# pedro-morgado/spatialaudiogen

Measured on AMD Instinct MI355X. Metric: ambisonic seconds generated/sec (0.1 s windows, 224x448 video), higher is better.
Workload: dtype f32 (fp32 in / out / accumulate; products on the 16-bit matrix cores with fp32-equivalent operand splits: two fp16 planes (3 products per multiply) for the ResNet trunk's 3x3 convs, whose operand ranges batch-norm bounds, three bf16 planes (6 products) elsewhere - measured against the fp64 oracle as

## Files before the change

spatialaudiogen_amd/csrc/fft.hip:

```cpp
#include "kernels.h"
#include <mutex>

namespace sagen {

__device__ float2 g_tw[1024];
__device__ float g_hann[1024];

__global__ void fft_tables_kernel() {
    const int n = blockIdx.x * blockDim.x + threadIdx.x;
    if (n >= 1024) return;
    double s, c;
    sincospi(2.0 * (double)n / 1024.0, &s, &c);
    g_tw[n] = make_float2((float)c, (float)(-s));
    g_hann[n] = (float)(0.5 - 0.5 * cos(2.0 * M_PI / 1024.0 * (double)n));
}

int fft_tables_ensure(hipStream_t s) {
    static std::mutex mu;
    static bool done[64] = {};
    int dev = 0;
    SAGEN_HIP_CHECK(hipGetDevice(&dev));
    std::lock_guard<std::mutex> lk(mu);
    if (dev < 64 && done[dev]) return SAGEN_OK;
    hipLaunchKernelGGL(fft_tables_kernel, dim3(4), dim3(256), 0, s);
    SAGEN_LAUNCH_CHECK();
    SAGEN_HIP_CHECK(hipStreamSynchronize(s));
    if (dev < 64) done[dev] = true;
    return SAGEN_OK;
}

__device__ __forceinline__ float2 cmul(float2 a, float2 b) {
    return make_float2(a.x * b.x - a.y * b.y, a.x * b.y + a.y * b.x);
}

template <bool INV>
__device__ __forceinline__ float2* fft1024(float2* a, float2* b, int tid) {
    float2* src = a;
    float2* dst = b;
#pragma unroll
    for (int s = 0; s < 5; ++s) {
        const int Ns = 1 << (2 * s);
        const int k = tid & (Ns - 1);
        float2 u0 = src[tid], u1 = src[tid + 256], u2 = src[tid + 512], u3 = src[tid + 768];
        if (s > 0) {
            const int step = k * (256 / Ns);
            float2 w1 = g_tw[step], w2 = g_tw[2 * step], w3 = g_tw[3 * step];
            if (INV) { w1.y = -w1.y; w2.y = -w2.y; w3.y = -w3.y; }
            u1 = cmul(u1, w1); u2 = cmul(u2, w2); u3 = cmul(u3, w3);
        }
        const float2 v0 = make_float2(u0.x + u2.x, u0.y + u2.y);
        const float2 v1 = make_float2(u0.x - u2.x, u0.y - u2.y);
        const float2 v2 = make_float2(u1.x + u3.x, u1.y + u3.y);
        const float2 d = make_float2(u1.x - u3.x, u1.y - u3.y);
        const float2 v3 = INV ? make_float2(-d.y, d.x) : make_float2(d.y, -d.x);
        const int j0 = ((tid - k) << 2) + k;
        dst[j0] = make_float2(v0.x + v2.x, v0.y + v2.y);
        dst[j0 + Ns] = make_float2(v1.x + v3.x, v1.y + v3.y);
        dst[j0 + 2 * Ns] = make_float2(v0.x - v2.x, v0.y - v2.y);
        dst[j0 + 3 * Ns] = make_float2(v1.x - v3.x, v1.y - v3.y);
        __syncthreads();
        float2* t = src; src = dst; dst = t;
    }
    return src;
}

__global__ __launch_bounds__(256) void stft_kernel(const float* __restrict__ audio_, int n_samples, int f0, int f1,
                                                   float* __restrict__ mag_, int c0, int c1, float2* __restrict__ spec_,
                                                   float* __restrict__ zero_ptr_, int zero_n, const GroupInfo gi) {
    const float* __restrict__ audio = audio_ + (size_t)blockIdx.z * ((size_t)gridDim.y * n_samples);
    float* __restrict__ mag = SAGEN_GRP(mag_);
    float2* __restrict__ spec = SAGEN_GRP(spec_);
    float* __restrict__ zero_ptr = SAGEN_GRP(zero_ptr_);
    __shared__ float2 bufA[1024], bufB[1024];
    const int tid = threadIdx.x;
    for (int i = (blockIdx.y * gridDim.x + blockIdx.x) * 256 + tid; i < zero_n; i += gridDim.x * gridDim.y * 256) zero_ptr[i] = 0.f;
    const int b = blockIdx.y;
    const int fa = f0 + 2 * blockIdx.x, fb = fa + 1;
    const bool has_b = fb < f1;
    const float* xa = audio + (long)b * n_samples + 256L * fa;
#pragma unroll
    for (int t = 0; t < 4; ++t) {
        const int n = tid + 256 * t;
        const float h = g_hann[n];
        const float va = xa[n] * h;
        const float vb = has_b ? xa[256 + n] * h : 0.f;
        bufA[n] = make_float2(va, vb);
    }
    __syncthreads();
    const float2* Z = fft1024<false>(bufA, bufB, tid);
    const int nf = f1 - f0, nc = c1 - c0;
#pragma unroll
    for (int t = 0; t < 4; ++t) {
        const int k = tid + 256 * t;
        const float2 zk = Z[k];
        float2 zn = Z[(1024 - k) & 1023];
        zn.y = -zn.y;
        const float2 xA = make_float2(0.5f * (zk.x + zn.x), 0.5f * (zk.y + zn.y));
        const float dx = zk.x - zn.x, dy = zk.y - zn.y;
        const float2 xB = make_float2(0.5f * dy, -0.5f * dx);
        if (mag) {
            mag[((long)b * nf + (fa - f0)) * 1024 + k] = sqrtf(xA.x * xA.x + xA.y * xA.y);
            if (has_b) mag[((long)b * nf + (fb - f0)) * 1024 + k] = sqrtf(xB.x * xB.x + xB.y * xB.y);
        }
        if (spec && k <= 512) {
            if (fa >= c0 && fa < c1) spec[((long)b * nc + (fa - c0)) * 513 + k] = xA;
            if (has_b && fb >= c0 && fb < c1) spec[((long)b * nc + (fb - c0)) * 513 + k] = xB;
        }
    }
}

int stft_launch(const float* audio, int B, int n_samples, int f0, int f1, float* mag, int c0, int c1, float* spec,
                hipStream_t s, float* zero_ptr, int zero_n) {
    if (f1 <= f0 || 256L * (f1 - 1) + 1024 > n_samples)
        return fail(SAGEN_ERR_SHAPE, "stft: frames [%d,%d) do not fit %d samples", f0, f1, n_samples);
    if (spec && (c0 < f0 || c1 > f1 || c1 <= c0)) return fail(SAGEN_ERR_SHAPE, "stft: spec frames must lie in [f0,f1)");
    int rc = fft_tables_ensure(s);
    if (rc) return rc;
    const GroupInfo gi = cur_group();
    hipLaunchKernelGGL(stft_kernel, dim3(cdiv(f1 - f0, 2), B, gi.G), dim3(256), 0, s, audio, n_samples, f0, f1, mag, c0, c1,
                       (float2*)spec, zero_ptr, zero_ptr ? zero_n : 0, gi);
    SAGEN_LAUNCH_CHECK();
    return SAGEN_OK;
}

constexpr int MASK_F_LO = 1, MASK_F_HI = 24, MASK_NF = MASK_F_HI - MASK_F_LO;
constexpr int OUT_SHIFT = 1216;

template <int NTR>
__global__ __launch_bounds__(256) void mask_istft_kernel(const float* __restrict__ dmask_, long dmask_bstride, int dmask_f0,
                                                         const float2* __restrict__ spec_, const float* __restrict__ coeffs_,
                                                         float* __restrict__ frames_, const float* __restrict__ ebuf_, const GroupInfo gi) {
    const float* __restrict__ dmask = SAGEN_GRP(dmask_);
    const float2* __restrict__ spec = SAGEN_GRP(spec_);
    const float* __restrict__ coeffs = SAGEN_GRP(coeffs_);
    float* __restrict__ frames = SAGEN_GRP(frames_);
    const float* __restrict__ ebuf = SAGEN_GRP(ebuf_);
    __shared__ __attribute__((aligned(16))) float2 fftbuf[2048];
    float2* const bufA = fftbuf;
    float2* const bufB = fftbuf + 1024;
    __shared__ float E[6][1024];
    __shared__ float2 X[513];
    __shared__ float wl[2][3][NTR];
    const int tid = threadIdx.x;
    const int fi = blockIdx.x, f = MASK_F_LO + fi, b = blockIdx.y;
    const int n_lo = max(256 * f - OUT_SHIFT, 0), n_hi = min(256 * f - OUT_SHIFT + 1023, 4799);
    const int s_lo = n_lo / 1600, s_hi = n_hi / 1600;
    const bool two = s_hi != s_lo;

    for (int i = tid; i < 2 * 3 * NTR; i += 256) {
        const int j = i % NTR, o = (i / NTR) % 3, si = i / (3 * NTR);
        const int st = si ? s_hi : s_lo;
        wl[si][o][j] = coeffs[(((long)b * 3 + st) * 3 + o) * (NTR + 1) + j];
    }
    for (int k = tid; k < 513; k += 256) X[k] = spec[((long)b * 28 + f) * 513 + k];

    if (ebuf != nullptr) {
        const float4* src = reinterpret_cast<const float4*>(ebuf + ((long)b * MASK_NF + fi) * 1024 * 8);
        __syncthreads();
        for (int k = tid; k < 1024; k += 256) {
            const float4 lo = src[2 * k], hi = src[2 * k + 1];
            E[0][k] = lo.x; E[1][k] = lo.y; E[2][k] = lo.z; E[3][k] = lo.w; E[4][k] = hi.x; E[5][k] = hi.y;
        }
        __syncthreads();
    } else {
    constexpr int NC = NTR / 4;
    constexpr int RPP = 4096 / NTR;
    constexpr int TPRW = 256 / RPP;
    constexpr int NPASS = 1024 / RPP;
    float4* const stage = reinterpret_cast<float4*>(fftbuf);
    const float4* src = reinterpret_cast<const float4*>(dmask + (long)b * dmask_bstride + (long)(f - dmask_f0) * 1024 * NTR);
    float4 nx0 = src[tid], nx1 = src[tid + 256], nx2 = src[tid + 512], nx3 = src[tid + 768];
    __syncthreads();
    const int row = tid / TPRW, part = tid % TPRW;
    auto park = [&](int i, const float4& v) {
        const int idx = tid + 256 * i, r = idx / NC, ch = idx % NC;
        stage[r * NC + (ch ^ (r & (NC - 1)))] = v;
    };
#pragma unroll 1
    for (int ps = 0; ps < NPASS; ++ps) {
        park(0, nx0); park(1, nx1); park(2, nx2); park(3, nx3);
        __syncthreads();
        const int pn = ps + 1 < NPASS ? ps + 1 : ps;
        nx0 = src[pn * 1024 + tid]; nx1 = src[pn * 1024 + tid + 256]; nx2 = src[pn * 1024 + tid + 512]; nx3 = src[pn * 1024 + tid + 768];
        float e[6] = {0.f, 0.f, 0.f, 0.f, 0.f, 0.f};
#pragma unroll
        for (int q = 0; q < 4; ++q) {
            const float4 v = stage[row * NC + ((part * 4 + q) ^ (row & (NC - 1)))];
            const float sg[4] = {1.f / (1.f + expf(-v.x)), 1.f / (1.f + expf(-v.y)), 1.f / (1.f + expf(-v.z)),
                                 1.f / (1.f + expf(-v.w))};
#pragma unroll
            for (int u = 0; u < 4; ++u) {
                const int j = (part * 4 + q) * 4 + u;
#pragma unroll
                for (int o = 0; o < 3; ++o) {
                    e[o] = fmaf(wl[0][o][j], sg[u], e[o]);
                    if (two) e[3 + o] = fmaf(wl[1][o][j], sg[u], e[3 + o]);
                }
            }
        }
#pragma unroll
        for (int c = 0; c < 6; ++c) {
            e[c] = wave_sum<1, TPRW>(e[c]);
            if (part == 0) E[c][ps * RPP + row] = e[c];
        }
        __syncthreads();
    }
    }

    float* fout = frames + ((long)b * MASK_NF + fi) * 3 * 1024;
    const int npack = two ? 3 : 2;
    for (int pk = 0; pk < npack; ++pk) {
        int ca, cb;
        if (pk == 0) { ca = 0; cb = 1; }
        else if (pk == 1) { ca = 2; cb = two ? 5 : -1; }
        else { ca = 3; cb = 4; }
#pragma unroll
        for (int t = 0; t < 4; ++t) {
            const int k = tid + 256 * t;
            const int km = (1024 - k) & 1023;
            float2 xk = (k <= 512) ? X[k] : X[km];
            if (k > 512) xk.y = -xk.y;
            const float ma = 0.5f * (E[ca][k] + E[ca][km]);
            const float mb = cb >= 0 ? 0.5f * (E[cb][k] + E[cb][km]) : 0.f;
            bufA[k] = make_float2(ma * xk.x - mb * xk.y, ma * xk.y + mb * xk.x);
        }
        __syncthreads();
        const float2* Y = fft1024<true>(bufA, bufB, tid);
#pragma unroll
        for (int t = 0; t < 4; ++t) {
            const int p = tid + 256 * t;
            const int n = 256 * f + p - OUT_SHIFT;
            if (n >= 0 && n < 4800) {
                const int st = n / 1600;
                const float2 y = Y[p];
                const int oa = ca % 3, sa = (ca / 3) ? s_hi : s_lo;
                if (st == sa) fout[oa * 1024 + p] = y.x * (1.f / 1024.f);
                if (cb >= 0) {
                    const int ob = cb % 3, sb = (cb / 3) ? s_hi : s_lo;
                    if (st == sb) fout[ob * 1024 + p] = y.y * (1.f / 1024.f);
                }
            }
        }
        __syncthreads();
    }
}

__global__ __launch_bounds__(256) void ola_mix_kernel(const float* __restrict__ frames_, const float* __restrict__ coeffs_,
                                                      int ntr, float* __restrict__ out_, int B, const GroupInfo gi) {
    const float* __restrict__ frames = SAGEN_GRP(frames_);
    const float* __restrict__ coeffs = SAGEN_GRP(coeffs_);
    float* __restrict__ out = out_ + (size_t)blockIdx.z * ((size_t)B * 4800 * 3);
    const long total = (long)B * 4800 * 3;
    for (long i = (long)blockIdx.x * 256 + threadIdx.x; i < total; i += (long)gridDim.x * 256) {
        const int o = (int)(i % 3);
        long r = i / 3;
        const int n = (int)(r % 4800);
        const int b = (int)(r / 4800);
        const int st = n / 1600;
        float acc = 0.f;
        const int fl = max((n + 193 + 255) / 256, MASK_F_LO), fh = min((n + OUT_SHIFT) / 256, MASK_F_HI - 1);
        for (int f = fl; f <= fh; ++f)
            acc += frames[(((long)b * MASK_NF + (f - MASK_F_LO)) * 3 + o) * 1024 + (n + OUT_SHIFT - 256 * f)];
        out[i] = fmaf(acc, 0.25f, coeffs[(((long)b * 3 + st) * 3 + o) * (ntr + 1) + ntr]);
    }
}

size_t mask_istft_scratch_bytes(int B) { return (size_t)B * MASK_NF * 3 * 1024 * sizeof(float); }

int mask_istft_mix_launch(const float* dmask, long dmask_bstride, int dmask_f0, const float* spec, const float* coeffs,
                          int B, int ntracks, float* out, float* scratch, hipStream_t s, const float* ebuf) {
    int rc = fft_tables_ensure(s);
    if (rc) return rc;
    if (dmask_f0 > MASK_F_LO) return fail(SAGEN_ERR_SHAPE, "mask_istft: dmask must start at frame <= %d", MASK_F_LO);
    const GroupInfo gi = cur_group();
    dim3 grid(MASK_NF, B, gi.G);
    if (ntracks == 32)
        hipLaunchKernelGGL(mask_istft_kernel<32>, grid, dim3(256), 0, s, dmask, dmask_bstride, dmask_f0, (const float2*)spec, coeffs, scratch, ebuf, gi);
    else if (ntracks == 64)
        hipLaunchKernelGGL(mask_istft_kernel<64>, grid, dim3(256), 0, s, dmask, dmask_bstride, dmask_f0, (const float2*)spec, coeffs, scratch, ebuf, gi);
    else if (ntracks == 16)
        hipLaunchKernelGGL(mask_istft_kernel<16>, grid, dim3(256), 0, s, dmask, dmask_bstride, dmask_f0, (const float2*)spec, coeffs, scratch, ebuf, gi);
    else
        return fail(SAGEN_ERR_UNSUPPORTED, "mask_istft: num_sep_tracks=%d (supported: 16, 32, 64)", ntracks);
    SAGEN_LAUNCH_CHECK();
    const long total = (long)B * 4800 * 3;
    hipLaunchKernelGGL(ola_mix_kernel, dim3((int)std::min<long>(cdiv(total, 256), 4096L), 1, gi.G), dim3(256), 0, s, scratch, coeffs,
                       ntracks, out, B, gi);
    SAGEN_LAUNCH_CHECK();
    return SAGEN_OK;
}

__global__ __launch_bounds__(256) void stft_multi_kernel(const float* __restrict__ audio_, int n_samples, int nin, int f0, int f1,
                                                         float* __restrict__ mag_, int c0, int c1, float2* __restrict__ spec_,
                                                         float* __restrict__ zero_ptr_, int zero_n, const GroupInfo gi) {
    const float* __restrict__ audio = audio_ + (size_t)blockIdx.z * ((size_t)gridDim.y * n_samples * nin);
    float* __restrict__ mag = SAGEN_GRP(mag_);
    float2* __restrict__ spec = SAGEN_GRP(spec_);
    float* __restrict__ zero_ptr = SAGEN_GRP(zero_ptr_);
    __shared__ float2 bufA[1024], bufB[1024];
    const int tid = threadIdx.x;
    for (int i = (blockIdx.y * gridDim.x + blockIdx.x) * 256 + tid; i < zero_n; i += gridDim.x * gridDim.y * 256) zero_ptr[i] = 0.f;
    const int b = blockIdx.y, ch = blockIdx.x % nin;
    const int fa = f0 + 2 * (blockIdx.x / nin), fb = fa + 1;
    const bool has_b = fb < f1;
    const float* xa = audio + ((long)b * n_samples + 256L * fa) * nin + ch;
#pragma unroll
    for (int t = 0; t < 4; ++t) {
        const int n = tid + 256 * t;
        const float h = g_hann[n];
        const float va = xa[(long)n * nin] * h;
        const float vb = has_b ? xa[(long)(256 + n) * nin] * h : 0.f;
        bufA[n] = make_float2(va, vb);
    }
    __syncthreads();
    const float2* Z = fft1024<false>(bufA, bufB, tid);
    const int nf = f1 - f0, nc = c1 - c0;
#pragma unroll
    for (int t = 0; t < 4; ++t) {
        const int k = tid + 256 * t;
        const float2 zk = Z[k];
        float2 zn = Z[(1024 - k) & 1023];
        zn.y = -zn.y;
        const float2 xA = make_float2(0.5f * (zk.x + zn.x), 0.5f * (zk.y + zn.y));
        const float dx = zk.x - zn.x, dy = zk.y - zn.y;
        const float2 xB = make_float2(0.5f * dy, -0.5f * dx);
        if (mag) {
            mag[(((long)b * nf + (fa - f0)) * 1024 + k) * nin + ch] = sqrtf(xA.x * xA.x + xA.y * xA.y);
            if (has_b) mag[(((long)b * nf + (fb - f0)) * 1024 + k) * nin + ch] = sqrtf(xB.x * xB.x + xB.y * xB.y);
        }
        if (spec && k <= 512) {
            float2* sp = spec + ((long)b * nin + ch) * nc * 513;
            if (fa >= c0 && fa < c1) sp[(long)(fa - c0) * 513 + k] = xA;
            if (has_b && fb >= c0 && fb < c1) sp[(long)(fb - c0) * 513 + k] = xB;
        }
    }
}

int stft_multi_launch(const float* audio, int B, int n_samples, int nin, int f0, int f1, float* mag, int c0, int c1, float* spec,
                      hipStream_t s, float* zero_ptr, int zero_n) {
    if (nin < 1 || nin > 16) return fail(SAGEN_ERR_SHAPE, "stft: %d input channels", nin);
    if (f1 <= f0 || 256L * (f1 - 1) + 1024 > n_samples)
        return fail(SAGEN_ERR_SHAPE, "stft: frames [%d,%d) do not fit %d samples", f0, f1, n_samples);
    if (spec && (c0 < f0 || c1 > f1 || c1 <= c0)) return fail(SAGEN_ERR_SHAPE, "stft: spec frames must lie in [f0,f1)");
    int rc = fft_tables_ensure(s);
    if (rc) return rc;
    const GroupInfo gi = cur_group();
    hipLaunchKernelGGL(stft_multi_kernel, dim3(cdiv(f1 - f0, 2) * nin, B, gi.G), dim3(256), 0, s, audio, n_samples, nin, f0, f1, mag, c0, c1,
                       (float2*)spec, zero_ptr, zero_ptr ? zero_n : 0, gi);
    SAGEN_LAUNCH_CHECK();
    return SAGEN_OK;
}

template <int NTR, int NIN, int NOUT>
__global__ __launch_bounds__(256) void mask_istft_hoa_kernel(const float* __restrict__ dmask_, long dmask_bstride, int dmask_f0,
                                                             const float2* __restrict__ spec_, const float* __restrict__ coeffs_,
                                                             float* __restrict__ frames_, const GroupInfo gi) {
    constexpr int QPI = NTR / 4;
    constexpr int CPB = NIN * QPI;
    static_assert(CPB <= 64 && (CPB & (CPB - 1)) == 0, "one bin's chunks must fit a power-of-two lane group of a wave");
    constexpr int BPI = 256 / CPB;
    constexpr int NS = 2 * NOUT;
    const float* __restrict__ dmask = SAGEN_GRP(dmask_);
    const float2* __restrict__ spec = SAGEN_GRP(spec_);
    const float* __restrict__ coeffs = SAGEN_GRP(coeffs_);
    float* __restrict__ frames = SAGEN_GRP(frames_);
    __shared__ float2 Y[NS][1024];
    __shared__ float2 fbuf[2][1024];
    const int tid = threadIdx.x;
    const int fi = blockIdx.x, f = MASK_F_LO + fi, b = blockIdx.y;
    const int n_lo = max(256 * f - OUT_SHIFT, 0), n_hi = min(256 * f - OUT_SHIFT + 1023, 4799);
    const int s_lo = n_lo / 1600, s_hi = n_hi / 1600;
    const bool two = s_hi != s_lo;

    const int q = tid % CPB, i = q / QPI, j0 = (q % QPI) * 4;
    float w[2][NOUT][4];
#pragma unroll
    for (int si = 0; si < 2; ++si)
#pragma unroll
        for (int o = 0; o < NOUT; ++o)
#pragma unroll
            for (int u = 0; u < 4; ++u)
                w[si][o][u] = coeffs[((((long)b * 3 + (si ? s_hi : s_lo)) * NOUT + o) * NIN + i) * (NTR + 1) + j0 + u];
    const float4* src = reinterpret_cast<const float4*>(dmask + (long)b * dmask_bstride + (long)(f - dmask_f0) * 1024 * NIN * NTR);
    const float2* X = spec + ((long)b * NIN + i) * 28 * 513 + (long)f * 513;
#pragma unroll 2
    for (int k = tid / CPB; k < 1024; k += BPI) {
        const float4 v = src[(long)k * CPB + q];
        float2 xk = X[k <= 512 ? k : 1024 - k];
        if (k > 512) xk.y = -xk.y;
        const float sg[4] = {1.f / (1.f + expf(-v.x)), 1.f / (1.f + expf(-v.y)), 1.f / (1.f + expf(-v.z)), 1.f / (1.f + expf(-v.w))};
        float yr[2][NOUT], yi[2][NOUT];
#pragma unroll
        for (int si = 0; si < 2; ++si)
#pragma unroll
            for (int o = 0; o < NOUT; ++o) {
                float m = 0.f;
#pragma unroll
                for (int u = 0; u < 4; ++u) m = fmaf(w[si][o][u], sg[u], m);
                m = wave_sum<1, QPI>(m);
                yr[si][o] = wave_sum<QPI, CPB>(m * xk.x);
                yi[si][o] = wave_sum<QPI, CPB>(m * xk.y);
            }
        if (q == 0) {
#pragma unroll
            for (int si = 0; si < 2; ++si)
#pragma unroll
                for (int o = 0; o < NOUT; ++o) Y[si * NOUT + o][k] = make_float2(yr[si][o], yi[si][o]);
        }
    }
    __syncthreads();

    float* fout = frames + ((long)b * MASK_NF + fi) * NOUT * 1024;
    const int ns = two ? NS : NOUT;
    for (int ca = 0; ca < ns; ca += 2) {
        const int cb = ca + 1 < ns ? ca + 1 : -1;
#pragma unroll
        for (int t = 0; t < 4; ++t) {
            const int k = tid + 256 * t;
            const int km = (1024 - k) & 1023;
            const float2 a0 = Y[ca][k], a1 = Y[ca][km];
            const float2 ha = make_float2(0.5f * (a0.x + a1.x), 0.5f * (a0.y - a1.y));
            float2 hb = make_float2(0.f, 0.f);
            if (cb >= 0) {
                const float2 b0 = Y[cb][k], b1 = Y[cb][km];
                hb = make_float2(0.5f * (b0.x + b1.x), 0.5f * (b0.y - b1.y));
            }
            fbuf[0][k] = make_float2(ha.x - hb.y, ha.y + hb.x);
        }
        __syncthreads();
        const float2* R = fft1024<true>(fbuf[0], fbuf[1], tid);
#pragma unroll
        for (int t = 0; t < 4; ++t) {
            const int p = tid + 256 * t;
            const int n = 256 * f + p - OUT_SHIFT;
            if (n >= 0 && n < 4800) {
                const int st = n / 1600;
                const float2 y = R[p];
                if (st == ((ca / NOUT) ? s_hi : s_lo)) fout[(ca % NOUT) * 1024 + p] = y.x * (1.f / 1024.f);
                if (cb >= 0 && st == ((cb / NOUT) ? s_hi : s_lo)) fout[(cb % NOUT) * 1024 + p] = y.y * (1.f / 1024.f);
            }
        }
        __syncthreads();
    }
}

template <int NIN, int NOUT>
__global__ __launch_bounds__(256) void ola_mix_hoa_kernel(const float* __restrict__ frames_, const float* __restrict__ coeffs_,
                                                          int ntr, float* __restrict__ out_, int B, const GroupInfo gi) {
    const float* __restrict__ frames = SAGEN_GRP(frames_);
    const float* __restrict__ coeffs = SAGEN_GRP(coeffs_);
    float* __restrict__ out = out_ + (size_t)blockIdx.z * ((size_t)B * 4800 * NOUT);
    const long total = (long)B * 4800 * NOUT;
    for (long idx = (long)blockIdx.x * 256 + threadIdx.x; idx < total; idx += (long)gridDim.x * 256) {
        const int o = (int)(idx % NOUT);
        const long r = idx / NOUT;
        const int n = (int)(r % 4800);
        const int b = (int)(r / 4800);
        const int st = n / 1600;
        float acc = 0.f;
        const int fl = max((n + 193 + 255) / 256, MASK_F_LO), fh = min((n + OUT_SHIFT) / 256, MASK_F_HI - 1);
        for (int f = fl; f <= fh; ++f)
            acc += frames[(((long)b * MASK_NF + (f - MASK_F_LO)) * NOUT + o) * 1024 + (n + OUT_SHIFT - 256 * f)];
        out[idx] = fmaf(acc, 0.25f, coeffs[((((long)b * 3 + st) * NOUT + o) * NIN + 0) * (ntr + 1) + ntr]);
    }
}

size_t mask_istft_hoa_scratch_bytes(int B, int nout) { return (size_t)B * MASK_NF * nout * 1024 * sizeof(float); }

int mask_istft_hoa_launch(const float* dmask, long dmask_bstride, int dmask_f0, const float* spec, const float* coeffs, int B,
                          int ntracks, int nin, int nout, float* out, float* scratch, hipStream_t s) {
    int rc = fft_tables_ensure(s);
    if (rc) return rc;
    if (dmask_f0 > MASK_F_LO || dmask_f0 < 0) return fail(SAGEN_ERR_SHAPE, "mask_istft_hoa: dmask must start at frame 0..%d", MASK_F_LO);
    if (nin != 4 || nout != 5) return fail(SAGEN_ERR_UNSUPPORTED, "mask_istft_hoa: (nin, nout) = (%d, %d) (supported: (4, 5), ambi_order 2)", nin, nout);
    const GroupInfo gi = cur_group();
    dim3 grid(MASK_NF, B, gi.G);
    if (ntracks == 32)
        hipLaunchKernelGGL((mask_istft_hoa_kernel<32, 4, 5>), grid, dim3(256), 0, s, dmask, dmask_bstride, dmask_f0, (const float2*)spec, coeffs, scratch, gi);
    else if (ntracks == 64)
        hipLaunchKernelGGL((mask_istft_hoa_kernel<64, 4, 5>), grid, dim3(256), 0, s, dmask, dmask_bstride, dmask_f0, (const float2*)spec, coeffs, scratch, gi);
    else if (ntracks == 16)
        hipLaunchKernelGGL((mask_istft_hoa_kernel<16, 4, 5>), grid, dim3(256), 0, s, dmask, dmask_bstride, dmask_f0, (const float2*)spec, coeffs, scratch, gi);
    else
        return fail(SAGEN_ERR_UNSUPPORTED, "mask_istft_hoa: num_sep_tracks=%d (supported: 16, 32, 64)", ntracks);
    SAGEN_LAUNCH_CHECK();
    const long total = (long)B * 4800 * nout;
    hipLaunchKernelGGL((ola_mix_hoa_kernel<4, 5>), dim3((int)std::min<long>(cdiv(total, 256), 4096L), 1, gi.G), dim3(256), 0, s, scratch, coeffs,
                       ntracks, out, B, gi);
    SAGEN_LAUNCH_CHECK();
    return SAGEN_OK;
}

template <int NTR>
__global__ __launch_bounds__(256) void mask_istft_bwd_kernel(const float* __restrict__ dmask, long dmask_bstride, int dmask_f0,
                                                             const float2* __restrict__ spec, const float* __restrict__ coeffs,
                                                             const float* __restrict__ dpred, float* __restrict__ d_dmask,
                                                             long dd_bstride, int dd_f0, float* __restrict__ partial) {
    __shared__ __attribute__((aligned(16))) float2 fftbuf[2048];
    float2* const bufA = fftbuf;
    float2* const bufB = fftbuf + 1024;
    __shared__ float Q[6][1024];
// ... 162 lines not shown
```

spatialaudiogen_amd/csrc/kernels.h:

```cpp
#pragma once
#include "common.h"
#include "wave_reduce.h"

namespace sagen {

struct BnRef {
    const double* acc = nullptr;
    const float* gamma = nullptr;
    const float* beta = nullptr;
    double inv_count = 0.0;
    float eps = 1e-3f;
};

constexpr int H2_AMAX_SLOTS = 64, H2_AMAX_STRIDE = 32, H2_AMAX_FLOATS = H2_AMAX_SLOTS * H2_AMAX_STRIDE;

struct IgemmDesc {
    const float* x = nullptr;
    const float* w = nullptr;
    int w_split = 0;
    float* y = nullptr;
    const float* bias = nullptr;
    const float* in_scale = nullptr;
    const float* in_shift = nullptr;
    BnRef bn_in;
// ... 2 lines not shown
    float* splitk_ws = nullptr;
    int* sk_ticket = nullptr;
    int sk_rep = 1;
    int M = 0, N = 0, K = 0, Kpad = 0;
    int Hg = 1, Wg = 1, g_h0 = 0, g_w0 = 0;
    int Hin = 1, Win = 1, Cin = 0, ldx = 0;
    long x_bstride = 0;
    int in_sh = 1, in_sw = 1;
    int ntaps = 1, TW = 1, tap_sh = 1, tap_sw = 1, tap_h0 = 0, tap_w0 = 0;
    int log2Cin = -1;
    int dsh = 1, dsw = 1, Cout = 0;
    int Hlim = 1, Wlim = 1;
    long y_bstride = 0;
    long y_rstride = 0;
    int ldy = 0;
    int relu_out = 0;
    int splitk = 1;
    unsigned x_bytes = 0, w_bytes = 0;
    unsigned y_bytes = 0;
    int no_bounds = 0;
    int uniform_taps = 0;
    const void* xp3 = nullptr;
    unsigned xp3_bytes = 0, xp3_cstride = 0;
    int p3_np = 0;
    int xp3_fmt = 0;
    int xp3_row0 = 0, xp3_rows = 0;
    const void* wh2 = nullptr;
    unsigned wh2_bytes = 0;
    const float* h2_a_inv = nullptr;
    const float* h2_w_inv = nullptr;
    unsigned p3_magic_wp = 0, p3_magic_h = 0;
    const float* mm_coeffs = nullptr;
    float* mm_out = nullptr;
    int mm_row0 = 0, mm_nf = 0;
    int mm_f_lo = 1;
    void* trace = nullptr;
    int trace_block = 0;
    GroupInfo grp;
};
__device__ __forceinline__ void igemm_relocate(IgemmDesc& d, int g) {
    const GroupInfo gi = d.grp;
    d.x = grp_ptr(d.x, gi, g); d.y = grp_ptr(d.y, gi, g);
    d.in_scale = grp_ptr(d.in_scale, gi, g); d.in_shift = grp_ptr(d.in_shift, gi, g);
    d.bn_in.acc = grp_ptr(d.bn_in.acc, gi, g);
    d.stats = grp_ptr(d.stats, gi, g); d.amax_out = grp_ptr(d.amax_out, gi, g);
    d.splitk_ws = grp_ptr(d.splitk_ws, gi, g); d.sk_ticket = grp_ptr(d.sk_ticket, gi, g);
    d.xp3 = grp_ptr(d.xp3, gi, g);
    d.h2_a_inv = grp_ptr(d.h2_a_inv, gi, g); d.h2_w_inv = grp_ptr(d.h2_w_inv, gi, g);
    d.mm_coeffs = grp_ptr(d.mm_coeffs, gi, g); d.mm_out = grp_ptr(d.mm_out, gi, g);
}

enum IgemmTile {
    TILE_128x128 = 0, TILE_128x64, TILE_256x64, TILE_64x64, TILE_128x32, TILE_32x128,
    TILE_128x128_S2, TILE_128x64_S2, TILE_256x64_S2, TILE_64x64_S2,
    TILE_64x128, TILE_64x128_S2, TILE_64x256, TILE_64x256_S2, TILE_256x32,
    TILE_64x64_K32, TILE_64x128_K32, TILE_128x64_K32, TILE_128x128_K32, TILE_32x128_K32, TILE_128x32_K32,
    TILE_B3_128x128, TILE_B3_128x64, TILE_B3_256x64, TILE_B3_64x64, TILE_B3_64x128, TILE_B3_64x256, TILE_B3_32x128,
    TILE_B3_128x32,
    TILE_B3_128x64_K2, TILE_B3_64x64_K2, TILE_B3_64x128_K2, TILE_B3_32x128_K2, TILE_B3_128x32_K2,
    TILE_B3DW_128x128, TILE_B3DW_128x64, TILE_B3DW_256x64, TILE_B3DW_64x128, TILE_B3DW_64x64, TILE_B3DW_64x256,
    TILE_B3DWM_128x64, TILE_B3DWM_256x64, TILE_B3DWM_64x64, TILE_B3DWM_64x128,
    TILE_B3S2_256x64, TILE_B3S2_128x64,
    TILE_P3_128x64, TILE_P3_128x128, TILE_P3_64x64,
    TILE_P3PP_PAIR, TILE_P3PP_SPLITK,
    TILE_P3G_128x64_K2, TILE_P3G_64x64_K2, TILE_P3G_64x128_K2, TILE_P3G_128x128_K1,
    TILE_P3H_128x64, TILE_P3H_128x128, TILE_P3H_64x64, TILE_P3H_256x64,
    TILE_P3GH_128x64_K3, TILE_P3GH_64x64_K4, TILE_P3GH_128x128_K2, TILE_P3GH_64x128_K3,
    TILE_P3H_128x64_C2, TILE_P3H_64x64_C2, TILE_P3H_64x64_C4,
    TILE_P3GH_MM_64x128_K2, TILE_P3GH_MM_64x128_K4, TILE_P3GH_MM_128x128_K2, TILE_P3GH_MM_128x256_K2,
    TILE_P3HR_256x64, TILE_P3HR_128x64, TILE_P3HR_64x64_C2,
    TILE_P3HR_128x128,
    TILE_AUTO
};

int igemm_launch(const IgemmDesc& d, IgemmTile tile, hipStream_t s);
int igemm_grid_m(const IgemmDesc& d, IgemmTile tile);
IgemmTile igemm_pick_tile(const IgemmDesc& d);
const char* igemm_tile_name(IgemmTile t);
int igemm_tile_bm(IgemmTile t);
int igemm_tile_bn(IgemmTile t);
int igemm_tile_bk(IgemmTile t);
bool igemm_tile_split(IgemmTile t);
int igemm3_dispatch(const IgemmDesc& d, IgemmTile tile, hipStream_t s);
int igemm3dw_dispatch(const IgemmDesc& d, IgemmTile tile, hipStream_t s);
int igemm3s2_dispatch(const IgemmDesc& d, IgemmTile tile, hipStream_t s);
int conv3p_dispatch(const IgemmDesc& d, IgemmTile tile, hipStream_t s);
int conv3g_dispatch(const IgemmDesc& d, IgemmTile tile, hipStream_t s);
int conv3h_dispatch(const IgemmDesc& d, IgemmTile tile, hipStream_t s);
int h2_filter_pack_launch(const float* wp, int N, int Kpad, void* w2, unsigned* scratch, float* w_inv, hipStream_t s);
struct H2Job {
    const float* wp = nullptr;
    void* w2 = nullptr;
    float* w_inv = nullptr;
    int N = 0, Kpad = 0, first_block = 0, pad_ = 0;
};
int h2_filter_pack_multi_launch(const H2Job* jobs_dev, int njobs, int nblocks, unsigned* amax, hipStream_t s);
bool conv3g_ok(const IgemmDesc& d);
constexpr int SK_TICKETS = 8192;
inline bool igemm_tile_fused_splitk(IgemmTile) { return true; }
bool igemm_tile_p3(IgemmTile t);
bool igemm_tile_grouped(IgemmTile t);
bool igemm_tile_dh_split(IgemmTile t);
bool igemm_p3_eligible(const IgemmDesc& d);
bool igemm_tile_ok(const IgemmDesc& d, IgemmTile t);
constexpr int SPLITK_RB = 16;
int splitk_reduce_launch(const float* ws, int splitk, int M, int N, const float* bias, int relu,
                         float* y, int ldy, int rep, double* stats, hipStream_t s, float* amax_out = nullptr);

struct DeconvGather {
    int B = 0, Hin = 0, Win = 0, kh = 1, kw = 1, sh = 1, sw = 1, Cout = 0;
    int in_row0 = 0, R = 0;
    int y0 = 0, y1 = 0;
    int relu = 0, ldy = 0;
    const float* bias = nullptr;
    float* y = nullptr;
    float* amax_out = nullptr;
};
int deconv_gather_launch(const float* ws, int splitk, const DeconvGather& g, hipStream_t s);

int pack_conv_launch(const float* w_hwio, int ntaps, int cin_src, int cin_pad, int cout,
                     float* wp, int Npad, int Kpad, hipStream_t s, int tw_src = 0, int tw_pad = 0);
int pack_split_launch(float* wp, int N, int Kpad, hipStream_t s);
inline size_t packed_split_floats(size_t n_fp32) { return n_fp32 + (3 * n_fp32 + 1) / 2; }
enum PackKind { PACK_CONV = 0, PACK_DECONV, PACK_FLIPT, PACK_ROWS, PACK_DECONV_PHASE };
struct PackJob {
    const float* src = nullptr;
    float* dst = nullptr;
    int kind = 0, N = 0, Kpad = 0;
    int p[7] = {0, 0, 0, 0, 0, 0, 0};
    int first_block = 0;
};
inline int pack_job_blocks(int kind, long N, long Kpad) {
    return kind == PACK_CONV ? (int)(((N + 31) / 32) * ((Kpad + 31) / 32)) : (int)((N * Kpad + 1023) / 1024);
}
int pack_multi_launch(const PackJob* jobs_dev, int njobs, int nblocks, hipStream_t s, int block0 = 0);
int pack_deconv_launch(const float* w_hwoi, int kh, int kw, int cout, int cin, int sh, int sw,
                       float* wp, int Npad, int Kpad, hipStream_t s);

int bn_finalize_launch(const double* stats, long count, int C, const float* gamma,
                       const float* beta, float eps, float* scale, float* shift, hipStream_t s);
int bn_apply_relu_launch(const float* x, const float* scale, const float* shift, const BnRef& bn, const float* residual,
                         float* y, long n_pixels, int C, hipStream_t s);
int maxpool3x3s2_launch(const float* x, const float* scale, const float* shift, const BnRef& bn, float* y,
                        int B, int H, int W, int C, hipStream_t s);
int pad_nhwc3to4_launch(const float* x, float* y, int B, int H, int W, int pt, int pb, int pl, int pr,
                        hipStream_t s);
int pad_u8_nhwc3to4_launch(const unsigned char* x, float* y, int B, int H, int W, int pt, int pb, int pl, int pr, hipStream_t s);
int stempool_launch(const float* xpad, const float* wp, const float* gamma, float* pooled, double* stats, int B, hipStream_t s);
size_t stem8_plane_bytes(int B);
int stem8_prep_launch(const unsigned char* x, void* plane, int B, hipStream_t s, float* zero_ptr = nullptr, long zero_n = 0, int half = 0);
int stem8pool_h2_launch(const void* plane, const float* wp, const void* wh2, const float* w_inv, const float* gamma, float* pooled, double* stats, int B,
                        hipStream_t s);
int stem8pool_launch(const void* plane, const float* wp, const float* gamma, float* pooled, double* stats, int B, hipStream_t s);
int stem16_prep_launch(const float* x, void* planes, float* part, float* a_inv, int B, hipStream_t s, float* zero_ptr = nullptr, long zero_n = 0);
int stem16pool_launch(const void* planes, const void* wh2, const float* gamma, float* pooled, double* stats, const float* a_inv, const float* w_inv,
                      int B, hipStream_t s);
constexpr int STEM16_PARTS = 1024;
int stem8raw_launch(const void* plane, const float* wp, float* y0, double* stats, int B, hipStream_t s);
int stem8rawpool_launch(const void* plane, const float* wp, const float* gamma, float* y0, float* pooled, double* stats, int B, hipStream_t s);
int assemble_wyzx_launch(const float* audio, const float* yzx, float* out, int B, int snd_size,
                         int snd_contx, int snd_dur, hipStream_t s);
int power_map_launch(const float* ambi, long T, const float* sh, int P, float* rms, hipStream_t s);
int power_map_batched_launch(const float* ambi, int nchunks, long T, const float* sh, int P, float* rms, double* moments, hipStream_t s);
int nosep_mix_launch(const float* audio, const float* coeffs, float* out, int B, int snd_size,
                     int snd_contx, int snd_dur, int num_out, hipStream_t s);
int nosep_mix_multi_launch(const float* audio, const float* coeffs, float* out, int B, int snd_size, int snd_contx,
                           int snd_dur, int nin, int num_out, hipStream_t s);

size_t p3_bytes(int B, int H, int W, int C);
constexpr int H2S_FILTER_FIRST = 8;
constexpr int H2S_FIXED_FIRST = 232;
constexpr int H2S_A_INV_X = 232;
constexpr int H2S_A_INV_B = 236;
constexpr int H2S_S16_A_INV = 238;
constexpr int H2_RIG_OFF = 240;
struct P3hScale {
    float* a_inv = nullptr;
    const float* res_bound = nullptr;
    const double* res_acc = nullptr;
    double res_inv_count = 0.0;
    float* bound_out = nullptr;
    unsigned* sat_count = nullptr;
    unsigned char* relu_bits = nullptr;
    const void* res_planes = nullptr;
    const float* res_a_inv = nullptr;
};
int p3_pack_launch(const float* x, const float* scale, const float* shift, const BnRef& bn, const float* residual, int relu,
                   float* y, void* p3, int B, int H, int W, int C, hipStream_t s, int fmt = 0, const P3hScale* h2 = nullptr);
size_t p3h_bytes(int B, int H, int W, int C);
int h2_pack_rows_launch(const float* x, long x_bstride, long x_rstride, int ldx, int row0, int B, int R, int W, int C, const float* amax0,
                        const float* amax1, void* planes, float* a_inv, unsigned* sat_count, hipStream_t s);
int p3_maxpool_launch(const float* x, const float* scale, const float* shift, const BnRef& bn, float* y, void* p3, int B, int H,
                      int W, int C, hipStream_t s, int fmt = 0, const P3hScale* h2 = nullptr);

int fft_tables_ensure(hipStream_t s);
int stft_launch(const float* audio, int B, int n_samples, int f0, int f1, float* mag,
                int c0, int c1, float* spec, hipStream_t s, float* zero_ptr = nullptr, int zero_n = 0);
size_t mask_istft_scratch_bytes(int B);
int mask_istft_mix_launch(const float* dmask, long dmask_bstride, int dmask_f0, const float* spec,
                          const float* coeffs, int B, int ntracks, float* out, float* scratch,
                          hipStream_t s, const float* ebuf = nullptr);
int stft_multi_launch(const float* audio, int B, int n_samples, int nin, int f0, int f1, float* mag, int c0, int c1, float* spec,
                      hipStream_t s, float* zero_ptr = nullptr, int zero_n = 0);
size_t mask_istft_hoa_scratch_bytes(int B, int nout);
int mask_istft_hoa_launch(const float* dmask, long dmask_bstride, int dmask_f0, const float* spec, const float* coeffs, int B,
                          int ntracks, int nin, int nout, float* out, float* scratch, hipStream_t s);

size_t eval_scratch_floats(int B);
int eval_init_launch(float* scratch, hipStream_t s);
int eval_metrics_launch(const float* pred, const float* gt, int B, float* ps, double* pw, float* scratch, hipStream_t s);
size_t eval_scratch_floats_c(int B, int C);
int eval_metrics_c_launch(const float* pred, const float* gt, int B, int C, float* ps, double* pw, float* scratch, hipStream_t s);
size_t evalx_scratch_floats(int B, int C);
int evalx_mel_env_launch(const float* pred, const float* gt, int B, int C, float* mel_lsd, float* env_mse, float* scratch,
                         hipStream_t s);
int evalx_emd_launch(const float* p, const float* q, int n_maps, int nodes, const double* cost, double* out, unsigned int* not_converged,
                     hipStream_t s);

int stft_loss_grad_launch(const float* pred, const float* gt, const float* mask, int B, float* grad, double* loss, hipStream_t s);
int adam_update_launch(float* p, const float* g, float* m, float* v, long n, float lr_t, float beta1, float beta2, float eps,
                       float gscale, hipStream_t s);

struct WgradDesc {
    const float* g = nullptr;
    const float* d = nullptr;
    float* out = nullptr;
    float* ws = nullptr;
    int B = 1, Hd = 1, Wd = 1;
    int HG = 1, WG = 1, ldg = 0, Cg = 0;
    int ldd = 0, Cd = 0;
    unsigned g_bstride = 0, g_rstride = 0, d_bstride = 0, d_rstride = 0;
    int sh = 1, sw = 1, TH = 1, TW = 1, h0 = 0, w0 = 0;
    int tsh = 1, tsw = 1;
    int splitk = 1;
    int defer_reduce = 0;
    const void* gp = nullptr;
    const void* dp = nullptr;
    const float* gp_a_inv = nullptr;
    const float* dp_a_inv = nullptr;
    unsigned gp_bytes = 0, dp_bytes = 0;
    int P = 0, fold = 1;
    unsigned g_bytes = 0, d_bytes = 0, magic_w = 0, magic_h = 0;
};
int wgrad_launch(const WgradDesc& d, hipStream_t s);
int wgrad_pick_splitk(const WgradDesc& d, size_t ws_capacity_floats);
int wgrad_reduce_launch(const WgradDesc& d, hipStream_t s);
const char* wgrad_kernel_name(const WgradDesc& d);
bool wgrad_reads_fp32_operands();
bool wgrad_planes_enabled();

size_t reduce_scratch_floats(int C);
int relu_bwd_launch(const float* ga, int lda, const float* gb, int ldb, const float* act, int ldact, float* dy, int lddy, long R,
                    int C, double* colsum, float* scratch, hipStream_t s, float* colsum_f32 = nullptr,
                    long band_rows = 0, long batch_rows = 0, long row0 = 0);
int bn_bwd_reduce_launch(const float* ga, const float* gb, const float* act, const float* y, const BnRef& bn, long n_pixels, int C,
                         double* acc, float* scratch, hipStream_t s, int self_mask = 0, float* mx_part = nullptr, int* mx_blocks = nullptr,
                         const unsigned char* relu_bits = nullptr);
int bn_bwd_apply_launch(const float* ga, const float* gb, const float* act, const float* y, const BnRef& bn, const double* acc,
                        long n_pixels, int C, float* dy, float* dz_out, float* dgamma, float* dbeta, hipStream_t s, int self_mask = 0);
int bn_bwd_apply_h2_launch(const float* ga, const float* gb, const float* act, const float* y, const BnRef& bn, const double* acc,
                           int B, int H, int W, int C, float* dy, float* dz_out, float* dgamma, float* dbeta, hipStream_t s, int self_mask,
                           void* planes, const float* mx_part, int mx_blocks, float* a_inv, unsigned* sat_count,
                           const unsigned char* relu_bits = nullptr);
int maxpool_bwd_launch(const float* y0, const BnRef& bn, const float* pooled, const float* ga, const float* gb, float* dz,
                       int B, int H, int W, int C, hipStream_t s);
int maxpool_bn_bwd_launch(const float* y0, const BnRef& bn, const float* pooled, const float* ga, const float* gb, float* dy0, int B,
                          int H, int W, int C, double* acc, float* scratch, float* dgamma, float* dbeta, hipStream_t s,
                          const float* pooled_raw = nullptr);
int sum_rows_launch(const float* ina, int lda, const float* inb, int ldb, int rep, long M, int C, float* out, int ldo, hipStream_t s);
int acc_to_f32_launch(const double* acc, float* dst, int n, hipStream_t s);
int bn_moving_update_launch(const BnRef& bn, float* moving_mean, float* moving_var, int C, float decay, hipStream_t s);
constexpr int BN_MOVING_MAX_JOBS = 40;
struct BnMovingJob { const double* acc = nullptr; double inv_count = 0.0; float* mm = nullptr; float* mv = nullptr; int C = 0; };
int bn_moving_update_multi_launch(const BnMovingJob* jobs, int n, float decay, hipStream_t s);
int pack_conv_flipT_launch(const float* w_hwio, int ntaps, int cin, int cout, float* wp, int Kpad, hipStream_t s);
int pack_rows_launch(const float* w, int rows, int cols, float* wp, int Kpad, hipStream_t s);
int stem_wgrad_unpack_launch(const float* tmp, float* dw, hipStream_t s);

size_t mask_istft_bwd_scratch_floats(int B, int ntracks);
int mask_istft_mix_bwd_launch(const float* dmask, long dmask_bstride, int dmask_f0, const float* spec, const float* coeffs,
                              const float* dpred, int B, int ntracks, float* d_dmask, long dd_bstride, int dd_f0, float* dcoeffs,
                              int ldc, float* scratch, hipStream_t s);

}
```

spatialaudiogen_amd/csrc/model.h:

```cpp
#pragma once
#include "kernels.h"
#include "fcm.h"
#include <algorithm>
#include <cstdlib>
#include <functional>
#include <map>
#include <string>
#include <vector>

namespace sagen {

struct VarSpec {
    std::string name;
    int ndim;
    int64_t shape[4];
    long numel() const {
        long n = 1;
        for (int i = 0; i < ndim; ++i) n *= shape[i];
        return n;
    }
};

struct Buf {
    size_t off = 0, n = 0;
};

struct Named {
    Buf buf;
    size_t extra_off = 0;
    int ndim = 0;
    int64_t shape[4] = {0, 0, 0, 0};
    int64_t pixel_stride = 0;
};

static const int AENC_F[5] = {32, 64, 128, 256, 512};
static const int AENC_K[5][2] = {{7, 16}, {3, 7}, {3, 5}, {3, 5}, {3, 5}};
static const int AENC_S[5][2] = {{4, 8}, {2, 4}, {2, 2}, {1, 1}, {1, 1}};

}

using namespace sagen;

constexpr int SAGEN_MAX_GROUPS = 32;

struct ProfRec {
    std::string kernel, layer;
    double flops = 0.0;
    hipEvent_t e0 = nullptr, e1 = nullptr;
};

struct Choice {
    int tile = -1;
    int splitk = 0;
    float us = 0.f;
};

struct sagen_ctx {
    sagen_config cfg;
    std::map<std::string, Choice> plan;
    std::map<std::string, bool> materialize;
    bool tuning = false;
    bool fp32_only = false;
    bool use_p3 = true;
    int p3_from_stage = 3;
    hipEvent_t tune_e0 = nullptr, tune_e1 = nullptr;
    hipStream_t aux = nullptr;
    hipEvent_t ev_fork = nullptr, ev_join = nullptr, ev_stft = nullptr, ev_pack = nullptr;
    int pack_early_jobs = 0, pack_early_blocks = 0;
    bool late_repack = false;
    bool profiling = false;
    std::vector<ProfRec> prof;
    std::vector<hipEvent_t> event_pool;
    size_t events_used = 0;
    int B = 0;
    int snd_size = 52799, snd_contx = 48000, snd_dur = 4800;
    int enc_h[6], enc_w[6], enc_c[6];
    int Cb = 0;
    int nsep = 32;
    int nin = 1, nout = 3;
    bool has_video = false, has_flow = false, freq_mask = true;

    std::vector<VarSpec> vars;
    std::map<std::string, int> var_index;
    std::vector<const float*> var_ptr;
    bool bound = false;

    int G = 1;
    int tune_groups = 0;
    int inter_group = 0;
    size_t grp_off = 0, grp_floats = 0;
    GroupInfo group_info() const {
        GroupInfo gi;
        if (G > 1 && ws) {
            gi.lo = reinterpret_cast<const char*>(ws + grp_off);
            gi.span = (unsigned long long)grp_floats * sizeof(float);
            gi.stride = gi.span;
            gi.G = G;
        }
        return gi;
    }
    size_t ws_floats = 0;
    float* ws = nullptr;
    std::map<std::string, Buf> bufs;
    std::map<std::string, Named> named;
    std::vector<PackJob> pack_jobs, pack_jobs_bwd;
    int pack_blocks = 0, pack_blocks_bwd = 0;
    bool train_mode = false;
    bool train_ready = false;
    bool stem_fused = true;
    bool materialize_mask = false;
    bool mask_fused_last = false;
    bool video_u8 = false;
    bool train_h2 = true;
    bool use_h2 = true;
    bool train_h2d = true;
    bool no_aud_planes = false;
    bool no_dh_split = false;
    bool sk_fused = false;
    bool train_h2w = true;
    std::map<std::string, int> h2d_slot;
    std::vector<H2Job> h2d_jobs;
    int h2d_blocks = 0;
    std::map<std::string, int> h2_slot;
    std::vector<H2Job> h2_jobs;
    int h2_blocks = 0;
    bool use_p3g = true;
    bool rawpool_last = false;
    bool train_rawpool = true;
    bool train_bands = true;
    int dec_lo[7] = {0, 0, 0, 0, 0, 0, 0}, dec_hi[7] = {0, 0, 0, 0, 0, 0, 0};
    bool no_scatter = false, no_d1_planes = false, no_lean_trunk = false;
    int dec_planes_min_batch = 16;
    bool use_fcm = false;
    std::map<std::string, int> fcm_slices;
    bool stem8h = true;
    bool stem16 = true;
    bool stem8 = true;
    size_t tws_floats = 0;
    float* tws = nullptr;
    std::map<std::string, Buf> tbufs;
    std::vector<float*> grad_ptr;
    std::vector<int> ms_bucket;
    std::vector<int> ms_count, ms_left;
    std::vector<hipEvent_t> ms_event;
    std::vector<char> ms_done;
    std::vector<int> ms_touched;
    hipEvent_t ms_tmp = nullptr;
    std::vector<float*> mov_ptr;
    Buf talloc(const std::string& name, size_t n) {
        Buf b;
        b.off = tws_floats;
        b.n = n;
        tws_floats += (n + 63) / 64 * 64;
        tbufs[name] = b;
        return b;
    }
    size_t cap(const std::string& name) const { auto it = bufs.find(name); return it != bufs.end() ? it->second.n : tbufs.at(name).n; }

    Buf alloc(const std::string& name, size_t n) {
        Buf b;
        b.off = ws_floats;
        b.n = n;
        ws_floats += (n + 63) / 64 * 64;
        bufs[name] = b;
        return b;
    }
    float* p(const std::string& name) const {
        auto it = bufs.find(name);
        if (it != bufs.end()) return ws + it->second.off;
        return tws + tbufs.at(name).off;
    }
    const float* v(const std::string& name) const { return var_ptr[var_index.at(name)]; }
    void add_var(const std::string& name, std::initializer_list<int64_t> shape) {
        VarSpec s;
        s.name = name;
        s.ndim = (int)shape.size();
        int i = 0;
        for (auto d : shape) s.shape[i++] = d;
        for (; i < 4; ++i) s.shape[i] = 1;
        var_index[name] = (int)vars.size();
        vars.push_back(s);
    }
    void expose(const std::string& name, const std::string& buf, size_t extra, std::initializer_list<int64_t> shape,
                int64_t pixel_stride) {
        Named nm;
        nm.buf = bufs.at(buf);
        nm.extra_off = extra;
        nm.ndim = (int)shape.size();
        int i = 0;
        for (auto d : shape) nm.shape[i++] = d;
        nm.pixel_stride = pixel_stride;
        named[name] = nm;
    }
};

namespace sagen {

static inline void add_resnet_vars(sagen_ctx* c, const std::string& scope) {
    auto bn = [&](const std::string& p, int ch) {
        for (const char* leaf : {"beta", "gamma", "moving_mean", "moving_variance"}) c->add_var(p + "/bn/" + leaf, {ch});
    };
    c->add_var(scope + "/conv1/conv/weights", {7, 7, 3, 64});
    bn(scope + "/conv1/conv", 64);
    int cin = 64;
    const int couts[4] = {64, 128, 256, 512};
    for (int st = 0; st < 4; ++st) {
        const int cout = couts[st];
        for (int unit = 1; unit <= 2; ++unit) {
            const std::string pfx = scope + "/conv" + std::to_string(st + 2) + "_" + std::to_string(unit);
            if (unit == 1 && cin != cout) c->add_var(pfx + "/shortcut/weights", {1, 1, cin, cout});
            c->add_var(pfx + "/conv_1/weights", {3, 3, cin, cout});
            bn(pfx + "/conv_1", cout);
            c->add_var(pfx + "/conv_2/weights", {3, 3, cout, cout});
            bn(pfx + "/conv_2", cout);
            cin = cout;
        }
    }
}

static inline bool conv3g_ok_desc(const IgemmDesc& d, int cin) {
    return cin % 16 == 0 && d.Kpad == d.K && d.in_scale == nullptr && d.bn_in.acc == nullptr && d.dsh * d.dsw == 1;
}

static inline size_t packed_floats(long N, long K) { return (size_t)N * ((K + 15) / 16 * 16); }

static inline int auto_splitk(const IgemmDesc& d, IgemmTile tile) {
    const int bm = (tile == TILE_32x128) ? 32 : 64, bn = (tile == TILE_32x128) ? 128 : 64;
    const long blocks = (long)cdiv(d.M, bm) * cdiv(d.N, bn);
    const int nk = d.Kpad / 16;
    if (blocks >= 384 || nk < 16) return 1;
    int sk = (int)std::min<long>({(512 + blocks - 1) / blocks, (long)nk / 8, 64L});
    return std::max(sk, 1);
}

}


int sagen_repack_impl(sagen_ctx* c, hipStream_t s);
int sagen_repack_part(sagen_ctx* c, hipStream_t s, int part);
bool sagen_forward_forks(const sagen_ctx* c);
int sagen_upload_pack_jobs(std::vector<PackJob>& jobs, void* dev, hipStream_t s);
int sagen_forward_impl(sagen_ctx* c, const float* audio, const float* video, const float* flow, float* out, hipStream_t s);

namespace sagen {

struct Fwd {
    sagen_ctx* c;
    hipStream_t s;
    int rc = SAGEN_OK;
    std::string layer;
    std::string wsname = "splitk";
    std::string sfx;
    hipEvent_t wait_before_mfma = nullptr;
    hipEvent_t wait_packs = nullptr;
    std::function<int(const float* ws, int sk, hipStream_t s)> custom_reduce;
    const char* custom_reduce_name = "";

    hipEvent_t next_event() {
        if (c->events_used == c->event_pool.size()) {
            hipEvent_t e = nullptr;
            if (hipEventCreate(&e) != hipSuccess) return nullptr;
            c->event_pool.push_back(e);
        }
        return c->event_pool[c->events_used++];
    }
    template <class F>
    void timed(const char* kernel, double flops, F&& launch) {
        if (rc) return;
        if (!c->profiling) { rc = launch(); return; }
        ProfRec r;
        r.kernel = kernel; r.layer = layer; r.flops = flops;
        r.e0 = next_event(); r.e1 = next_event();
        if (!r.e0 || !r.e1) { rc = fail(SAGEN_ERR_HIP, "hipEventCreate failed"); return; }
        hipError_t he = hipEventRecord(r.e0, s);
        rc = launch();
        if (he == hipSuccess) he = hipEventRecord(r.e1, s);
        if (he != hipSuccess && !rc) rc = fail(SAGEN_ERR_HIP, "hipEventRecord: %s", hipGetErrorString(he));
        c->prof.push_back(r);
    }

    bool dense_out(const IgemmDesc& d) const {
        return d.dsh * d.dsw == 1 && d.g_h0 == 0 && d.g_w0 == 0 && d.y_rstride == (long)d.Wg * d.ldy &&
               (d.M <= d.Hg * d.Wg || d.y_bstride == (long)d.Hg * d.Wg * d.ldy);
    }
    size_t ws_capacity() const { return c->bufs.at(wsname).n; }
    hipError_t memset_groups(void* p, size_t bytes) {
        for (int g = 0; g < c->G; ++g) {
            const hipError_t e = hipMemsetAsync(reinterpret_cast<char*>(p) + (size_t)g * c->grp_floats * sizeof(float), 0, bytes, s);
            if (e != hipSuccess) return e;
        }
// ... 105 lines not shown
        for (int k = 0; k < nc; ++k) {
            std::sort(runs[k].begin(), runs[k].end());
            top[k].us = runs[k][runs[k].size() / 2];
            if (top[k].us < top[best].us) best = k;
        }
        return top[best];
    }

    int contract(const IgemmDesc& d_in, int rep = 1, bool allow_split = true) {
        if (rc) return 0;
        IgemmDesc d = d_in;
        d.w_split = c->fp32_only ? 0 : 1;
        if (rep > 1 && !dense_out(d)) { rc = fail(SAGEN_ERR_UNSUPPORTED, "replicated store needs a dense plain epilogue"); return 0; }
        Choice ch;
        auto it = c->plan.find(layer);
        if (c->tuning) {
            const bool was_prof = c->profiling;
            c->profiling = false;
            ch = tune(d, rep, allow_split);
            c->profiling = was_prof;
            c->plan[layer] = ch;
            if (d.stats && !rc && memset_groups(d.stats, (size_t)2 * d.N * sizeof(double)) != hipSuccess)
                rc = fail(SAGEN_ERR_HIP, "autotune: memset failed");
        } else if (it != c->plan.end()) {
            ch = it->second;
            if (!igemm_tile_ok(d, (IgemmTile)ch.tile)) ch = heuristic(d, rep, allow_split);
            const bool dh3 = ch.splitk == 3 && igemm_tile_dh_split((IgemmTile)ch.tile);
            if (ch.splitk > 1 && (!allow_split || !dense_out(d) || (igemm_tile_p3((IgemmTile)ch.tile) && !dh3) || d.Kpad / igemm_tile_bk((IgemmTile)ch.tile) / ch.splitk < 1)) ch.splitk = 1;
        } else {
            ch = heuristic(d, rep, allow_split);
        }
        if ((ch.splitk > 1 || rep > 1 || custom_reduce) && (size_t)std::max(ch.splitk, 1) * d.M * d.N > ws_capacity()) {
            rc = fail(SAGEN_ERR_WORKSPACE, "split-K scratch too small for %s", layer.c_str());
            return 0;
        }
        return run_choice(d, rep, (IgemmTile)ch.tile, std::max(ch.splitk, 1));
    }
    void gemm(const IgemmDesc& d, int rep = 1, bool allow_split = true) { contract(d, rep, allow_split); }

    IgemmDesc conv_desc(const float* x, int Hin, int Win, int Cin, int ldx, const float* wp, int kh, int kw, int sh, int sw,
                        bool same, int Cout, float* y, int ldy, int& Hout, int& Wout) {
        IgemmDesc d;
        int pt = 0, pl = 0;
        if (same) {
            Hout = cdiv(Hin, sh); Wout = cdiv(Win, sw);
            pt = std::max((Hout - 1) * sh + kh - Hin, 0) / 2;
            pl = std::max((Wout - 1) * sw + kw - Win, 0) / 2;
        } else {
            Hout = (Hin - kh) / sh + 1; Wout = (Win - kw) / sw + 1;
        }
        d.x = x; d.w = wp; d.y = y;
        d.M = c->B * Hout * Wout; d.N = Cout; d.K = kh * kw * Cin; d.Kpad = (d.K + 15) / 16 * 16;
        d.Hg = Hout; d.Wg = Wout;
        d.Hin = Hin; d.Win = Win; d.Cin = Cin; d.ldx = ldx; d.x_bstride = (long)Hin * Win * ldx;
        d.in_sh = sh; d.in_sw = sw;
        d.ntaps = kh * kw; d.TW = kw; d.tap_sh = 1; d.tap_sw = 1; d.tap_h0 = -pt; d.tap_w0 = -pl;
        d.log2Cin = ilog2_exact(Cin);
        d.Cout = Cout; d.Hlim = Hout; d.Wlim = Wout;
        d.ldy = ldy; d.y_rstride = (long)Wout * ldy; d.y_bstride = (long)Hout * Wout * ldy;
        return d;
    }

    void fc(const float* x, int M, int K, int ldx, const std::string& name, int N, bool relu, float* y, int ldy, int rep = 1, float* amax_out = nullptr) {
        layer = name;
        IgemmDesc d;
        d.x = x; d.w = c->p("pk:" + name + "/weights"); d.y = y; d.bias = c->v(name + "/biases");
        d.M = M; d.N = N; d.K = K; d.Kpad = (K + 15) / 16 * 16;
        d.Hg = 1; d.Wg = 1; d.Hin = 1; d.Win = 1; d.Cin = K; d.ldx = ldx; d.x_bstride = ldx;
        d.ntaps = 1; d.Cout = N; d.Hlim = 1; d.Wlim = 1; d.ldy = ldy; d.y_rstride = ldy; d.y_bstride = ldy;
        d.relu_out = relu;
        d.amax_out = amax_out;
        gemm(d, rep);
    }

    void deconv(const float* x, int Hin, int Win, int Cin, int l, float* y, int ldy, bool relu, int a0, int a1, int Ylim,
                long y_bstride, long y_row0, const float* mm_coeffs = nullptr, float* mm_out = nullptr, int mm_nf = 0,
                const std::function<void(IgemmDesc&)>& tweak = nullptr) {
        const std::string name = "separation/deconv" + std::to_string(l + 1);
        layer = name;
        const int kh = AENC_K[l][0], kw = AENC_K[l][1], sh = AENC_S[l][0], sw = AENC_S[l][1];
        const int Cout = l == 0 ? c->nsep * c->nin : AENC_F[l - 1];
        const int Hout = Hin * sh + kh - sh, Wout = Win * sw + kw - sw;
        const int nth = cdiv(kh, sh), ntw = cdiv(kw, sw);
        IgemmDesc d;
        d.x = x; d.w = c->p("pk:" + name + "/weights"); d.bias = c->v(name + "/biases");
        d.Hg = (a1 > a0 ? a1 - a0 : cdiv(Hout, sh)); d.g_h0 = a0; d.Wg = cdiv(Wout, sw);
        d.M = c->B * d.Hg * d.Wg; d.N = sh * sw * Cout; d.K = nth * ntw * Cin; d.Kpad = (d.K + 15) / 16 * 16;
        d.Hin = Hin; d.Win = Win; d.Cin = Cin; d.ldx = Cin; d.x_bstride = (long)Hin * Win * Cin;
        d.ntaps = nth * ntw; d.TW = ntw; d.tap_sh = -1; d.tap_sw = -1; d.log2Cin = ilog2_exact(Cin);
        d.dsh = sh; d.dsw = sw; d.Cout = Cout;
        d.Hlim = Ylim > 0 ? Ylim : Hout; d.Wlim = Wout;
        d.ldy = ldy; d.y_rstride = (long)Wout * ldy;
        d.y_bstride = y_bstride > 0 ? y_bstride : (long)Hout * Wout * ldy;
        d.y = y - y_row0 * d.y_rstride;
        d.relu_out = relu;
        if (mm_out) { d.mm_coeffs = mm_coeffs; d.mm_out = mm_out; d.mm_row0 = (int)y_row0; d.mm_nf = mm_nf; d.mm_f_lo = 1; }
        if (tweak) tweak(d);
        gemm(d);
    }

    float* cat_amax(int l, int half) { return c->p("amax") + (size_t)((l - 1) * 2 + half) * H2_AMAX_FLOATS; }
    float* cat_a_inv(int l) { return c->p("amax") + (size_t)10 * H2_AMAX_FLOATS + l; }
    void deconv_scatter(const float* x, int Hin, int Win, int Cin, int l, float* y, int ldy, bool relu, int in_row0, int R, int y0, int y1,
                        float* amax_out = nullptr, bool x_planes = false) {
        const std::string name = "separation/deconv" + std::to_string(l + 1);
        layer = name;
        DeconvGather gd;
        gd.B = c->B; gd.Hin = Hin; gd.Win = Win; gd.kh = AENC_K[l][0]; gd.kw = AENC_K[l][1]; gd.sh = AENC_S[l][0]; gd.sw = AENC_S[l][1];
        gd.Cout = l == 0 ? c->nsep : AENC_F[l - 1];
        gd.in_row0 = in_row0; gd.R = R; gd.y0 = y0; gd.y1 = y1; gd.relu = relu ? 1 : 0; gd.ldy = ldy;
        gd.bias = c->v(name + "/biases"); gd.y = y; gd.amax_out = amax_out;
        IgemmDesc d;
        d.x = x + (long)in_row0 * Win * Cin; d.w = c->p("pks:" + name + "/weights");
        d.M = c->B * R * Win; d.N = gd.kh * gd.kw * gd.Cout; d.K = Cin; d.Kpad = Cin;
        d.Hg = R; d.Wg = Win; d.Hin = Hin - in_row0; d.Win = Win; d.Cin = Cin; d.ldx = Cin; d.x_bstride = (long)Hin * Win * Cin;
        d.ntaps = 1; d.Cout = d.N; d.Hlim = R; d.Wlim = Win; d.ldy = d.N; d.y_rstride = (long)Win * d.N; d.y_bstride = (long)R * Win * d.N;
        d.y = c->ws + c->bufs.at(wsname).off;
        if (x_planes && !c->tuning) {
            auto it = c->plan.find(name);
            if (it != c->plan.end() && !igemm_tile_p3((IgemmTile)it->second.tile)) x_planes = false;
        }
        if (x_planes) {
            const int lx = l + 1;
            void* planes = c->p("catp");
            timed("h2_pack_rows_kernel", 0.0, [&] {
                return h2_pack_rows_launch(x, (long)Hin * Win * Cin, (long)Win * Cin, Cin, in_row0, c->B, R, Win, Cin, cat_amax(lx, 0), cat_amax(lx, 1), planes,
                                           cat_a_inv(lx), reinterpret_cast<unsigned*>(c->p("h2s") + 7), s); });
            d.xp3 = planes; d.xp3_fmt = 1; d.xp3_row0 = 0; d.xp3_rows = R;
            d.p3_np = c->B * R * (Win + 1);
            d.xp3_cstride = (unsigned)((size_t)d.p3_np * 64);
            d.xp3_bytes = (unsigned)((size_t)d.xp3_cstride * (Cin / 16));
            d.wh2 = c->p("pkhs:" + name + "/weights"); d.wh2_bytes = (unsigned)((size_t)d.N * d.Kpad * 4);
            d.h2_a_inv = cat_a_inv(lx); d.h2_w_inv = c->p("h2s") + c->h2_slot.at("pks:" + name);
        }
        custom_reduce_name = "deconv_gather_kernel";
        custom_reduce = [gd](const float* ws, int sk, hipStream_t st) { return deconv_gather_launch(ws, sk, gd, st); };
        gemm(d);
        custom_reduce = nullptr;
    }

    bool h2() const { return c->use_h2 && c->use_p3 && !c->fp32_only && (!c->train_mode || c->train_h2); }
    int p3_fmt() const { return h2() ? 1 : 0; }
    float* h2_a_inv() { return c->p("h2s") + (sfx.empty() ? 0 : 1); }
    float* h2_a_inv_x(int parity) { return c->p("h2s") + H2S_A_INV_X + 2 * (parity & 1) + (sfx.empty() ? 0 : 1); }
    float* h2_a_inv_b() { return c->p("h2s") + H2S_A_INV_B + (sfx.empty() ? 0 : 1); }
    float* h2_xbound(int parity) { return c->p("h2s") + 2 + 2 * (parity & 1) + (sfx.empty() ? 0 : 1); }
    P3hScale h2_scale(float* bound_out = nullptr, const float* res_bound = nullptr, const double* res_acc = nullptr, double res_inv_count = 0.0) {
        P3hScale h;
        h.a_inv = h2_a_inv(); h.bound_out = bound_out; h.res_bound = res_bound; h.res_acc = res_acc; h.res_inv_count = res_inv_count;
        h.sat_count = reinterpret_cast<unsigned*>(c->p("h2s") + 7);
        return h;
    }

    double* bn_acc(int layer_index) { return reinterpret_cast<double*>(c->p("bnacc" + sfx)) + (size_t)layer_index * 2 * 512; }
    BnRef bn_ref(int layer_index, const std::string& bn_name, long count) {
        BnRef r;
        r.acc = bn_acc(layer_index);
        r.gamma = c->v(bn_name + "/bn/gamma");
        r.beta = c->v(bn_name + "/bn/beta");
        r.inv_count = 1.0 / (double)count;
        r.eps = 1e-3f;
        return r;
    }

    void conv_bn(const float* x, int Hin, int Win, int Cin, const std::string& name, int k, int stride, int Cout,
                 const BnRef& bn_in, float* y, int& Hout, int& Wout, int bn_index, const std::string& plan_key = "",
                 const void* planes = nullptr, const float* planes_a_inv = nullptr) {
        if (rc) return;
        IgemmDesc d = conv_desc(x, Hin, Win, Cin, Cin, c->p("pk:" + name + "/weights"), k, k, stride, stride, true, Cout, y,
                                Cout, Hout, Wout);
        if (planes) {
            d.xp3 = planes;
            d.p3_np = c->B * Hin * (Win + 1);
            auto hs = c->h2_slot.find(name);
            if (h2() && (stride == 1 || c->use_p3g) && k == 3 && hs != c->h2_slot.end()) {
                d.xp3_fmt = 1;
                d.xp3_cstride = (unsigned)((size_t)d.p3_np * 64);
                d.xp3_bytes = (unsigned)p3h_bytes(c->B, Hin, Win, Cin);
                d.wh2 = c->p("pkh:" + name + "/weights");
                d.wh2_bytes = (unsigned)((size_t)d.N * d.Kpad * 4);
                d.h2_a_inv = planes_a_inv ? planes_a_inv : h2_a_inv();
                d.h2_w_inv = c->p("h2s") + hs->second;
            } else {
                d.xp3_cstride = (unsigned)((size_t)d.p3_np * 96);
                d.xp3_bytes = (unsigned)p3_bytes(c->B, Hin, Win, Cin);
            }
        }
        d.bn_in = bn_in;
        d.stats = bn_acc(bn_index);
        layer = plan_key.empty() ? name : plan_key;
        contract(d);
    }

    const float* resnet(const float* img, const std::string& scope) {
        const int B = c->B;
        int li = 0;
        const bool tune_general = c->tuning && c->G == 1;
        const bool fast8 = c->video_u8 && scope == "video_encoder" && c->stem8 && !tune_general && !c->fp32_only && !c->train_mode;
        const bool fast8h = fast8 && c->stem8h && h2() && c->h2_slot.count(scope + "/conv1/conv") != 0;
        const bool fast16 = !fast8 && !(c->video_u8 && scope == "video_encoder") && c->stem16 && !tune_general && !c->fp32_only && !c->train_mode && h2() &&
                            c->use_p3 && c->p3_from_stage <= 2 && c->bufs.count("s16:part" + sfx) != 0 && c->h2_slot.count(scope + "/conv1/conv") != 0;
        if (!fast8 && !fast16 && !rc && hipMemsetAsync(c->p("bnacc" + sfx), 0, c->bufs.at("bnacc" + sfx).n * sizeof(float), s) != hipSuccess)
            rc = fail(SAGEN_ERR_HIP, "hipMemsetAsync(bn accumulators) failed");
        layer = scope + "/pad";
        const bool pool_planes = c->use_p3 && c->p3_from_stage <= 2;
        const bool no_lean = c->no_lean_trunk;
        const bool lean = !no_lean && h2() && pool_planes && c->use_p3g && c->bufs.count("p3b" + sfx) != 0 && !c->train_mode;
        float* const s16_a_inv = c->p("h2s") + H2S_S16_A_INV + (sfx.empty() ? 0 : 1);
        if (fast16)
            timed("stem16_amax_kernel+stem16_prep_kernel", 0.0, [&] { return stem16_prep_launch(img, c->p("xpad" + sfx), c->p("s16:part" + sfx), s16_a_inv, B, s,
                                                                                               c->p("bnacc" + sfx), (long)c->bufs.at("bnacc" + sfx).n); });
        else if (fast8)
            timed("stem8_prep_kernel", 0.0, [&] { return stem8_prep_launch(reinterpret_cast<const unsigned char*>(img), c->p("xpad" + sfx), B, s,
                                                                          c->p("bnacc" + sfx), (long)c->bufs.at("bnacc" + sfx).n, fast8h ? 1 : 0); });
        else if (c->video_u8 && scope == "video_encoder")
            timed("pad_u8_nhwc3to4_kernel", 0.0, [&] { return pad_u8_nhwc3to4_launch(reinterpret_cast<const unsigned char*>(img), c->p("xpad" + sfx), B, 224, 448, 2, 3, 2, 4, s); });
        else
            timed("pad_nhwc3to4_kernel", 0.0, [&] { return pad_nhwc3to4_launch(img, c->p("xpad" + sfx), B, 224, 448, 2, 3, 2, 4, s); });
        int H = 0, W = 0;
        if (!rc && wait_before_mfma) {
            if (hipStreamWaitEvent(s, wait_before_mfma, 0) != hipSuccess) rc = fail(SAGEN_ERR_HIP, "hipStreamWaitEvent failed");
            wait_before_mfma = nullptr;
        }
        {
            const std::string name = scope + "/conv1/conv";
            const bool fused = c->stem_fused && !c->tuning && !c->fp32_only && !(c->use_p3 && c->p3_from_stage <= 2);
            if (fast8 || fast16) {
                H = 112; W = 224;
                layer = name + "+pool";
                if (fast16)
                    timed("stem8pool_kernel<f16>", 2.0 * B * H * W * 64 * 224, [&] {
                        return stem16pool_launch(c->p("xpad" + sfx), c->p("pkh:" + name + "/weights"), c->v(name + "/bn/gamma"), c->p("rx0" + sfx), bn_acc(li),
                                                 s16_a_inv, c->p("h2s") + c->h2_slot.at(name), B, s); });
                else if (fast8h)
                    timed("stem8pool_kernel<h2>", 2.0 * B * H * W * 64 * 224, [&] {
                        return stem8pool_h2_launch(c->p("xpad" + sfx), c->p("pk:" + name + "/weights"), c->p("pkh:" + name + "/weights"), c->p("h2s") + c->h2_slot.at(name),
                                                   c->v(name + "/bn/gamma"), c->p("rx0" + sfx), bn_acc(li), B, s); });
                else
                timed("stem8pool_kernel", 2.0 * B * H * W * 64 * 224, [&] {
                    return stem8pool_launch(c->p("xpad" + sfx), c->p("pk:" + name + "/weights"), c->v(name + "/bn/gamma"), c->p("rx0" + sfx), bn_acc(li), B, s); });
                const BnRef bnf = bn_ref(li, name, (long)B * H * W);
                layer = name + "/bn-relu";
                P3hScale hs0 = h2_scale(h2_xbound(0));
                if (lean) hs0.a_inv = h2_a_inv_x(0);
                if (pool_planes)
                    timed("p3_pack_kernel", 0.0, [&] { return p3_pack_launch(c->p("rx0" + sfx), nullptr, nullptr, bnf, nullptr, 1, lean ? nullptr : c->p("rx0" + sfx), c->p("p3" + sfx), B, 56, 112, 64, s, p3_fmt(), &hs0); });
                else
                    timed("bn_apply_relu_kernel", 0.0, [&] { return bn_apply_relu_launch(c->p("rx0" + sfx), nullptr, nullptr, bnf, nullptr, c->p("rx0" + sfx), (long)B * 56 * 112, 64, s); });
            } else if (fused) {
                H = 112; W = 224;
                layer = name + "+pool";
                timed("stempool_kernel", 2.0 * B * H * W * 64 * 224, [&] {
                    return stempool_launch(c->p("xpad" + sfx), c->p("pk:" + name + "/weights"), c->v(name + "/bn/gamma"), c->p("rx0" + sfx), bn_acc(li), B, s); });
                const BnRef bnf = bn_ref(li, name, (long)B * H * W);
                layer = name + "/bn-relu";
                timed("bn_apply_relu_kernel", 0.0, [&] { return bn_apply_relu_launch(c->p("rx0" + sfx), nullptr, nullptr, bnf, nullptr, c->p("rx0" + sfx), (long)B * 56 * 112, 64, s); });
            } else {
            IgemmDesc d = conv_desc(c->p("xpad" + sfx), 229, 454, 4, 4, c->p("pk:" + name + "/weights"), 7, 8, 2, 2, false, 64,
                                    c->p("y0" + sfx), 64, H, W);
            d.stats = bn_acc(li);
            layer = name;
            contract(d);
            const BnRef bn = bn_ref(li, name, (long)B * H * W);
            if (c->use_p3 && c->p3_from_stage <= 2)
            {
                P3hScale hs0 = h2_scale(h2_xbound(0));
                if (lean) hs0.a_inv = h2_a_inv_x(0);
                timed("p3_maxpool_kernel", 0.0, [&] { return p3_maxpool_launch(c->p("y0" + sfx), nullptr, nullptr, bn, lean ? nullptr : c->p("rx0" + sfx), c->p("p3" + sfx), B, H, W, 64, s, p3_fmt(), &hs0); });
            }
            else
                timed("maxpool3x3s2_kernel", 0.0, [&] { return maxpool3x3s2_launch(c->p("y0" + sfx), nullptr, nullptr, bn, c->p("rx0" + sfx), B, H, W, 64, s); });
            }
            ++li;
            H = (H + 1) / 2; W = (W + 1) / 2;
        }
        float* xin = c->p("rx0" + sfx);
        float* xout = c->p("rx1" + sfx);
        int cin = 64;
        const int couts[4] = {64, 128, 256, 512};
        bool x_in_planes = pool_planes;
        int xb_par = 0;
        bool x_fp32_valid = !lean;
        for (int st = 0; st < 4; ++st) {
            const int cout = couts[st];
            for (int unit = 1; unit <= 2; ++unit) {
                const std::string pfx = scope + "/conv" + std::to_string(st + 2) + "_" + std::to_string(unit);
                const bool first = unit == 1 && cin != cout;
                const int stride = first ? 2 : 1;
                int Ho = 0, Wo = 0;
                const float* shortcut = xin;
                const bool p3_here = c->use_p3 && st + 2 >= c->p3_from_stage;
                void* planes = p3_here ? (void*)c->p((lean ? "p3b" : "p3") + sfx) : nullptr;
                void* const xplanes = p3_here ? (void*)c->p("p3" + sfx) : nullptr;
                const float* const x_ai = lean ? h2_a_inv_x(xb_par) : nullptr;
                const void* in_planes = (p3_here && x_in_planes) ? xplanes : nullptr;
                if (first) {
                    IgemmDesc d = conv_desc(xin, H, W, cin, cin, c->p("pk:" + pfx + "/shortcut/weights"), 1, 1, 2, 2, true,
                                            cout, c->p("rsc" + sfx), cout, Ho, Wo);
                    if (!x_fp32_valid) d.x = nullptr;
                    if (in_planes) {
                        d.xp3 = in_planes;
                        d.p3_np = B * H * (W + 1);
                        auto hs = c->h2_slot.find(pfx + "/shortcut");
                        if (h2() && hs != c->h2_slot.end()) {
                            d.xp3_fmt = 1;
                            d.xp3_cstride = (unsigned)((size_t)d.p3_np * 64);
                            d.xp3_bytes = (unsigned)p3h_bytes(B, H, W, cin);
                            d.wh2 = c->p("pkh:" + pfx + "/shortcut/weights");
                            d.wh2_bytes = (unsigned)((size_t)d.N * d.Kpad * 4);
                            d.h2_a_inv = x_ai ? x_ai : h2_a_inv();
                            d.h2_w_inv = c->p("h2s") + hs->second;
                        } else {
                            d.xp3_cstride = (unsigned)((size_t)d.p3_np * 96);
                            d.xp3_bytes = (unsigned)p3_bytes(B, H, W, cin);
                        }
                    }
                    if (h2() && p3_here) d.stats = bn_acc(20 + st);
                    layer = pfx + "/shortcut";
                    gemm(d, 1, false);
                    shortcut = c->p("rsc" + sfx);
                }
                conv_bn(x_fp32_valid ? xin : nullptr, H, W, cin, pfx + "/conv_1", 3, stride, cout, BnRef(), c->p("ry1" + sfx), Ho, Wo, li, "", in_planes, x_ai);
                const BnRef bn1 = bn_ref(li, pfx + "/conv_1", (long)B * Ho * Wo);
                ++li;
                int H2, W2;
                if (p3_here) {
                    layer = pfx + "/bn1-relu";
                    P3hScale hs1 = h2_scale();
                    if (lean) hs1.a_inv = h2_a_inv_b();
                    timed("p3_pack_kernel", 0.0, [&] { return p3_pack_launch(c->p("ry1" + sfx), nullptr, nullptr, bn1, nullptr, 1, nullptr, planes, B, Ho, Wo, cout, s, p3_fmt(), &hs1); });
                    conv_bn(nullptr, Ho, Wo, cout, pfx + "/conv_2", 3, 1, cout, BnRef(), c->p("ry2" + sfx), H2, W2, li, "", planes, lean ? h2_a_inv_b() : nullptr);
                    const BnRef bn2 = bn_ref(li, pfx + "/conv_2", (long)B * Ho * Wo);
                    layer = pfx + "/merge";
                    const bool to_next_stage = unit == 2 && c->use_p3g && st < 3;
                    const bool next_p3 = unit == 1 || to_next_stage;
                    P3hScale hs2 = first ? h2_scale(h2_xbound(xb_par ^ 1), nullptr, bn_acc(20 + st), 1.0 / ((double)B * Ho * Wo))
                                         : h2_scale(h2_xbound(xb_par ^ 1), h2_xbound(xb_par));
                    const bool res_planes = lean && !first;
                    const bool y_fp32 = lean ? !next_p3 : !to_next_stage;
                    if (lean) {
                        hs2.a_inv = h2_a_inv_x(xb_par ^ 1);
                        if (res_planes) { hs2.res_planes = xplanes; hs2.res_a_inv = h2_a_inv_x(xb_par); }
                    }
                    xb_par ^= 1;
                    timed("p3_pack_kernel", 0.0, [&] { return p3_pack_launch(c->p("ry2" + sfx), nullptr, nullptr, bn2, res_planes ? nullptr : shortcut, 1, y_fp32 ? xout : nullptr, next_p3 ? xplanes : nullptr, B, Ho, Wo, cout, s, p3_fmt(), &hs2); });
                    x_in_planes = next_p3;
                    x_fp32_valid = y_fp32;
                    ++li;
                    std::swap(xin, xout);
                    H = Ho; W = Wo; cin = cout;
                    continue;
                }
                const std::string l2 = pfx + "/conv_2";
                auto run_prologue = [&] { conv_bn(c->p("ry1" + sfx), Ho, Wo, cout, l2, 3, 1, cout, bn1, c->p("ry2" + sfx), H2, W2, li); };
                auto run_materialized = [&](const std::string& key) {
                    layer = pfx + "/bn1-relu";
                    timed("bn_apply_relu_kernel", 0.0, [&] { return bn_apply_relu_launch(c->p("ry1" + sfx), nullptr, nullptr, bn1, nullptr, c->p("ry1n" + sfx), (long)B * Ho * Wo, cout, s); });
                    conv_bn(c->p("ry1n" + sfx), Ho, Wo, cout, l2, 3, 1, cout, BnRef(), c->p("ry2" + sfx), H2, W2, li, key);
                };
                if (c->tuning && !rc) {
                    run_prologue();
                    const float t_pro = c->plan[l2].us;
                    (void)hipEventRecord(c->tune_e0, s);
                    (void)bn_apply_relu_launch(c->p("ry1" + sfx), nullptr, nullptr, bn1, nullptr, c->p("ry1n" + sfx), (long)B * Ho * Wo, cout, s);
                    (void)hipEventRecord(c->tune_e1, s);
                    (void)hipEventSynchronize(c->tune_e1);
                    float ms = 0.f;
                    (void)hipEventElapsedTime(&ms, c->tune_e0, c->tune_e1);
                    if (!rc && hipMemsetAsync(bn_acc(li), 0, (size_t)2 * cout * sizeof(double), s) != hipSuccess) rc = fail(SAGEN_ERR_HIP, "memset failed");
                    run_materialized(l2 + "#mat");
                    const float t_mat = c->plan[l2 + "#mat"].us + ms * 1e3f;
                    c->materialize[l2] = t_mat < t_pro;
                    if (!c->materialize[l2] && !rc) {
                        if (hipMemsetAsync(bn_acc(li), 0, (size_t)2 * cout * sizeof(double), s) != hipSuccess) rc = fail(SAGEN_ERR_HIP, "memset failed");
                        c->tuning = false; run_prologue(); c->tuning = true;
                    }
                } else if (c->materialize.count(l2) && c->materialize[l2]) {
                    run_materialized(l2 + "#mat");
                } else {
                    run_prologue();
                }
                const BnRef bn2 = bn_ref(li, pfx + "/conv_2", (long)B * Ho * Wo);
                layer = pfx + "/merge";
                const bool planes_out = unit == 2 && st < 3 && c->use_p3g && c->use_p3 && st + 3 >= c->p3_from_stage;
                if (planes_out)
                    timed("p3_pack_kernel", 0.0, [&] { return p3_pack_launch(c->p("ry2" + sfx), nullptr, nullptr, bn2, shortcut, 1, nullptr, c->p("p3" + sfx), B, Ho, Wo, cout, s); });
// ... 155 lines not shown
```

spatialaudiogen_amd/csrc/model.hip:

```cpp
#include "model.h"

void sagen_destroy_impl(sagen_ctx* c);
int sagen_groups_impl(const sagen_ctx* c) { return c->G; }
int sagen_create_impl(sagen_ctx** out, const sagen_config* cfg, int groups) {
    if (!out || !cfg) return fail(SAGEN_ERR_NULL, "sagen_create: null argument");
    if (groups < 1 || groups > SAGEN_MAX_GROUPS) return fail(SAGEN_ERR_SHAPE, "sagen_create_grouped: groups=%d (1..%d)", groups, SAGEN_MAX_GROUPS);
    if (groups > 1 && cfg->separation != SAGEN_SEP_FREQ_MASK)
        return fail(SAGEN_ERR_UNSUPPORTED, "sagen_create_grouped: the grouped launch covers the FREQ_MASK path only");
    if (cfg->batch <= 0) return fail(SAGEN_ERR_SHAPE, "sagen_create: batch=%d", cfg->batch);
    if (!(cfg->encoders & SAGEN_ENC_AUDIO))
        return fail(SAGEN_ERR_UNSUPPORTED, "the audio encoder is mandatory (reference model.py:207)");
    if (cfg->audio_rate != 48000 || cfg->video_rate != 10 || cfg->context != 1.0f || cfg->sample_duration != 0.1f ||
        cfg->fft_window != 0.025f)
        return fail(SAGEN_ERR_UNSUPPORTED,
                    "HIP path implements audio_rate=48000 video_rate=10 context=1.0 sample_duration=0.1 "
                    "fft_window=0.025 (the geometry of every BASELINE config)");
    if (cfg->ambi_order != 1 && cfg->ambi_order != 2)
        return fail(SAGEN_ERR_UNSUPPORTED, "ambi_order=%d (supported: 1, 2; order 3 would need audio_encoder/conv1 with cin = 9, "
                    "which the contraction kernels do not take)", cfg->ambi_order);
    if (cfg->separation != SAGEN_SEP_NONE && cfg->separation != SAGEN_SEP_FREQ_MASK)
        return fail(SAGEN_ERR_UNSUPPORTED, "unknown separation mode %d", cfg->separation);
    if (cfg->separation == SAGEN_SEP_NONE && cfg->num_sep_tracks > 1)
        return fail(SAGEN_ERR_UNSUPPORTED, "separation 'none' decodes the mono track only: num_sep_tracks must be 1 (got %d); the reference's fc3 "
                    "would be [.., 3*(num_sep_tracks+1)] (model.py:254) against a single separated track (model.py:274-280)", cfg->num_sep_tracks);
    if (cfg->separation == SAGEN_SEP_FREQ_MASK && cfg->num_sep_tracks != 16 && cfg->num_sep_tracks != 32 &&
        cfg->num_sep_tracks != 64)
        return fail(SAGEN_ERR_UNSUPPORTED, "num_sep_tracks=%d (supported 16/32/64)", cfg->num_sep_tracks);
    if (cfg->n_loc_units < 0 || cfg->n_loc_units > 4) return fail(SAGEN_ERR_SHAPE, "n_loc_units=%d", cfg->n_loc_units);
    for (int i = 0; i < cfg->n_loc_units; ++i)
        if (cfg->loc_units[i] <= 0 || cfg->loc_units[i] % 4) return fail(SAGEN_ERR_UNSUPPORTED, "loc_units[%d]=%d must be a positive multiple of 4", i, cfg->loc_units[i]);

    sagen_ctx* c = new sagen_ctx();
    c->G = groups;

    c->fp32_only = getenv("SAGEN_FP32_ONLY") != nullptr;
    c->use_p3 = !c->fp32_only && getenv("SAGEN_NO_P3") == nullptr;
    if (const char* e = getenv("SAGEN_P3_FROM_STAGE")) c->p3_from_stage = atoi(e);
    c->stem_fused = getenv("SAGEN_NO_STEMPOOL") == nullptr && (getenv("SAGEN_ONE_STREAM") == nullptr || getenv("SAGEN_STEMPOOL") != nullptr);
    c->stem8 = getenv("SAGEN_NO_STEM8") == nullptr;
    c->stem16 = getenv("SAGEN_NO_STEM16") == nullptr;
    c->stem8h = getenv("SAGEN_NO_STEM8_H2") == nullptr;
    c->use_h2 = getenv("SAGEN_NO_H2") == nullptr;
    c->train_h2 = getenv("SAGEN_TRAIN_NO_H2") == nullptr;
    c->train_h2d = getenv("SAGEN_TRAIN_NO_H2D") == nullptr;
    c->train_h2w = getenv("SAGEN_TRAIN_NO_H2W") == nullptr;
    c->sk_fused = getenv("SAGEN_SK_FUSED") != nullptr;
    c->no_dh_split = getenv("SAGEN_NO_DH_SPLIT") != nullptr;
    c->no_aud_planes = getenv("SAGEN_NO_AUDIO_PLANES") != nullptr;
    if (const char* e = getenv("SAGEN_TUNE_GROUPS")) c->tune_groups = atoi(e);
    c->no_scatter = getenv("SAGEN_NO_DECONV_SCATTER") != nullptr;
    c->train_bands = getenv("SAGEN_TRAIN_NO_BANDS") == nullptr;
    c->train_rawpool = getenv("SAGEN_TRAIN_NO_RAWPOOL") == nullptr;
    c->no_d1_planes = getenv("SAGEN_NO_DECONV1_PLANES") != nullptr;
    c->no_lean_trunk = getenv("SAGEN_NO_LEAN_TRUNK") != nullptr;
    if (getenv("SAGEN_NO_DECODER_PLANES") != nullptr) c->dec_planes_min_batch = 1 << 30;
    if (getenv("SAGEN_P3_FROM_STAGE") == nullptr) c->p3_from_stage = (c->use_h2 && c->use_p3) ? 2 : 3;
    c->use_p3g = c->use_p3 && (getenv("SAGEN_P3G") != nullptr || (c->use_h2 && getenv("SAGEN_NO_P3G") == nullptr));
    c->cfg = *cfg;
    c->B = cfg->batch;
    c->has_video = cfg->encoders & SAGEN_ENC_VIDEO;
    c->has_flow = cfg->encoders & SAGEN_ENC_FLOW;
    c->freq_mask = cfg->separation == SAGEN_SEP_FREQ_MASK;
    c->nsep = c->freq_mask ? cfg->num_sep_tracks : 1;
    c->nin = cfg->ambi_order * cfg->ambi_order;
    c->nout = (cfg->ambi_order + 1) * (cfg->ambi_order + 1) - cfg->ambi_order * cfg->ambi_order;
    const int B = c->B;

    c->enc_h[0] = 127; c->enc_w[0] = 1024; c->enc_c[0] = c->nin;
    for (int l = 0; l < 5; ++l) {
        c->enc_h[l + 1] = (c->enc_h[l] - AENC_K[l][0]) / AENC_S[l][0] + 1;
        c->enc_w[l + 1] = (c->enc_w[l] - AENC_K[l][1]) / AENC_S[l][1] + 1;
        c->enc_c[l + 1] = AENC_F[l];
    }
    c->Cb = 1024 + (c->has_video ? 512 : 0) + (c->has_flow ? 512 : 0);

    {
        int cin = c->nin;
        for (int l = 0; l < 5; ++l) {
            const std::string n = "audio_encoder/conv" + std::to_string(l + 1);
            c->add_var(n + "/weights", {AENC_K[l][0], AENC_K[l][1], cin, AENC_F[l]});
            c->add_var(n + "/biases", {AENC_F[l]});
            cin = AENC_F[l];
        }
        if (c->has_video) add_resnet_vars(c, "video_encoder");
        if (c->has_flow) add_resnet_vars(c, "flow_encoder");
        c->add_var("bottleneck/audio-fc/weights", {c->enc_w[5] * c->enc_c[5], 1024});
        c->add_var("bottleneck/audio-fc/biases", {1024});
        for (const char* e : {"video", "flow"}) {
            if ((std::string(e) == "video" && !c->has_video) || (std::string(e) == "flow" && !c->has_flow)) continue;
            c->add_var(std::string("bottleneck/") + e + "-fc-red/weights", {512, 128});
            c->add_var(std::string("bottleneck/") + e + "-fc-red/biases", {128});
            c->add_var(std::string("bottleneck/") + e + "-fc/weights", {7 * 14 * 128, 512});
            c->add_var(std::string("bottleneck/") + e + "-fc/biases", {512});
        }
        int fin = c->Cb;
        for (int i = 0; i < cfg->n_loc_units; ++i) {
            const std::string n = "localization/fc" + std::to_string(i + 1);
            c->add_var(n + "/weights", {fin, cfg->loc_units[i]});
            c->add_var(n + "/biases", {cfg->loc_units[i]});
            fin = cfg->loc_units[i];
        }
        const int nlast = c->nout * c->nin * (c->nsep + 1);
        const std::string n = "localization/fc" + std::to_string(cfg->n_loc_units + 1);
        c->add_var(n + "/weights", {fin, nlast});
        c->add_var(n + "/biases", {nlast});
        if (c->freq_mask) {
            c->add_var("separation/fc-feats/weights", {c->Cb, 512});
            c->add_var("separation/fc-feats/biases", {512});
            const int nfs[5] = {c->nsep * c->nin, 32, 64, 128, 256};
            int dcin = 1024;
            for (int l = 4; l >= 0; --l) {
                const std::string dn = "separation/deconv" + std::to_string(l + 1);
                c->add_var(dn + "/weights", {AENC_K[l][0], AENC_K[l][1], nfs[l], dcin});
                c->add_var(dn + "/biases", {nfs[l]});
                dcin = nfs[l] + (l > 0 ? AENC_F[l - 1] : 0);
            }
        }
    }
    c->var_ptr.assign(c->vars.size(), nullptr);

    size_t h2_pack_blocks = 0;
    for (const auto& vs : c->vars) {
        if (vs.name.size() < 8 || vs.name.compare(vs.name.size() - 8, 8, "/weights") != 0) continue;
        size_t n;
        if (vs.name.find("/deconv") != std::string::npos) {
            const int l = vs.name[vs.name.find("/deconv") + 7] - '1';
            const int sh = AENC_S[l][0], sw = AENC_S[l][1];
            const long taps = (long)cdiv(vs.shape[0], sh) * cdiv(vs.shape[1], sw);
            n = packed_floats((long)sh * sw * vs.shape[2], taps * vs.shape[3]);
        } else if (vs.ndim == 4) {
            long cinp = vs.shape[2] == 3 ? 4 : vs.shape[2];
            long taps = vs.shape[0] * vs.shape[1];
            if (vs.shape[2] == 3) taps = vs.shape[0] * (vs.shape[1] + 1);
            if (vs.shape[2] == 1) { cinp = vs.shape[1]; taps = vs.shape[0]; }
            n = packed_floats(vs.shape[3], taps * cinp);
        } else {
            n = packed_floats(vs.shape[1], vs.shape[0]);
        }
        c->alloc("pk:" + vs.name, packed_split_floats(n));
        if (vs.name.find("/deconv") != std::string::npos) {
            const int l = vs.name[vs.name.find("/deconv") + 7] - '1';
            if (l >= 1 && vs.shape[3] % 16 == 0) {
                const size_t ns = packed_floats((long)vs.shape[0] * vs.shape[1] * vs.shape[2], vs.shape[3]);
                c->alloc("pks:" + vs.name, packed_split_floats(ns));
                c->alloc("pkhs:" + vs.name, ns);
                h2_pack_blocks += ns / 1024 + 1;
                c->h2_slot["pks:" + vs.name.substr(0, vs.name.size() - 8)] = -1;
            }
        }
        if ((vs.ndim == 4 && ((vs.shape[0] == 3 && vs.shape[1] == 3) || (vs.shape[0] == 1 && vs.shape[1] == 1)) && vs.shape[2] % 16 == 0 &&
             vs.name.find("_encoder/conv") != std::string::npos) || vs.name == "separation/deconv1/weights" ||
            (vs.ndim == 4 && vs.shape[2] == 3 && vs.name.find("_encoder/conv1/conv/weights") != std::string::npos) ||
            (vs.ndim == 4 && vs.shape[2] % 16 == 0 && vs.name.compare(0, 18, "audio_encoder/conv") == 0)) {
            c->alloc("pkh:" + vs.name, n);
            h2_pack_blocks += n / 1024 + 1;
            c->h2_slot[vs.name.substr(0, vs.name.size() - 8)] = -1;
        }
    }
    {
        int slot = H2S_FILTER_FIRST;
        for (auto& kv : c->h2_slot) kv.second = slot++;
        static_assert(H2S_A_INV_X + 4 <= H2S_A_INV_B && H2S_A_INV_B + 2 <= H2S_S16_A_INV && H2S_S16_A_INV + 2 <= H2_RIG_OFF &&
                      2 + H2_RIG_OFF + 4 <= 256, "h2s: the fixed slots overlap");
        if (slot > H2S_FIXED_FIRST) return fail(SAGEN_ERR_UNSUPPORTED, "too many fp16x2 layers for the scale table");
    }
    c->alloc("h2:jobs", (c->h2_slot.size() + 1) * sizeof(H2Job) / sizeof(float) + 64);
    c->alloc("h2:amax", c->h2_slot.size() + h2_pack_blocks + 64);
    c->alloc("pk:jobs", (c->vars.size() + 1) * sizeof(PackJob) / sizeof(float) + 64);
    c->grp_off = c->ws_floats;
    c->alloc("h2s", 256);
    c->alloc("mag", (size_t)B * 127 * 1024 * c->nin);
    c->alloc("spec", (size_t)B * c->nin * 28 * 513 * 2);
    for (int l = 1; l <= 5; ++l)
        c->alloc("cat" + std::to_string(l), (size_t)B * c->enc_h[l] * c->enc_w[l] * 2 * c->enc_c[l]);
    c->alloc("bott", (size_t)B * 3 * c->Cb);
    for (int i = 0; i < cfg->n_loc_units; ++i) c->alloc("loc" + std::to_string(i + 1), (size_t)B * 3 * cfg->loc_units[i]);
    c->alloc("coeffs", (size_t)B * 3 * c->nout * c->nin * (c->nsep + 1));
    {
        struct L { std::string name; int rows, K, N; };
        std::vector<L> ls;
        ls.push_back({"bottleneck/audio-fc", 3 * B, c->enc_w[5] * c->enc_c[5], 1024});
        if (c->has_video) ls.push_back({"bottleneck/video-fc", B, 7 * 14 * 128, 512});
        if (c->has_flow) ls.push_back({"bottleneck/flow-fc", B, 7 * 14 * 128, 512});
        int fin = c->Cb;
        for (int i = 0; i < cfg->n_loc_units; ++i) { ls.push_back({"localization/fc" + std::to_string(i + 1), 3 * B, fin, cfg->loc_units[i]}); fin = cfg->loc_units[i]; }
        ls.push_back({"localization/fc" + std::to_string(cfg->n_loc_units + 1), 3 * B, fin, c->nout * c->nin * (c->nsep + 1)});
        if (c->freq_mask) ls.push_back({"separation/fc-feats", 3 * B, c->Cb, 512});
        bool ok = getenv("SAGEN_FCM") != nullptr && !c->sk_fused && 3 * B <= FCM_MAX_M;
        for (const L& l : ls) ok = ok && fcm_pick_slices(l.K, (long)l.K * l.N) > 0;
        c->use_fcm = ok;
        if (ok)
            for (const L& l : ls) {
                int ns = fcm_pick_slices(l.K, (long)l.K * l.N);
                if (l.name == "separation/fc-feats") ns = c->fcm_slices.at("localization/fc1");
// ... 125 lines not shown
        j.kind = PACK_DECONV;
        j.N = sh * sw * (int)vs.shape[2];
        j.Kpad = (nth * ntw * (int)vs.shape[3] + 15) / 16 * 16;
        j.p[0] = (int)vs.shape[0]; j.p[1] = (int)vs.shape[1]; j.p[2] = (int)vs.shape[2]; j.p[3] = (int)vs.shape[3]; j.p[4] = sh; j.p[5] = sw; j.p[6] = ntw;
    } else if (vs.ndim == 4) {
        int cin = (int)vs.shape[2], cinp = cin == 3 ? 4 : cin, taps = (int)(vs.shape[0] * vs.shape[1]);
        if (cin == 1) { cin = cinp = (int)vs.shape[1]; taps = (int)vs.shape[0]; }
        const bool stem = cin == 3;
        if (stem) taps = (int)(vs.shape[0] * (vs.shape[1] + 1));
        j.kind = PACK_CONV;
        j.N = (int)vs.shape[3];
        j.Kpad = (taps * cinp + 15) / 16 * 16;
        j.p[0] = taps; j.p[1] = cin; j.p[2] = cinp; j.p[3] = (int)vs.shape[3];
        j.p[4] = stem ? (int)vs.shape[1] : 0; j.p[5] = stem ? (int)vs.shape[1] + 1 : 0;
    } else {
        const int K = (int)vs.shape[0], N = (int)vs.shape[1];
        j.kind = PACK_CONV;
        j.N = N; j.Kpad = (K + 15) / 16 * 16;
        j.p[0] = 1; j.p[1] = K; j.p[2] = K; j.p[3] = N;
    }
    return j;
}

int sagen_upload_pack_jobs(std::vector<PackJob>& jobs, void* dev, hipStream_t s) {
    int nb = 0;
    for (auto& j : jobs) { j.first_block = nb; nb += pack_job_blocks(j.kind, j.N, j.Kpad); }
    if (!jobs.empty() && hipMemcpyAsync(dev, jobs.data(), jobs.size() * sizeof(PackJob), hipMemcpyHostToDevice, s) != hipSuccess) return -1;
    return nb;
}

int sagen_repack_part(sagen_ctx* c, hipStream_t s, int part) {
    if (c->pack_jobs.empty()) {
        for (int pass = 0; pass < 2; ++pass) {
            for (const auto& vs : c->vars) {
                if (vs.name.size() < 8 || vs.name.compare(vs.name.size() - 8, 8, "/weights") != 0) continue;
                const bool stem = vs.name.find("/conv1/conv/") != std::string::npos;
                if (stem == (pass == 0)) c->pack_jobs.push_back(forward_pack_job(c, vs));
                if (pass == 1 && c->bufs.count("pks:" + vs.name)) {
                    PackJob j;
                    j.src = c->v(vs.name); j.dst = c->p("pks:" + vs.name);
                    j.kind = PACK_ROWS;
                    j.N = (int)(vs.shape[0] * vs.shape[1] * vs.shape[2]); j.Kpad = (int)vs.shape[3];
                    j.p[0] = j.N; j.p[1] = (int)vs.shape[3];
                    c->pack_jobs.push_back(j);
                }
            }
            if (pass == 0) c->pack_early_jobs = (int)c->pack_jobs.size();
        }
        if (c->pack_jobs.size() * sizeof(PackJob) > c->bufs.at("pk:jobs").n * sizeof(float)) return fail(SAGEN_ERR_WORKSPACE, "pack job table too small");
        c->pack_blocks = sagen_upload_pack_jobs(c->pack_jobs, c->p("pk:jobs"), s);
        if (c->pack_blocks < 0) return fail(SAGEN_ERR_HIP, "pack job upload failed");
        c->pack_early_blocks = c->pack_early_jobs < (int)c->pack_jobs.size() ? c->pack_jobs[c->pack_early_jobs].first_block : c->pack_blocks;
    }
    const PackJob* jobs = reinterpret_cast<const PackJob*>(c->p("pk:jobs"));
    const int ne = c->pack_early_jobs, be = c->pack_early_blocks, n = (int)c->pack_jobs.size();
    int rc = SAGEN_OK;
    if (part == 1) return ne > 0 ? pack_multi_launch(jobs, ne, be, s) : SAGEN_OK;
    if (part == 2) rc = n > ne ? pack_multi_launch(jobs + ne, n - ne, c->pack_blocks - be, s, be) : SAGEN_OK;
    else rc = pack_multi_launch(jobs, n, c->pack_blocks, s);
    if (rc || c->fp32_only || !c->use_p3) return rc;
    if (c->h2_jobs.empty()) {
        int nb = 0;
        for (const auto& kv : c->h2_slot) {
            const bool scatter = kv.first.compare(0, 4, "pks:") == 0;
            const std::string vname = (scatter ? kv.first.substr(4) : kv.first) + "/weights";
            const VarSpec* vs = nullptr;
            for (const auto& v : c->vars) if (v.name == vname) vs = &v;
            if (!vs) continue;
            H2Job j;
            if (scatter) {
                j.N = (int)(vs->shape[0] * vs->shape[1] * vs->shape[2]); j.Kpad = (int)vs->shape[3];
                j.wp = c->p("pks:" + vs->name); j.w2 = c->p("pkhs:" + vs->name); j.w_inv = c->p("h2s") + kv.second;
                j.first_block = nb;
                nb += (int)(((long)j.N * j.Kpad + 1023) / 1024);
                c->h2_jobs.push_back(j);
                continue;
            }
            j.N = (int)vs->shape[3]; j.Kpad = (int)(vs->shape[0] * vs->shape[1] * vs->shape[2]);
            if (vs->shape[2] == 3) j.Kpad = (int)(vs->shape[0] * (vs->shape[1] + 1) * 4);
            if (vs->name.find("/deconv") != std::string::npos) {
                const int l = vs->name[vs->name.find("/deconv") + 7] - '1';
                j.N = AENC_S[l][0] * AENC_S[l][1] * (int)vs->shape[2];
                j.Kpad = cdiv(vs->shape[0], AENC_S[l][0]) * cdiv(vs->shape[1], AENC_S[l][1]) * (int)vs->shape[3];
            }
            j.wp = c->p("pk:" + vs->name); j.w2 = c->p("pkh:" + vs->name); j.w_inv = c->p("h2s") + kv.second;
            j.first_block = nb;
            nb += (int)(((long)j.N * j.Kpad + 1023) / 1024);
            c->h2_jobs.push_back(j);
        }
        c->h2_blocks = nb;
        if (c->h2_jobs.size() * sizeof(H2Job) > c->bufs.at("h2:jobs").n * sizeof(float)) return fail(SAGEN_ERR_WORKSPACE, "fp16x2 job table too small");
        if (!c->h2_jobs.empty() && hipMemcpyAsync(c->p("h2:jobs"), c->h2_jobs.data(), c->h2_jobs.size() * sizeof(H2Job), hipMemcpyHostToDevice, s) != hipSuccess)
            return fail(SAGEN_ERR_HIP, "fp16x2 job upload failed");
    }
    return h2_filter_pack_multi_launch(reinterpret_cast<const H2Job*>(c->p("h2:jobs")), (int)c->h2_jobs.size(), c->h2_blocks,
                                       reinterpret_cast<unsigned*>(c->p("h2:amax")), s);
}
int sagen_repack_impl(sagen_ctx* c, hipStream_t s) { return sagen_repack_part(c, s, 0); }
bool sagen_forward_forks(const sagen_ctx* c) {
    static const bool one_stream = getenv("SAGEN_ONE_STREAM") != nullptr;
    return c->aux && !c->tuning && !one_stream && (c->has_video || c->has_flow);
}


int sagen_forward_impl(sagen_ctx* c, const float* audio, const float* video, const float* flow, float* out, hipStream_t s) {
    if (!c || !audio || !out) return fail(SAGEN_ERR_NULL, "sagen_forward: null argument");
    if (!c->bound) return fail(SAGEN_ERR_WEIGHTS, "sagen_forward: weights are not bound");
    if (c->has_video && !video) return fail(SAGEN_ERR_NULL, "sagen_forward: video encoder enabled but video is NULL");
    if (c->has_flow && !flow) return fail(SAGEN_ERR_NULL, "sagen_forward: flow encoder enabled but flow is NULL");
    const int B = c->B;
    c->events_used = 0;
    c->prof.clear();
    struct GroupScope {
        GroupInfo saved;
        explicit GroupScope(const GroupInfo& gi) : saved(cur_group()) { cur_group() = gi; }
        ~GroupScope() { cur_group() = saved; }
    } group_scope(c->group_info());
    if (c->G > 1) {
        if (c->train_mode) return fail(SAGEN_ERR_UNSUPPORTED, "the training step has no grouped launch");
        if (!c->freq_mask || c->fp32_only || !c->use_h2 || !c->use_p3 || !c->use_p3g || c->p3_from_stage > 2 || c->no_lean_trunk || c->use_fcm || c->sk_fused ||
            (c->has_video && !c->video_u8 && !c->stem16) || (c->has_video && c->video_u8 && !c->stem8) || (c->has_flow && !c->stem16))
            return fail(SAGEN_ERR_UNSUPPORTED, "grouped forward: an option moved the path off the kernels that take a group dimension "
                        "(fp16x2 / planes_from_stage / plane_gather / u8_fast_stem / f16_fast_stem must keep their defaults)");
    }

    const bool forked = sagen_forward_forks(c);
    Fwd f{c, s};
    Fwd g{c, forked ? c->aux : s};
    auto bail = [&](int rc) {
        if (forked) {
            if (hipEventRecord(c->ev_join, c->aux) == hipSuccess) (void)hipStreamWaitEvent(s, c->ev_join, 0);
            else (void)hipStreamSynchronize(c->aux);
        }
        return rc;
    };
    if (forked) {
        g.wsname = "splitk_aux";
        SAGEN_HIP_CHECK(hipEventRecord(c->ev_fork, s));
        SAGEN_HIP_CHECK(hipStreamWaitEvent(c->aux, c->ev_fork, 0));
    }

    const bool no_d1p = c->no_d1_planes;
    bool d1_planes = !no_d1p && !c->sk_fused && c->freq_mask && !c->train_mode && !c->materialize_mask && !c->fp32_only && c->nsep == 32 && c->nin == 1 && f.h2() &&
                     c->bufs.count("cat1p") != 0 && c->h2_slot.count("separation/deconv1") != 0 && getenv("SAGEN_NO_MASKFUSE") == nullptr;
    if (d1_planes && !c->tuning) {
        auto it = c->plan.find("separation/deconv1");
        if (it != c->plan.end() && !igemm_tile_p3((IgemmTile)it->second.tile)) d1_planes = false;
    }
    const bool no_decp = c->dec_planes_min_batch > (1 << 29);
    static const bool train_no_decp = getenv("SAGEN_TRAIN_NO_DEC_PLANES") != nullptr;
    const bool dec_planes = !no_decp && c->B >= c->dec_planes_min_batch && !c->sk_fused && c->freq_mask && !(c->train_mode && (train_no_decp || !c->train_bands)) &&
                            !c->fp32_only && f.h2() && c->bufs.count("catp") != 0 && !c->no_scatter;
    const bool want_amax = d1_planes || dec_planes;

    g.layer = "stft";
    if (c->nin == 1)
        g.timed("stft_kernel", 0.0, [&] { return stft_launch(audio, B, c->snd_size, 46, 173, c->p("mag"), 89, 117, c->p("spec"), g.s,
                                                             want_amax ? c->p("amax") : nullptr, 10 * H2_AMAX_FLOATS + 64); });
    else
        g.timed("stft_multi_kernel", 0.0, [&] { return stft_multi_launch(audio, B, c->snd_size, c->nin, 46, 173, c->p("mag"), 89, 117, c->p("spec"), g.s,
                                                                         want_amax ? c->p("amax") : nullptr, 10 * H2_AMAX_FLOATS + 64); });
    if (forked) {
        SAGEN_HIP_CHECK(hipEventRecord(c->ev_stft, c->aux));
        f.wait_before_mfma = c->ev_stft;
    }
    if (c->late_repack) {
        c->late_repack = false;
        if (!forked) return bail(fail(SAGEN_ERR_UNSUPPORTED, "late repack without a second stream"));
        const int rc = sagen_repack_part(c, c->aux, 2);
        if (rc) return bail(rc);
        SAGEN_HIP_CHECK(hipEventRecord(c->ev_pack, c->aux));
        f.wait_packs = c->ev_pack;
    }

    for (int l = 0; l < 5 && !g.rc; ++l) {
        const std::string name = "audio_encoder/conv" + std::to_string(l + 1);
        const int ce = c->enc_c[l + 1];
        float* y = c->p("cat" + std::to_string(l + 1)) + (l == 4 ? 0 : ce);
        int Ho, Wo;
        IgemmDesc d;
        if (l == 0 && c->nin > 1) {
            d = g.conv_desc(c->p("mag"), 127, 1024, c->nin, c->nin, c->p("pk:" + name + "/weights"), 7, 16, 4, 8, false, ce, y, 2 * ce, Ho, Wo);
        } else if (l == 0) {
            d = g.conv_desc(c->p("mag"), 127, 1024, 16, 1, c->p("pk:" + name + "/weights"), 7, 1, 4, 8, false, ce, y, 2 * ce, Ho, Wo);
            Wo = c->enc_w[1];
            d.M = B * Ho * Wo; d.Wg = Wo; d.Wlim = Wo;
            d.y_rstride = (long)Wo * 2 * ce; d.y_bstride = (long)Ho * Wo * 2 * ce;
        } else {
            const int cp = c->enc_c[l];
            const float* x = c->p("cat" + std::to_string(l)) + (l == 5 ? 0 : cp);
            d = g.conv_desc(x, c->enc_h[l], c->enc_w[l], cp, 2 * cp, c->p("pk:" + name + "/weights"), AENC_K[l][0], AENC_K[l][1],
                            AENC_S[l][0], AENC_S[l][1], false, ce, y, 2 * ce, Ho, Wo);
        }
        d.bias = c->v(name + "/biases");
        d.relu_out = 1;
        if (want_amax) d.amax_out = g.cat_amax(l + 1, 1);
        g.layer = name;
        bool aud_planes = l >= 1 && want_amax && !c->no_aud_planes && f.h2() && c->bufs.count("aencp") != 0 && c->h2_slot.count(name) != 0 &&
                          conv3g_ok_desc(d, c->enc_c[l]);
        if (aud_planes && !c->tuning) {
            auto it = c->plan.find(name);
            if (it != c->plan.end() ? !igemm_tile_p3((IgemmTile)it->second.tile)
                                    : B < 128)
                aud_planes = false;
        }
        if (aud_planes) {
            const int cp = c->enc_c[l], Hl = c->enc_h[l], Wl = c->enc_w[l];
            float* const a_inv = c->p("amax") + (size_t)10 * H2_AMAX_FLOATS + 8 + l;
            g.layer = name + "/planes";
            g.timed("h2_pack_rows_kernel", 0.0, [&] {
                return h2_pack_rows_launch(c->p("cat" + std::to_string(l)) + cp, (long)Hl * Wl * 2 * cp, (long)Wl * 2 * cp, 2 * cp, 0, B, Hl, Wl, cp,
                                           g.cat_amax(l, 1), nullptr, c->p("aencp"), a_inv, reinterpret_cast<unsigned*>(c->p("h2s") + 7), g.s); });
            g.layer = name;
            d.xp3 = c->p("aencp"); d.xp3_fmt = 1; d.xp3_row0 = 0; d.xp3_rows = 0;
            d.p3_np = B * Hl * (Wl + 1);
            d.xp3_cstride = (unsigned)((size_t)d.p3_np * 64);
            d.xp3_bytes = (unsigned)((size_t)d.xp3_cstride * (cp / 16));
            d.wh2 = c->p("pkh:" + name + "/weights"); d.wh2_bytes = (unsigned)((size_t)d.N * d.Kpad * 4);
            d.h2_a_inv = a_inv; d.h2_w_inv = c->p("h2s") + c->h2_slot.at(name);
        }
        g.gemm(d);
    }

    float* bott = c->p("bott");
    const bool fcm = c->use_fcm && !c->train_mode && !c->tuning;
    auto fcm_layer = [&](Fwd& w, const std::string& label, int M, int K, const std::vector<FcmSeg>& segs, const std::vector<std::string>& names, const std::vector<int>& Ns) {
        FcmDesc fd;
        fd.M = M; fd.K = K; fd.nseg = (int)segs.size(); fd.njobs = (int)names.size(); fd.nslices = c->fcm_slices.at(names[0]);
        for (size_t q = 0; q < segs.size(); ++q) fd.seg[q] = segs[q];
        double fl = 0.0;
        for (size_t j = 0; j < names.size(); ++j) {
            fd.job[j].w = c->v(names[j] + "/weights"); fd.job[j].N = Ns[j]; fd.job[j].out = c->p("fcm:" + names[j]);
            fl += 2.0 * M * K * Ns[j];
        }
        w.layer = label;
        w.timed(M <= 32 ? "fcm_kernel<1>" : (M <= 64 ? "fcm_kernel<2>" : "fcm_kernel<3>"), fl, [&] { return fcm_launch(fd, w.s); });
    };
    auto fcm_finish = [&](Fwd& w, const std::string& name, int rows, int N, bool relu, float* y, int ldy, int rep, float* amax_out = nullptr) {
        w.layer = name;
        w.timed("splitk_reduce_kernel", 0.0, [&] {
            return splitk_reduce_launch(c->p("fcm:" + name), c->fcm_slices.at(name), rows, N, c->v(name + "/biases"), relu ? 1 : 0, y, ldy, rep, nullptr, w.s, amax_out); });
    };
    if (fcm) {
        std::vector<FcmSeg> segs(6);
        for (int wq = 0; wq < 6; ++wq) {
            segs[wq].p = c->p("cat5") + (size_t)wq * 1024; segs[wq].k0 = wq * 512; segs[wq].k1 = (wq + 1) * 512; segs[wq].ld = 6 * 1024;
        }
        fcm_layer(g, "bottleneck/audio-fc", B * 3, 6 * 512, segs, {"bottleneck/audio-fc"}, {1024});
        fcm_finish(g, "bottleneck/audio-fc", B * 3, 1024, true, bott, c->Cb, 1);
    } else {
        IgemmDesc d;
        d.x = c->p("cat5"); d.w = c->p("pk:bottleneck/audio-fc/weights"); d.y = bott; d.bias = c->v("bottleneck/audio-fc/biases");
        d.M = B * 3; d.N = 1024; d.K = 6 * 512; d.Kpad = d.K;
        d.Hg = 3; d.Wg = 1; d.Hin = 3; d.Win = 6; d.Cin = 512; d.ldx = 1024; d.x_bstride = 3L * 6 * 1024;
        d.ntaps = 6; d.TW = 6; d.log2Cin = 9;
        d.Cout = 1024; d.Hlim = 3; d.Wlim = 1; d.ldy = c->Cb; d.y_rstride = c->Cb; d.y_bstride = 3L * c->Cb;
        d.relu_out = 1;
        g.layer = "bottleneck/audio-fc";
        g.gemm(d);
    }
    int choff = 1024;
    for (int e = 0; e < 2; ++e) {
        const bool on = e == 0 ? c->has_video : c->has_flow;
        if (!on) continue;
        const std::string enc = e == 0 ? "video" : "flow";
        Fwd& w = (e == 1 && c->has_video) ? g : f;
        w.sfx = (e == 1 && c->has_video) ? "_b" : "";
        const float* feat = c->train_mode ? w.resnet_train(e == 0 ? video : flow, enc + "_encoder")
                                          : w.resnet(e == 0 ? video : flow, enc + "_encoder");
        w.fc(feat, B * 98, 512, 512, "bottleneck/" + enc + "-fc-red", 128, true, c->p("fcred" + w.sfx), 128);
        if (fcm) {
            FcmSeg sg;
            sg.p = c->p("fcred" + w.sfx); sg.k0 = 0; sg.k1 = 98 * 128; sg.ld = 98 * 128;
            fcm_layer(w, "bottleneck/" + enc + "-fc", B, 98 * 128, {sg}, {"bottleneck/" + enc + "-fc"}, {512});
            fcm_finish(w, "bottleneck/" + enc + "-fc", B, 512, true, bott + choff, c->Cb, 3);
        } else {
            w.fc(c->p("fcred" + w.sfx), B, 98 * 128, 98 * 128, "bottleneck/" + enc + "-fc", 512, true, bott + choff, c->Cb, 3);
        }
        choff += 512;
    }
    if (f.rc || g.rc) return bail(f.rc ? f.rc : g.rc);
    if (forked) {
        SAGEN_HIP_CHECK(hipEventRecord(c->ev_join, c->aux));
        SAGEN_HIP_CHECK(hipStreamWaitEvent(s, c->ev_join, 0));
    }

    static const bool no_fork2 = getenv("SAGEN_NO_FORK2") != nullptr;
    const bool fork2 = forked && c->freq_mask && !no_fork2;
    const int nlast_fcm = c->nout * c->nin * (c->nsep + 1);
    if (fcm) {
        const int M3 = B * 3, nl = c->cfg.n_loc_units;
        auto plain = [&](const float* x, int K) { FcmSeg sg; sg.p = x; sg.k0 = 0; sg.k1 = K; sg.ld = K; return sg; };
        std::vector<std::string> names{"localization/fc1"};
        std::vector<int> Ns{nl > 0 ? c->cfg.loc_units[0] : nlast_fcm};
        if (c->freq_mask) { names.push_back("separation/fc-feats"); Ns.push_back(512); }
        fcm_layer(f, c->freq_mask ? "localization/fc1+separation/fc-feats" : "localization/fc1", M3, c->Cb, {plain(bott, c->Cb)}, names, Ns);
        if (c->freq_mask) fcm_finish(f, "separation/fc-feats", M3, 512, true, c->p("cat5") + 512, 1024, 6, want_amax ? f.cat_amax(5, 0) : nullptr);
        if (fork2) {
            SAGEN_HIP_CHECK(hipEventRecord(c->ev_fork, s));
            SAGEN_HIP_CHECK(hipStreamWaitEvent(c->aux, c->ev_fork, 0));
        }
        Fwd& w = fork2 ? g : f;
        int K = Ns[0];
        for (int i = 1; i <= nl; ++i) {
            const std::string prev = "localization/fc" + std::to_string(i), cur = "localization/fc" + std::to_string(i + 1);
            const int N = i < nl ? c->cfg.loc_units[i] : nlast_fcm;
            float* y = c->p("loc" + std::to_string(i));
            fcm_finish(w, prev, M3, K, true, y, K, 1);
            fcm_layer(w, cur, M3, K, {plain(y, K)}, {cur}, {N});
            K = N;
        }
        fcm_finish(w, "localization/fc" + std::to_string(nl + 1), M3, nlast_fcm, false, c->p("coeffs"), nlast_fcm, 1);
        if (f.rc || g.rc) return bail(f.rc ? f.rc : g.rc);
    } else {
// ... 61 lines not shown
        SAGEN_HIP_CHECK(hipStreamWaitEvent(s, c->ev_join, 0));
    }
    float* const ebuf = fused_tail ? c->p("dmask") : nullptr;
    std::function<void(IgemmDesc&)> d1_tweak = nullptr;
    if (d1_planes && fused_tail) {
        const int W1 = c->enc_w[1], C1 = 2 * c->enc_c[1];
        f.layer = "separation/cat1-planes";
        f.timed("h2_pack_rows_kernel", 0.0, [&] {
            return h2_pack_rows_launch(c->p("cat1"), (long)c->enc_h[1] * W1 * C1, (long)W1 * C1, C1, 10, B, 7, W1, C1, f.cat_amax(1, 0), f.cat_amax(1, 1), c->p("cat1p"),
                                       f.cat_a_inv(1), reinterpret_cast<unsigned*>(c->p("h2s") + 7), s); });
        const float* w_inv = c->p("h2s") + c->h2_slot.at("separation/deconv1");
        const void* planes = c->p("cat1p");
        const void* wh2 = c->p("pkh:separation/deconv1/weights");
        const float* a_inv = f.cat_a_inv(1);
        d1_tweak = [=](IgemmDesc& d) {
            d.xp3 = planes; d.xp3_fmt = 1; d.xp3_row0 = 10; d.xp3_rows = 7;
            d.p3_np = B * 7 * (W1 + 1);
            d.xp3_cstride = (unsigned)((size_t)d.p3_np * 64);
            d.xp3_bytes = (unsigned)((size_t)d.xp3_cstride * (C1 / 16));
            d.wh2 = wh2; d.wh2_bytes = (unsigned)((size_t)d.N * d.Kpad * 4);
            d.h2_a_inv = a_inv; d.h2_w_inv = w_inv;
        };
    }
    const int nmask = c->nsep * c->nin;
    f.deconv(c->p("cat1"), 31, 127, 64, 0, c->p("dmask"), nmask, false, 11, 17, 67, 23L * 1024 * nmask, 44, c->p("coeffs"), ebuf, 23, d1_tweak);
    if (fork2 && !fused_tail) {
        SAGEN_HIP_CHECK(hipEventRecord(c->ev_join, c->aux));
        SAGEN_HIP_CHECK(hipStreamWaitEvent(s, c->ev_join, 0));
    }
    f.layer = "separation/mask-istft-mix";
    if (c->nin > 1) {
        f.timed("mask_istft_hoa_kernel+ola_mix_hoa_kernel", 0.0, [&] {
            return mask_istft_hoa_launch(c->p("dmask"), 23L * 1024 * nmask, 1, c->p("spec"), c->p("coeffs"), B, c->nsep, c->nin, c->nout, out,
                                         c->p("frames"), s); });
        return f.rc;
    }
    f.timed("mask_istft_kernel+ola_mix_kernel", 0.0, [&] {
        return mask_istft_mix_launch(c->p("dmask"), 23L * 1024 * c->nsep, 1, c->p("spec"), c->p("coeffs"), B, c->nsep, out,
                                     c->p("frames"), s, ebuf); });
    return f.rc;
}
int sagen_forward_u8_impl(sagen_ctx* c, const float* audio, const uint8_t* video_u8, const float* flow, float* out, hipStream_t s) {
    if (!c) return fail(SAGEN_ERR_NULL, "sagen_forward_u8: null ctx");
    if (!c->has_video) return fail(SAGEN_ERR_UNSUPPORTED, "sagen_forward_u8: the video encoder is not enabled");
    c->video_u8 = true;
    const int rc = sagen_forward_impl(c, audio, reinterpret_cast<const float*>(video_u8), flow, out, s);
    c->video_u8 = false;
    return rc;
}
void sagen_destroy_impl(sagen_ctx* c) {
    if (!c) return;
    for (hipEvent_t e : c->event_pool) (void)hipEventDestroy(e);
    if (c->tune_e0) { (void)hipEventDestroy(c->tune_e0); (void)hipEventDestroy(c->tune_e1); }
    if (c->ev_fork) (void)hipEventDestroy(c->ev_fork);
    if (c->ev_join) (void)hipEventDestroy(c->ev_join);
    if (c->ev_stft) (void)hipEventDestroy(c->ev_stft);
    if (c->ev_pack) (void)hipEventDestroy(c->ev_pack);
    if (c->aux) (void)hipStreamDestroy(c->aux);
    delete c;
}


int sagen_autotune_impl(sagen_ctx* c, const float* audio, const float* video, const float* flow, float* out, hipStream_t s) {
    if (!c) return fail(SAGEN_ERR_NULL, "sagen_autotune: null ctx");
    if (getenv("SAGEN_NO_AUTOTUNE")) return SAGEN_OK;
    if (!c->tune_e0) {
        SAGEN_HIP_CHECK(hipEventCreate(&c->tune_e0));
        SAGEN_HIP_CHECK(hipEventCreate(&c->tune_e1));
    }
    c->plan.clear();
    c->materialize.clear();
    c->tuning = true;
    const int rc = sagen_forward_impl(c, audio, video, flow, out, s);
    c->tuning = false;
    if (rc) { c->plan.clear(); return rc; }
    SAGEN_HIP_CHECK(hipStreamSynchronize(s));
    return SAGEN_OK;
}

int sagen_plan_set_impl(sagen_ctx* c, const char* layer, int tile, int splitk) {
    const std::string name(layer);
    const std::string sfx = "#materialize";
    if (name.size() > sfx.size() && name.compare(name.size() - sfx.size(), sfx.size(), sfx) == 0) {
        c->materialize[name.substr(0, name.size() - sfx.size())] = splitk != 0;
        return SAGEN_OK;
    }
    if (tile < 0 || tile >= (int)TILE_AUTO || splitk < 1 || splitk > 64) return fail(SAGEN_ERR_SHAPE, "sagen_plan_set: tile=%d splitk=%d", tile, splitk);
    Choice ch;
    ch.tile = tile; ch.splitk = splitk;
    c->plan[layer] = ch;
    return SAGEN_OK;
}

int sagen_plan_describe_impl(sagen_ctx* c, char* buf, size_t buflen) {
    std::string out;
    for (const auto& kv : c->plan) {
        char line[512];
        snprintf(line, sizeof line, "%s\t%s\t%d\t%.2f\n", kv.first.c_str(), igemm_tile_name((IgemmTile)kv.second.tile),
                 kv.second.splitk, kv.second.us);
        out += line;
    }
    int n = (int)c->plan.size();
    for (const auto& kv : c->materialize) {
        out += kv.first + "#materialize\t-\t" + (kv.second ? "1" : "0") + "\t0\n";
        ++n;
    }
    if (out.size() + 1 > buflen) return fail(SAGEN_ERR_WORKSPACE, "plan description needs %zu bytes", out.size() + 1);
    memcpy(buf, out.c_str(), out.size() + 1);
    return n;
}

int sagen_profile_enable_impl(sagen_ctx* c, int on) {
    c->profiling = on != 0;
    c->prof.clear();
    c->events_used = 0;
    return SAGEN_OK;
}

int sagen_profile_report_impl(sagen_ctx* c, char* buf, size_t buflen) {
    std::string out;
    for (const ProfRec& r : c->prof) {
        float ms = 0.f;
        hipError_t e = hipEventSynchronize(r.e1);
        if (e == hipSuccess) e = hipEventElapsedTime(&ms, r.e0, r.e1);
        if (e != hipSuccess) return fail(SAGEN_ERR_HIP, "profile: %s", hipGetErrorString(e));
        char line[512];
        snprintf(line, sizeof line, "%s\t%s\t%.3f\t%.6g\n", r.kernel.c_str(), r.layer.c_str(), ms * 1e3, r.flops);
        out += line;
    }
    if (out.size() + 1 > buflen) return fail(SAGEN_ERR_WORKSPACE, "profile report needs %zu bytes", out.size() + 1);
    memcpy(buf, out.c_str(), out.size() + 1);
    return (int)c->prof.size();
}
size_t sagen_workspace_bytes_impl(const sagen_ctx* c) { return c->ws_floats * sizeof(float); }
int sagen_num_variables_impl(const sagen_ctx* c) { return (int)c->vars.size(); }
int sagen_variable_spec_impl(const sagen_ctx* c, int i, const char** name, int32_t* ndim, int64_t shape[4]) {
    if (i < 0 || i >= (int)c->vars.size()) return fail(SAGEN_ERR_SHAPE, "variable index %d out of range", i);
    *name = c->vars[i].name.c_str();
    *ndim = c->vars[i].ndim;
    for (int k = 0; k < 4; ++k) shape[k] = c->vars[i].shape[k];
    return SAGEN_OK;
}
int sagen_set_option_impl(sagen_ctx* c, const char* name, int value) {
    const std::string n = name;
    if (n == "materialize_mask") { c->materialize_mask = value != 0; return SAGEN_OK; }
    if (n == "intermediate_group") {
        if (value < 0 || value >= c->G) return fail(SAGEN_ERR_SHAPE, "intermediate_group=%d of %d groups", value, c->G);
        c->inter_group = value;
        return SAGEN_OK;
    }
    if (n == "u8_fast_stem") { c->stem8 = value != 0; return SAGEN_OK; }
    if (n == "f16_fast_stem") { c->stem16 = value != 0; return SAGEN_OK; }
    if (n == "u8_stem_h2") { c->stem8h = value != 0; return SAGEN_OK; }
    if (n == "train_bands") { c->train_bands = value != 0; return SAGEN_OK; }
    if (n == "train_rawpool") { c->train_rawpool = value != 0; return SAGEN_OK; }
    if (n == "fp16x2") { c->use_h2 = value != 0; return SAGEN_OK; }
    if (n == "planes_from_stage") { if (value < 2 || value > 6) return fail(SAGEN_ERR_SHAPE, "planes_from_stage in 2..6"); c->p3_from_stage = value; return SAGEN_OK; }
    if (n == "decoder_planes") { c->dec_planes_min_batch = value ? 1 : (1 << 30); return SAGEN_OK; }
    if (n == "plane_gather") { c->use_p3g = c->use_p3 && value != 0; return SAGEN_OK; }
    return fail(SAGEN_ERR_UNSUPPORTED, "sagen_set_option: unknown option %s", name);
}

int sagen_counter_impl(sagen_ctx* c, const char* name, uint64_t* value, hipStream_t s) {
    if (!c->ws) return fail(SAGEN_ERR_WORKSPACE, "no workspace bound");
    if (std::string(name) != "fp16x2_saturations") return fail(SAGEN_ERR_UNSUPPORTED, "sagen_counter: unknown counter %s", name);
    unsigned v[SAGEN_MAX_GROUPS] = {0};
    for (int g = 0; g < c->G; ++g)
        SAGEN_HIP_CHECK(hipMemcpyAsync(&v[g], c->p("h2s") + (size_t)g * c->grp_floats + 7, sizeof(unsigned), hipMemcpyDeviceToHost, s));
    SAGEN_HIP_CHECK(hipStreamSynchronize(s));
    uint64_t tot = 0;
    for (int g = 0; g < c->G; ++g) tot += v[g];
    *value = tot;
    return SAGEN_OK;
}

int sagen_get_intermediate_impl(const sagen_ctx* c, const char* name, const float** data, int32_t* ndim, int64_t shape[4],
                                int64_t* pixel_stride) {
    if (!c->ws) return fail(SAGEN_ERR_WORKSPACE, "no workspace bound");
    auto it = c->named.find(name);
    if (it == c->named.end()) return fail(SAGEN_ERR_SHAPE, "unknown intermediate %s", name);
    const Named& nm = it->second;
    if (c->mask_fused_last && std::string(name) == "separation/deconv1")
        return fail(SAGEN_ERR_UNSUPPORTED, "separation/deconv1: the last forward fused the mask into the deconvolution's epilogue - "
                    "sagen_set_option(ctx, \"materialize_mask\", 1) keeps the logits");
    *data = c->ws + nm.buf.off + nm.extra_off + (size_t)c->inter_group * c->grp_floats;
    *ndim = nm.ndim;
    for (int k = 0; k < 4; ++k) shape[k] = nm.shape[k];
    *pixel_stride = nm.pixel_stride;
    return SAGEN_OK;
}
```

spatialaudiogen_amd/csrc/stem8.hip:

```cpp
#include "igemm3_common.h"
#include "h2_planes.h"

namespace sagen {

constexpr int S8_PH = 8, S8_PW = 7;
constexpr int S8_RH = 2 * S8_PH + 1;
constexpr int S8_RW = 2 * S8_PW + 1;
constexpr int S8_M = S8_RH * S8_RW;
__device__ __forceinline__ int s8_slot(int m) { return m ^ ((m >> 1) & 1); }
constexpr int S8_UH = 229, S8_UW = 456;
constexpr int S8_NH = 32;
constexpr int S8_W_BYTES = 14 * 3 * S8_NH * 32;
constexpr int S8_CT_BYTES = 256 * S8_NH * 4;
constexpr int S8_THREADS = 512;
constexpr int S8_LDS = S8_W_BYTES + S8_CT_BYTES + 2 * 8 * S8_NH * 4 + S8_NH * 4;
typedef _Float16 f16x8s __attribute__((ext_vector_type(8)));

size_t stem8_plane_bytes(int B) { return (size_t)B * S8_UH * S8_UW * 8; }

template <bool HALF>
__global__ __launch_bounds__(256) void stem8_prep_kernel(const unsigned char* __restrict__ x_, u32x2* __restrict__ plane_, int B,
                                                         float* __restrict__ zero_ptr_, long zero_n, const GroupInfo gi) {
    const unsigned char* __restrict__ x = x_ + (size_t)blockIdx.z * ((size_t)B * 224 * 448 * 3);
    u32x2* __restrict__ plane = SAGEN_GRP(plane_);
    float* __restrict__ zero_ptr = SAGEN_GRP(zero_ptr_);
    const long total = (long)B * S8_UH * S8_UW;
    for (long i = (long)blockIdx.x * 256 + threadIdx.x; i < zero_n; i += (long)gridDim.x * 256) zero_ptr[i] = 0.f;
    auto conv = [](unsigned u) -> unsigned {
        return HALF ? (unsigned)__builtin_bit_cast(unsigned short, (_Float16)(float)((int)u - 128))
                    : __builtin_bit_cast(unsigned, (float)((int)u - 128)) >> 16;
    };
    constexpr int QW = S8_UW / 4;
    static_assert(S8_UW % 4 == 0, "plane rows are whole quads");
    const long nquad = (long)B * S8_UH * QW;
    const unsigned border = HALF ? 0xB800u : 0xBF00u;
    for (long iq = (long)blockIdx.x * 256 + threadIdx.x; iq < nquad; iq += (long)gridDim.x * 256) {
        long p = iq;
        const int q = (int)(p % QW); p /= QW;
        const int h = (int)(p % S8_UH) - 2;
        const int b = (int)(p / S8_UH);
        const int w0 = 4 * q - 2;
        u32x2 o[4];
        if ((unsigned)h < 224u && w0 >= 0 && w0 + 3 < 448) {
            const long ob = (((long)b * 224 + h) * 448 + w0) * 3;
            constexpr unsigned sh = 2;
            const unsigned* src = reinterpret_cast<const unsigned*>(x + (ob - sh));
            const unsigned d[4] = {src[0], src[1], src[2], src[3]};
            unsigned by[12];
#pragma unroll
            for (int k = 0; k < 12; ++k) by[k] = (d[(sh + k) >> 2] >> (8 * ((sh + k) & 3))) & 0xffu;
#pragma unroll
            for (int k = 0; k < 4; ++k) o[k] = u32x2{conv(by[3 * k]) | (conv(by[3 * k + 1]) << 16), conv(by[3 * k + 2])};
        } else {
#pragma unroll
            for (int k = 0; k < 4; ++k) {
                const int w = w0 + k;
                unsigned c0 = border, c1 = border, c2 = border;
                if ((unsigned)h < 224u && (unsigned)w < 448u) {
                    const unsigned char* src = x + (((long)b * 224 + h) * 448 + w) * 3;
                    c0 = conv(src[0]); c1 = conv(src[1]); c2 = conv(src[2]);
                }
                o[k] = u32x2{c0 | (c1 << 16), c2};
            }
        }
        u32x4* dst = reinterpret_cast<u32x4*>(plane + iq * 4);
        dst[0] = u32x4{o[0][0], o[0][1], o[1][0], o[1][1]};
        dst[1] = u32x4{o[2][0], o[2][1], o[3][0], o[3][1]};
    }
    (void)total;
}

template <int OUT, int MODE = 0>
__global__ __launch_bounds__(S8_THREADS, 2) void stem8pool_kernel(const char* __restrict__ plane_, const float* __restrict__ wf32,
                                                                  const char* __restrict__ wplanes, const float* __restrict__ gamma,
                                                                  float* __restrict__ pooled_, double* __restrict__ stats_, int B,
                                                                  long plane_stride, const float* __restrict__ a_inv_, const float* __restrict__ w_inv_,
                                                                  float* __restrict__ raw2_, const GroupInfo gi) {
    const char* __restrict__ plane = SAGEN_GRP(plane_);
    float* __restrict__ pooled = SAGEN_GRP(pooled_);
    double* __restrict__ stats = SAGEN_GRP(stats_);
    const float* __restrict__ a_inv = SAGEN_GRP(a_inv_);
    const float* __restrict__ w_inv = SAGEN_GRP(w_inv_);
    float* __restrict__ raw2 = SAGEN_GRP(raw2_);
    constexpr bool F16 = MODE != 0;
    constexpr int NPLA = MODE == 1 ? 2 : 1, NPLW = MODE == 0 ? 3 : 2;
    constexpr int W_BYTES = 14 * NPLW * S8_NH * 32;
    extern __shared__ __attribute__((aligned(16))) char smem[];
    char* const wl = smem;
    char* const pa = smem + S8_W_BYTES;
    float* const ct = reinterpret_cast<float*>(smem + S8_W_BYTES);
    float* const red = reinterpret_cast<float*>(smem + S8_W_BYTES + S8_CT_BYTES);
    float* const cb = reinterpret_cast<float*>(smem + S8_W_BYTES + S8_CT_BYTES + 2 * 8 * S8_NH * 4);
    const int tid = threadIdx.x;
    const int lane = tid & 63;
    const int wave = __builtin_amdgcn_readfirstlane(tid >> 6);
    const int li = lane & 31, g = lane >> 5;
    const int nh = blockIdx.x & 1;
    const int wg = blockIdx.x >> 1, nwg = gridDim.x >> 1;

    for (int i = tid; i < W_BYTES / 16; i += S8_THREADS) {
        const int row = i >> 1, hf = i & 1;
        const int kp = row >> 5, n = row & 31;
        reinterpret_cast<f32x4*>(wl)[i] = *reinterpret_cast<const f32x4*>(wplanes + ((long)(kp * 64 + nh * 32 + n) * 32 + 16 * (hf ^ ((n >> 3) & 1))));
    }
    if (tid < S8_NH) {
        double s = 0.0;
        if (MODE != 1)
            for (int k = 0; k < 224; ++k) s += (double)wf32[(nh * S8_NH + tid) * 224 + k];
        cb[tid] = (float)(s * (0.5 / 255.0));
    }
    const float osc = MODE == 1 ? a_inv[0] * w_inv[0] : (MODE == 2 ? w_inv[0] * (1.f / 255.f) : 1.f / 255.f);
    const int pch4 = tid & 7;
    bool use_min[4];
#pragma unroll
    for (int k = 0; k < 4; ++k) use_min[k] = OUT == 1 ? false : gamma[nh * S8_NH + 4 * pch4 + k] < 0.f;
    constexpr bool SGN = OUT == 0;
    float sgn4[4];
#pragma unroll
    for (int k = 0; k < 4; ++k) sgn4[k] = (SGN && use_min[k]) ? -1.f : 1.f;
    const float sgn_l = (SGN && gamma[nh * S8_NH + li] < 0.f) ? -1.f : 1.f;
    int poff[9];
    {
        const int p = tid >> 3;
        const int pr_l = p / S8_PW, pc_l = p - pr_l * S8_PW;
#pragma unroll
        for (int dr = 0; dr < 3; ++dr)
#pragma unroll
            for (int dc = 0; dc < 3; ++dc) poff[dr * 3 + dc] = s8_slot((2 * pr_l + dr) * S8_RW + 2 * pc_l + dc) * S8_NH + 4 * pch4;
    }
    unsigned own = 0;
#pragma unroll
    for (int e = 0; e < 16; ++e) {
        const int m = wave * 32 + (e & 3) + 8 * (e >> 2) + 4 * g;
        const int r = m / S8_RW, c = m - r * S8_RW;
        if (m < S8_M && r < 2 * S8_PH && c < 2 * S8_PW) own |= 1u << e;
    }
    float ssum = 0.f, ssq = 0.f;
    __syncthreads();
    const float cbl = cb[li] * sgn_l;
    const float osc_l = osc * sgn_l;

    const int npatch = B * 7 * 16;
    constexpr int PROWS = 2 * (S8_RH - 1) + 7, PCH = (2 * (S8_RW - 1) + 8) / 2;
    constexpr int NCHUNK = PROWS * PCH;
    constexpr int PATCH_BYTES = NCHUNK * 16;
    static_assert(NCHUNK <= 2 * S8_THREADS && NPLA * PATCH_BYTES <= S8_CT_BYTES, "patch staging");
    const int ck0 = tid, ck1 = tid + S8_THREADS;
    const int cr0 = ck0 / PCH, cc0 = ck0 - cr0 * PCH, cr1 = ck1 / PCH, cc1 = ck1 - cr1 * PCH;
    auto patch_src = [&](int patch, int crow, int ccol) {
        const int b = patch / 112, rem = patch - b * 112;
        const int pr = rem >> 4, pc = rem & 15;
        const int row = min(2 * 16 * pr + crow, S8_UH - 1);
        return plane + (((long)b * S8_UH + row) * S8_UW + 2 * 14 * pc) * 8 + ccol * 16;
    };
    f32x4 ld0[NPLA], ld1[NPLA];
#pragma unroll
    for (int p = 0; p < NPLA; ++p) {
        ld0[p] = f32x4{0.f, 0.f, 0.f, 0.f}; ld1[p] = ld0[p];
        if (wg < npatch) {
            ld0[p] = *reinterpret_cast<const f32x4*>(patch_src(wg, cr0, cc0) + p * plane_stride);
            if (ck1 < NCHUNK) ld1[p] = *reinterpret_cast<const f32x4*>(patch_src(wg, cr1, cc1) + p * plane_stride);
        }
    }
    int aoff;
    {
        const int m = wave * 32 + li;
        int r = m / S8_RW, c = m - r * S8_RW;
        if (m >= S8_M) { r = 0; c = 0; }
        aoff = ((2 * r) * (2 * PCH) + 2 * c + 2 * g) * 8;
    }
    for (int patch = wg; patch < npatch; patch += nwg) {
        const int b = patch / 112, rem = patch - b * 112;
        const int pr = rem >> 4, pc = rem & 15;
        const int R0 = 16 * pr, C0 = 14 * pc;
#pragma unroll
        for (int p = 0; p < NPLA; ++p) {
            reinterpret_cast<f32x4*>(pa + p * PATCH_BYTES)[ck0] = ld0[p];
            if (ck1 < NCHUNK) reinterpret_cast<f32x4*>(pa + p * PATCH_BYTES)[ck1] = ld1[p];
        }
        __syncthreads();
        const int next_patch = patch + nwg;
        if (next_patch < npatch) {
#pragma unroll
            for (int p = 0; p < NPLA; ++p) {
                ld0[p] = *reinterpret_cast<const f32x4*>(patch_src(next_patch, cr0, cc0) + p * plane_stride);
                if (ck1 < NCHUNK) ld1[p] = *reinterpret_cast<const f32x4*>(patch_src(next_patch, cr1, cc1) + p * plane_stride);
            }
        }
        f32x16 acc[2];
#pragma unroll
        for (int j = 0; j < 2; ++j)
#pragma unroll
            for (int e = 0; e < 16; ++e) acc[j][e] = 0.f;
#pragma unroll
        for (int ks = 0; ks < 14; ++ks) {
            bf16x8 fa[NPLA], fb[NPLW];
#pragma unroll
            for (int p = 0; p < NPLA; ++p) fa[p] = *reinterpret_cast<const bf16x8*>(pa + p * PATCH_BYTES + aoff + ((ks >> 1) * (2 * PCH) + (ks & 1) * 4) * 8);
#pragma unroll
            for (int pl = 0; pl < NPLW; ++pl) fb[pl] = *reinterpret_cast<const bf16x8*>(wl + ((ks * NPLW + pl) * S8_NH + li) * 32 + 16 * (g ^ ((li >> 3) & 1)));
            const int a = ks & 1;
            if constexpr (MODE == 2) {
                acc[a] = __builtin_amdgcn_mfma_f32_32x32x16_f16(__builtin_bit_cast(f16x8s, fa[0]), __builtin_bit_cast(f16x8s, fb[1]), acc[a], 0, 0, 0);
                acc[a ^ 1] = __builtin_amdgcn_mfma_f32_32x32x16_f16(__builtin_bit_cast(f16x8s, fa[0]), __builtin_bit_cast(f16x8s, fb[0]), acc[a ^ 1], 0, 0, 0);
            } else if constexpr (F16) {
                acc[a] = __builtin_amdgcn_mfma_f32_32x32x16_f16(__builtin_bit_cast(f16x8s, fa[NPLA - 1]), __builtin_bit_cast(f16x8s, fb[0]), acc[a], 0, 0, 0);
                acc[a ^ 1] = __builtin_amdgcn_mfma_f32_32x32x16_f16(__builtin_bit_cast(f16x8s, fa[0]), __builtin_bit_cast(f16x8s, fb[NPLW - 1]), acc[a ^ 1], 0, 0, 0);
                acc[a] = __builtin_amdgcn_mfma_f32_32x32x16_f16(__builtin_bit_cast(f16x8s, fa[0]), __builtin_bit_cast(f16x8s, fb[0]), acc[a], 0, 0, 0);
            } else {
                acc[a] = __builtin_amdgcn_mfma_f32_32x32x16_bf16(fa[0], fb[NPLW - 1], acc[a], 0, 0, 0);
                acc[a ^ 1] = __builtin_amdgcn_mfma_f32_32x32x16_bf16(fa[0], fb[1], acc[a ^ 1], 0, 0, 0);
                acc[a] = __builtin_amdgcn_mfma_f32_32x32x16_bf16(fa[0], fb[0], acc[a], 0, 0, 0);
            }
        }
        __syncthreads();
#pragma unroll
        for (int e = 0; e < 16; ++e) {
            const float v = fmaf(acc[0][e] + acc[1][e], osc_l, cbl);
            ct[s8_slot(wave * 32 + (e & 3) + 8 * (e >> 2) + 4 * g) * S8_NH + li] = v;
            const float vo = ((own >> e) & 1u) ? v : 0.f;
            ssum += vo;
            ssq = fmaf(vo, vo, ssq);
        }
        __syncthreads();
        if (OUT >= 1) {
            float* const raw = OUT == 2 ? raw2 : pooled;
            for (int it = tid; it < 2 * S8_PH * 2 * S8_PW * 8; it += S8_THREADS) {
                const int p = it >> 3, q4 = it & 7;
                const int r = p / (2 * S8_PW), cc = p - r * (2 * S8_PW);
                *reinterpret_cast<float4*>(raw + (((long)b * 112 + R0 + r) * 224 + C0 + cc) * 64 + nh * S8_NH + 4 * q4) =
                    *reinterpret_cast<const float4*>(ct + s8_slot(r * S8_RW + cc) * S8_NH + 4 * q4);
            }
        }
        if (OUT != 1 && tid < S8_PH * S8_PW * 8) {
            const int p = tid >> 3;
            const int pr_l = p / S8_PW, pc_l = p - pr_l * S8_PW;
            float4 v[9];
            if (pr < 6 && pc < 15) {
#pragma unroll
                for (int k = 0; k < 9; ++k) v[k] = *reinterpret_cast<const float4*>(ct + poff[k]);
            } else {
#pragma unroll
                for (int dr = 0; dr < 3; ++dr)
#pragma unroll
                    for (int dc = 0; dc < 3; ++dc) {
                        const int rr = (R0 + 2 * pr_l + dr >= 112) ? 2 * pr_l : 2 * pr_l + dr;
                        const int cc = (C0 + 2 * pc_l + dc >= 224) ? 2 * pc_l : 2 * pc_l + dc;
                        v[dr * 3 + dc] = *reinterpret_cast<const float4*>(ct + s8_slot(rr * S8_RW + cc) * S8_NH + 4 * pch4);
                    }
            }
            float4 ext = v[0];
            if constexpr (SGN) {
#pragma unroll
                for (int k = 1; k < 9; ++k) {
                    ext.x = fmaxf(ext.x, v[k].x); ext.y = fmaxf(ext.y, v[k].y); ext.z = fmaxf(ext.z, v[k].z); ext.w = fmaxf(ext.w, v[k].w);
                }
                ext.x *= sgn4[0]; ext.y *= sgn4[1]; ext.z *= sgn4[2]; ext.w *= sgn4[3];
            } else {
#pragma unroll
                for (int k = 1; k < 9; ++k) {
                    ext.x = use_min[0] ? fminf(ext.x, v[k].x) : fmaxf(ext.x, v[k].x); ext.y = use_min[1] ? fminf(ext.y, v[k].y) : fmaxf(ext.y, v[k].y);
                    ext.z = use_min[2] ? fminf(ext.z, v[k].z) : fmaxf(ext.z, v[k].z); ext.w = use_min[3] ? fminf(ext.w, v[k].w) : fmaxf(ext.w, v[k].w);
                }
            }
            *reinterpret_cast<float4*>(pooled + (((long)b * 56 + 8 * pr + pr_l) * 112 + 7 * pc + pc_l) * 64 + nh * S8_NH + 4 * pch4) = ext;
        }
        __syncthreads();
    }
    ssum *= sgn_l;
    ssum = wave_xor_add<32>(ssum);
    ssq = wave_xor_add<32>(ssq);
    if (g == 0) {
        red[(0 * 8 + wave) * S8_NH + li] = ssum;
        red[(1 * 8 + wave) * S8_NH + li] = ssq;
    }
    __syncthreads();
    if (tid < 2 * S8_NH) {
        const int which = tid >> 5, ch = tid & 31;
        float s = 0.f;
#pragma unroll
        for (int k = 0; k < 8; ++k) s += red[(which * 8 + k) * S8_NH + ch];
        atomicAdd(&stats[which * 64 + nh * S8_NH + ch], (double)s);
    }
}

int stem8_prep_launch(const unsigned char* x, void* plane, int B, hipStream_t s, float* zero_ptr, long zero_n, int half) {
    if (!x || !plane) return fail(SAGEN_ERR_NULL, "stem8_prep: null argument");
    if (((uintptr_t)x % 4) || ((uintptr_t)plane % 16)) return fail(SAGEN_ERR_UNSUPPORTED, "stem8_prep: the frames must be 4-byte aligned, the plane 16-byte aligned");
    const long total = (long)B * S8_UH * S8_UW / 4;
    const int grid = (int)std::min<long>(cdiv(total, 256), 256L * 16);
    const GroupInfo gi = cur_group();
    if (half) hipLaunchKernelGGL(stem8_prep_kernel<true>, dim3(grid, 1, gi.G), dim3(256), 0, s, x, reinterpret_cast<u32x2*>(plane), B, zero_ptr, zero_ptr ? zero_n : 0L, gi);
    else hipLaunchKernelGGL(stem8_prep_kernel<false>, dim3(grid, 1, gi.G), dim3(256), 0, s, x, reinterpret_cast<u32x2*>(plane), B, zero_ptr, zero_ptr ? zero_n : 0L, gi);
    SAGEN_LAUNCH_CHECK();
    return SAGEN_OK;
}

int stem8pool_launch(const void* plane, const float* wp, const float* gamma, float* pooled, double* stats, int B, hipStream_t s) {
    if (!plane || !wp || !gamma || !pooled || !stats) return fail(SAGEN_ERR_NULL, "stem8pool: null argument");
    static bool attr_set = false;
    if (!attr_set) {
        SAGEN_HIP_CHECK(hipFuncSetAttribute(reinterpret_cast<const void*>(stem8pool_kernel<0>), hipFuncAttributeMaxDynamicSharedMemorySize, S8_LDS));
        attr_set = true;
    }
    const char* planes = reinterpret_cast<const char*>(wp + 64 * 224);
    const int npatch = B * 7 * 16;
    hipLaunchKernelGGL(stem8pool_kernel<0>, dim3(2 * std::min(npatch, 256), 1, cur_group().G), dim3(S8_THREADS), S8_LDS, s, reinterpret_cast<const char*>(plane), wp, planes, gamma,
                       pooled, stats, B, 0L, (const float*)nullptr, (const float*)nullptr, (float*)nullptr, cur_group());
    SAGEN_LAUNCH_CHECK();
    return SAGEN_OK;
}

int stem8pool_h2_launch(const void* plane, const float* wp, const void* wh2, const float* w_inv, const float* gamma, float* pooled, double* stats, int B,
                        hipStream_t s) {
    if (!plane || !wp || !wh2 || !w_inv || !gamma || !pooled || !stats) return fail(SAGEN_ERR_NULL, "stem8pool_h2: null argument");
    static bool attr_set = false;
    if (!attr_set) {
        SAGEN_HIP_CHECK(hipFuncSetAttribute(reinterpret_cast<const void*>(stem8pool_kernel<0, 2>), hipFuncAttributeMaxDynamicSharedMemorySize, S8_LDS));
        attr_set = true;
    }
    const int npatch = B * 7 * 16;
    hipLaunchKernelGGL((stem8pool_kernel<0, 2>), dim3(2 * std::min(npatch, 256), 1, cur_group().G), dim3(S8_THREADS), S8_LDS, s, reinterpret_cast<const char*>(plane), wp,
                       reinterpret_cast<const char*>(wh2), gamma, pooled, stats, B, 0L, (const float*)nullptr, w_inv, (float*)nullptr, cur_group());
    SAGEN_LAUNCH_CHECK();
    return SAGEN_OK;
}

int stem8raw_launch(const void* plane, const float* wp, float* y0, double* stats, int B, hipStream_t s) {
    if (!plane || !wp || !y0 || !stats) return fail(SAGEN_ERR_NULL, "stem8raw: null argument");
    static bool attr_set = false;
    if (!attr_set) {
        SAGEN_HIP_CHECK(hipFuncSetAttribute(reinterpret_cast<const void*>(stem8pool_kernel<1>), hipFuncAttributeMaxDynamicSharedMemorySize, S8_LDS));
        attr_set = true;
    }
    const char* planes = reinterpret_cast<const char*>(wp + 64 * 224);
    const int npatch = B * 7 * 16;
    hipLaunchKernelGGL(stem8pool_kernel<1>, dim3(2 * std::min(npatch, 256), 1, cur_group().G), dim3(S8_THREADS), S8_LDS, s, reinterpret_cast<const char*>(plane), wp, planes,
                       (const float*)nullptr, y0, stats, B, 0L, (const float*)nullptr, (const float*)nullptr, (float*)nullptr, cur_group());
    SAGEN_LAUNCH_CHECK();
    return SAGEN_OK;
}

int stem8rawpool_launch(const void* plane, const float* wp, const float* gamma, float* y0, float* pooled, double* stats, int B, hipStream_t s) {
    if (!plane || !wp || !gamma || !y0 || !pooled || !stats) return fail(SAGEN_ERR_NULL, "stem8rawpool: null argument");
    static bool attr_set = false;
    if (!attr_set) {
        SAGEN_HIP_CHECK(hipFuncSetAttribute(reinterpret_cast<const void*>(stem8pool_kernel<2>), hipFuncAttributeMaxDynamicSharedMemorySize, S8_LDS));
        attr_set = true;
    }
    const char* planes = reinterpret_cast<const char*>(wp + 64 * 224);
    const int npatch = B * 7 * 16;
    hipLaunchKernelGGL(stem8pool_kernel<2>, dim3(2 * std::min(npatch, 256), 1, cur_group().G), dim3(S8_THREADS), S8_LDS, s, reinterpret_cast<const char*>(plane), wp, planes,
                       gamma, pooled, stats, B, 0L, (const float*)nullptr, (const float*)nullptr, y0, cur_group());
    SAGEN_LAUNCH_CHECK();
    return SAGEN_OK;
}

constexpr int S16_PARTS = 1024;
__global__ __launch_bounds__(256) void stem16_amax_kernel(const float* __restrict__ x_, long n4, float* __restrict__ part_, float* __restrict__ zero_ptr_, long zero_n, const GroupInfo gi) {
    const float* __restrict__ x = x_ + (size_t)blockIdx.z * (size_t)n4 * 4;
    float* __restrict__ part = SAGEN_GRP(part_);
    float* __restrict__ zero_ptr = SAGEN_GRP(zero_ptr_);
    for (long i = (long)blockIdx.x * 256 + threadIdx.x; i < zero_n; i += (long)gridDim.x * 256) zero_ptr[i] = 0.f;
    float m = 0.f;
    for (long i = (long)blockIdx.x * 256 + threadIdx.x; i < n4; i += (long)gridDim.x * 256) {
        const float4 v = reinterpret_cast<const float4*>(x)[i];
        m = fmaxf(m, fmaxf(fmaxf(fabsf(v.x), fabsf(v.y)), fmaxf(fabsf(v.z), fabsf(v.w))));
    }
    m = wave_max_f(m);
    __shared__ float s_m[4];
    if ((threadIdx.x & 63) == 0) s_m[threadIdx.x >> 6] = m;
    __syncthreads();
    if (threadIdx.x == 0) part[blockIdx.x] = fmaxf(fmaxf(s_m[0], s_m[1]), fmaxf(s_m[2], s_m[3]));
}
__global__ __launch_bounds__(256) void stem16_prep_kernel(const float* __restrict__ x_, u32x2* __restrict__ hi_, u32x2* __restrict__ lo_, int B,
                                                          const float* __restrict__ part_, float* __restrict__ a_inv_, const GroupInfo gi) {
    const float* __restrict__ x = x_ + (size_t)blockIdx.z * ((size_t)B * 224 * 448 * 3);
    u32x2* __restrict__ hi = SAGEN_GRP(hi_);
    u32x2* __restrict__ lo = SAGEN_GRP(lo_);
    const float* __restrict__ part = SAGEN_GRP(part_);
    float* __restrict__ a_inv = SAGEN_GRP(a_inv_);
    float m = 0.f;
    for (int i = threadIdx.x & 63; i < S16_PARTS; i += 64) m = fmaxf(m, part[i]);
    m = wave_max_f(m);
    const float sa = h2_scale_of_bound(m);
    if (blockIdx.x == 0 && threadIdx.x == 0) a_inv[0] = 1.f / sa;
    const long total = (long)B * S8_UH * S8_UW;
    for (long i = (long)blockIdx.x * 256 + threadIdx.x; i < total; i += (long)gridDim.x * 256) {
        long p = i;
        const int w = (int)(p % S8_UW) - 2; p /= S8_UW;
        const int h = (int)(p % S8_UH) - 2;
        const int b = (int)(p / S8_UH);
        unsigned short hh[3] = {0, 0, 0}, ll[3] = {0, 0, 0};
        if ((unsigned)h < 224u && (unsigned)w < 448u) {
            const float* src = x + (((long)b * 224 + h) * 448 + w) * 3;
#pragma unroll
            for (int c = 0; c < 3; ++c) {
                const float v = src[c] * sa;
                const _Float16 a = __builtin_isfinite(v) ? (_Float16)v : __builtin_bit_cast(_Float16, (unsigned short)0x7e00);
                const _Float16 r = __builtin_isfinite(v) ? (_Float16)(v - (float)a) : (_Float16)0.f;
                hh[c] = __builtin_bit_cast(unsigned short, a); ll[c] = __builtin_bit_cast(unsigned short, r);
            }
        }
        hi[i] = u32x2{(unsigned)hh[0] | ((unsigned)hh[1] << 16), (unsigned)hh[2]};
        lo[i] = u32x2{(unsigned)ll[0] | ((unsigned)ll[1] << 16), (unsigned)ll[2]};
    }
}

int stem16_prep_launch(const float* x, void* planes, float* part, float* a_inv, int B, hipStream_t s, float* zero_ptr, long zero_n) {
    if (!x || !planes || !part || !a_inv) return fail(SAGEN_ERR_NULL, "stem16_prep: null argument");
    const long n = (long)B * 224 * 448 * 3;
    if (n % 4 || ((uintptr_t)x % 16)) return fail(SAGEN_ERR_UNSUPPORTED, "stem16_prep: the frames must be 16-byte aligned");
    const GroupInfo gi = cur_group();
    hipLaunchKernelGGL(stem16_amax_kernel, dim3(S16_PARTS, 1, gi.G), dim3(256), 0, s, x, n / 4, part, zero_ptr, zero_ptr ? zero_n : 0L, gi);
    const long total = (long)B * S8_UH * S8_UW;
    char* p = reinterpret_cast<char*>(planes);
    hipLaunchKernelGGL(stem16_prep_kernel, dim3((int)std::min<long>(cdiv(total, 256), 256L * 16), 1, gi.G), dim3(256), 0, s, x, reinterpret_cast<u32x2*>(p),
                       reinterpret_cast<u32x2*>(p + stem8_plane_bytes(B)), B, part, a_inv, gi);
    SAGEN_LAUNCH_CHECK();
    return SAGEN_OK;
}

int stem16pool_launch(const void* planes, const void* wh2, const float* gamma, float* pooled, double* stats, const float* a_inv, const float* w_inv,
                      int B, hipStream_t s) {
    if (!planes || !wh2 || !gamma || !pooled || !stats || !a_inv || !w_inv) return fail(SAGEN_ERR_NULL, "stem16pool: null argument");
    static bool attr_set = false;
    if (!attr_set) {
        SAGEN_HIP_CHECK(hipFuncSetAttribute(reinterpret_cast<const void*>(stem8pool_kernel<0, 1>), hipFuncAttributeMaxDynamicSharedMemorySize, S8_LDS));
        attr_set = true;
    }
    const int npatch = B * 7 * 16;
    hipLaunchKernelGGL((stem8pool_kernel<0, 1>), dim3(2 * std::min(npatch, 256), 1, cur_group().G), dim3(S8_THREADS), S8_LDS, s, reinterpret_cast<const char*>(planes),
                       (const float*)nullptr, reinterpret_cast<const char*>(wh2), gamma, pooled, stats, B, (long)stem8_plane_bytes(B), a_inv, w_inv, (float*)nullptr, cur_group());
    SAGEN_LAUNCH_CHECK();
    return SAGEN_OK;
}

}
```

Baseline: 3113.

## Fuse u8 frame conversion into stem conv kernel and drop prep pass

Adds a DIRECT mode to the stem8pool kernel that reads raw interleaved u8 RGB frames, converts them to fp16 in registers via alignbyte and stages them in a separate LDS patch region. This removes the separate stem8_prep kernel and its intermediate padded plane buffer. The batch-norm accumulator zeroing it used to do moves into the STFT kernel. Separate LDS regions for the patch and the conv tile let the direct path drop two per-patch barriers. In exchange the kernel does unaligned, bounds-checked byte loads and uses more LDS per block, which may lower occupancy.

```diff
diff --git a/spatialaudiogen_amd/csrc/fft.hip b/spatialaudiogen_amd/csrc/fft.hip
--- a/spatialaudiogen_amd/csrc/fft.hip
+++ b/spatialaudiogen_amd/csrc/fft.hip
@@ -66,14 +66,17 @@
 
 __global__ __launch_bounds__(256) void stft_kernel(const float* __restrict__ audio_, int n_samples, int f0, int f1,
                                                    float* __restrict__ mag_, int c0, int c1, float2* __restrict__ spec_,
-                                                   float* __restrict__ zero_ptr_, int zero_n, const GroupInfo gi) {
+                                                   float* __restrict__ zero_ptr_, int zero_n, float* __restrict__ zero2_ptr_, int zero2_n,
+                                                   const GroupInfo gi) {
     const float* __restrict__ audio = audio_ + (size_t)blockIdx.z * ((size_t)gridDim.y * n_samples);
     float* __restrict__ mag = SAGEN_GRP(mag_);
     float2* __restrict__ spec = SAGEN_GRP(spec_);
     float* __restrict__ zero_ptr = SAGEN_GRP(zero_ptr_);
+    float* __restrict__ zero2_ptr = SAGEN_GRP(zero2_ptr_);
     __shared__ float2 bufA[1024], bufB[1024];
     const int tid = threadIdx.x;
     for (int i = (blockIdx.y * gridDim.x + blockIdx.x) * 256 + tid; i < zero_n; i += gridDim.x * gridDim.y * 256) zero_ptr[i] = 0.f;
+    for (int i = (blockIdx.y * gridDim.x + blockIdx.x) * 256 + tid; i < zero2_n; i += gridDim.x * gridDim.y * 256) zero2_ptr[i] = 0.f;
     const int b = blockIdx.y;
     const int fa = f0 + 2 * blockIdx.x, fb = fa + 1;
     const bool has_b = fb < f1;
@@ -110,7 +113,7 @@
 }
 
 int stft_launch(const float* audio, int B, int n_samples, int f0, int f1, float* mag, int c0, int c1, float* spec,
-                hipStream_t s, float* zero_ptr, int zero_n) {
+                hipStream_t s, float* zero_ptr, int zero_n, float* zero2_ptr, int zero2_n) {
     if (f1 <= f0 || 256L * (f1 - 1) + 1024 > n_samples)
         return fail(SAGEN_ERR_SHAPE, "stft: frames [%d,%d) do not fit %d samples", f0, f1, n_samples);
     if (spec && (c0 < f0 || c1 > f1 || c1 <= c0)) return fail(SAGEN_ERR_SHAPE, "stft: spec frames must lie in [f0,f1)");
@@ -118,7 +121,7 @@
     if (rc) return rc;
     const GroupInfo gi = cur_group();
     hipLaunchKernelGGL(stft_kernel, dim3(cdiv(f1 - f0, 2), B, gi.G), dim3(256), 0, s, audio, n_samples, f0, f1, mag, c0, c1,
-                       (float2*)spec, zero_ptr, zero_ptr ? zero_n : 0, gi);
+                       (float2*)spec, zero_ptr, zero_ptr ? zero_n : 0, zero2_ptr, zero2_ptr ? zero2_n : 0, gi);
     SAGEN_LAUNCH_CHECK();
     return SAGEN_OK;
 }
@@ -292,14 +295,17 @@
 
 __global__ __launch_bounds__(256) void stft_multi_kernel(const float* __restrict__ audio_, int n_samples, int nin, int f0, int f1,
                                                          float* __restrict__ mag_, int c0, int c1, float2* __restrict__ spec_,
-                                                         float* __restrict__ zero_ptr_, int zero_n, const GroupInfo gi) {
+                                                         float* __restrict__ zero_ptr_, int zero_n, float* __restrict__ zero2_ptr_, int zero2_n,
+                                                         const GroupInfo gi) {
     const float* __restrict__ audio = audio_ + (size_t)blockIdx.z * ((size_t)gridDim.y * n_samples * nin);
     float* __restrict__ mag = SAGEN_GRP(mag_);
     float2* __restrict__ spec = SAGEN_GRP(spec_);
     float* __restrict__ zero_ptr = SAGEN_GRP(zero_ptr_);
+    float* __restrict__ zero2_ptr = SAGEN_GRP(zero2_ptr_);
     __shared__ float2 bufA[1024], bufB[1024];
     const int tid = threadIdx.x;
     for (int i = (blockIdx.y * gridDim.x + blockIdx.x) * 256 + tid; i < zero_n; i += gridDim.x * gridDim.y * 256) zero_ptr[i] = 0.f;
+    for (int i = (blockIdx.y * gridDim.x + blockIdx.x) * 256 + tid; i < zero2_n; i += gridDim.x * gridDim.y * 256) zero2_ptr[i] = 0.f;
     const int b = blockIdx.y, ch = blockIdx.x % nin;
     const int fa = f0 + 2 * (blockIdx.x / nin), fb = fa + 1;
     const bool has_b = fb < f1;
@@ -337,7 +343,7 @@
 }
 
 int stft_multi_launch(const float* audio, int B, int n_samples, int nin, int f0, int f1, float* mag, int c0, int c1, float* spec,
-                      hipStream_t s, float* zero_ptr, int zero_n) {
+                      hipStream_t s, float* zero_ptr, int zero_n, float* zero2_ptr, int zero2_n) {
     if (nin < 1 || nin > 16) return fail(SAGEN_ERR_SHAPE, "stft: %d input channels", nin);
     if (f1 <= f0 || 256L * (f1 - 1) + 1024 > n_samples)
         return fail(SAGEN_ERR_SHAPE, "stft: frames [%d,%d) do not fit %d samples", f0, f1, n_samples);
@@ -346,7 +352,7 @@
     if (rc) return rc;
     const GroupInfo gi = cur_group();
     hipLaunchKernelGGL(stft_multi_kernel, dim3(cdiv(f1 - f0, 2) * nin, B, gi.G), dim3(256), 0, s, audio, n_samples, nin, f0, f1, mag, c0, c1,
-                       (float2*)spec, zero_ptr, zero_ptr ? zero_n : 0, gi);
+                       (float2*)spec, zero_ptr, zero_ptr ? zero_n : 0, zero2_ptr, zero2_ptr ? zero2_n : 0, gi);
     SAGEN_LAUNCH_CHECK();
     return SAGEN_OK;
 }
diff --git a/spatialaudiogen_amd/csrc/kernels.h b/spatialaudiogen_amd/csrc/kernels.h
--- a/spatialaudiogen_amd/csrc/kernels.h
+++ b/spatialaudiogen_amd/csrc/kernels.h
@@ -178,6 +178,8 @@
 int stem8pool_h2_launch(const void* plane, const float* wp, const void* wh2, const float* w_inv, const float* gamma, float* pooled, double* stats, int B,
                         hipStream_t s);
 int stem8pool_launch(const void* plane, const float* wp, const float* gamma, float* pooled, double* stats, int B, hipStream_t s);
+int stem8pool_u8_launch(const unsigned char* frames, const float* wp, const void* wh2, const float* w_inv, const float* gamma, float* pooled, double* stats,
+                        int B, hipStream_t s);
 int stem16_prep_launch(const float* x, void* planes, float* part, float* a_inv, int B, hipStream_t s, float* zero_ptr = nullptr, long zero_n = 0);
 int stem16pool_launch(const void* planes, const void* wh2, const float* gamma, float* pooled, double* stats, const float* a_inv, const float* w_inv,
                       int B, hipStream_t s);
@@ -221,13 +223,14 @@
 
 int fft_tables_ensure(hipStream_t s);
 int stft_launch(const float* audio, int B, int n_samples, int f0, int f1, float* mag,
-                int c0, int c1, float* spec, hipStream_t s, float* zero_ptr = nullptr, int zero_n = 0);
+                int c0, int c1, float* spec, hipStream_t s, float* zero_ptr = nullptr, int zero_n = 0,
+                float* zero2_ptr = nullptr, int zero2_n = 0);
 size_t mask_istft_scratch_bytes(int B);
 int mask_istft_mix_launch(const float* dmask, long dmask_bstride, int dmask_f0, const float* spec,
                           const float* coeffs, int B, int ntracks, float* out, float* scratch,
                           hipStream_t s, const float* ebuf = nullptr);
 int stft_multi_launch(const float* audio, int B, int n_samples, int nin, int f0, int f1, float* mag, int c0, int c1, float* spec,
-                      hipStream_t s, float* zero_ptr = nullptr, int zero_n = 0);
+                      hipStream_t s, float* zero_ptr = nullptr, int zero_n = 0, float* zero2_ptr = nullptr, int zero2_n = 0);
 size_t mask_istft_hoa_scratch_bytes(int B, int nout);
 int mask_istft_hoa_launch(const float* dmask, long dmask_bstride, int dmask_f0, const float* spec, const float* coeffs, int B,
                           int ntracks, int nin, int nout, float* out, float* scratch, hipStream_t s);
diff --git a/spatialaudiogen_amd/csrc/model.h b/spatialaudiogen_amd/csrc/model.h
--- a/spatialaudiogen_amd/csrc/model.h
+++ b/spatialaudiogen_amd/csrc/model.h
@@ -136,6 +136,7 @@
     bool stem8h = true;
     bool stem16 = true;
     bool stem8 = true;
+    bool stem_direct = true;
     size_t tws_floats = 0;
     float* tws = nullptr;
     std::map<std::string, Buf> tbufs;
@@ -547,6 +548,13 @@
         return h;
     }
 
+    bool stem8_fast(const std::string& scope) const {
+        const bool tune_general = c->tuning && c->G == 1;
+        return c->video_u8 && scope == "video_encoder" && c->stem8 && !tune_general && !c->fp32_only && !c->train_mode;
+    }
+    bool stem8_fast_h2(const std::string& scope) const { return stem8_fast(scope) && c->stem8h && h2() && c->h2_slot.count(scope + "/conv1/conv") != 0; }
+    bool stem8_direct(const std::string& scope) const { return stem8_fast_h2(scope) && c->stem_direct; }
+
     double* bn_acc(int layer_index) { return reinterpret_cast<double*>(c->p("bnacc" + sfx)) + (size_t)layer_index * 2 * 512; }
     BnRef bn_ref(int layer_index, const std::string& bn_name, long count) {
         BnRef r;
@@ -591,8 +599,9 @@
         const int B = c->B;
         int li = 0;
         const bool tune_general = c->tuning && c->G == 1;
-        const bool fast8 = c->video_u8 && scope == "video_encoder" && c->stem8 && !tune_general && !c->fp32_only && !c->train_mode;
-        const bool fast8h = fast8 && c->stem8h && h2() && c->h2_slot.count(scope + "/conv1/conv") != 0;
+        const bool fast8 = stem8_fast(scope);
+        const bool fast8h = stem8_fast_h2(scope);
+        const bool direct8 = stem8_direct(scope);
         const bool fast16 = !fast8 && !(c->video_u8 && scope == "video_encoder") && c->stem16 && !tune_general && !c->fp32_only && !c->train_mode && h2() &&
                             c->use_p3 && c->p3_from_stage <= 2 && c->bufs.count("s16:part" + sfx) != 0 && c->h2_slot.count(scope + "/conv1/conv") != 0;
         if (!fast8 && !fast16 && !rc && hipMemsetAsync(c->p("bnacc" + sfx), 0, c->bufs.at("bnacc" + sfx).n * sizeof(float), s) != hipSuccess)
@@ -605,6 +614,8 @@
         if (fast16)
             timed("stem16_amax_kernel+stem16_prep_kernel", 0.0, [&] { return stem16_prep_launch(img, c->p("xpad" + sfx), c->p("s16:part" + sfx), s16_a_inv, B, s,
                                                                                                c->p("bnacc" + sfx), (long)c->bufs.at("bnacc" + sfx).n); });
+        else if (direct8) {
+        }
         else if (fast8)
             timed("stem8_prep_kernel", 0.0, [&] { return stem8_prep_launch(reinterpret_cast<const unsigned char*>(img), c->p("xpad" + sfx), B, s,
                                                                           c->p("bnacc" + sfx), (long)c->bufs.at("bnacc" + sfx).n, fast8h ? 1 : 0); });
@@ -627,6 +638,10 @@
                     timed("stem8pool_kernel<f16>", 2.0 * B * H * W * 64 * 224, [&] {
                         return stem16pool_launch(c->p("xpad" + sfx), c->p("pkh:" + name + "/weights"), c->v(name + "/bn/gamma"), c->p("rx0" + sfx), bn_acc(li),
                                                  s16_a_inv, c->p("h2s") + c->h2_slot.at(name), B, s); });
+                else if (direct8)
+                    timed("stem8pool_kernel<h2>", 2.0 * B * H * W * 64 * 224, [&] {
+                        return stem8pool_u8_launch(reinterpret_cast<const unsigned char*>(img), c->p("pk:" + name + "/weights"), c->p("pkh:" + name + "/weights"),
+                                                   c->p("h2s") + c->h2_slot.at(name), c->v(name + "/bn/gamma"), c->p("rx0" + sfx), bn_acc(li), B, s); });
                 else if (fast8h)
                     timed("stem8pool_kernel<h2>", 2.0 * B * H * W * 64 * 224, [&] {
                         return stem8pool_h2_launch(c->p("xpad" + sfx), c->p("pk:" + name + "/weights"), c->p("pkh:" + name + "/weights"), c->p("h2s") + c->h2_slot.at(name),
diff --git a/spatialaudiogen_amd/csrc/model.hip b/spatialaudiogen_amd/csrc/model.hip
--- a/spatialaudiogen_amd/csrc/model.hip
+++ b/spatialaudiogen_amd/csrc/model.hip
@@ -40,6 +40,7 @@
     c->stem8 = getenv("SAGEN_NO_STEM8") == nullptr;
     c->stem16 = getenv("SAGEN_NO_STEM16") == nullptr;
     c->stem8h = getenv("SAGEN_NO_STEM8_H2") == nullptr;
+    c->stem_direct = getenv("SAGEN_NO_STEM_DIRECT") == nullptr;
     c->use_h2 = getenv("SAGEN_NO_H2") == nullptr;
     c->train_h2 = getenv("SAGEN_TRAIN_NO_H2") == nullptr;
     c->train_h2d = getenv("SAGEN_TRAIN_NO_H2D") == nullptr;
@@ -471,14 +472,16 @@
     const bool dec_planes = !no_decp && c->B >= c->dec_planes_min_batch && !c->sk_fused && c->freq_mask && !(c->train_mode && (train_no_decp || !c->train_bands)) &&
                             !c->fp32_only && f.h2() && c->bufs.count("catp") != 0 && !c->no_scatter;
     const bool want_amax = d1_planes || dec_planes;
+    float* const bn_zero = c->has_video && f.stem8_direct("video_encoder") ? c->p("bnacc") : nullptr;
+    const int bn_zero_n = bn_zero ? (int)c->bufs.at("bnacc").n : 0;
 
     g.layer = "stft";
     if (c->nin == 1)
         g.timed("stft_kernel", 0.0, [&] { return stft_launch(audio, B, c->snd_size, 46, 173, c->p("mag"), 89, 117, c->p("spec"), g.s,
-                                                             want_amax ? c->p("amax") : nullptr, 10 * H2_AMAX_FLOATS + 64); });
+                                                             want_amax ? c->p("amax") : nullptr, 10 * H2_AMAX_FLOATS + 64, bn_zero, bn_zero_n); });
     else
         g.timed("stft_multi_kernel", 0.0, [&] { return stft_multi_launch(audio, B, c->snd_size, c->nin, 46, 173, c->p("mag"), 89, 117, c->p("spec"), g.s,
-                                                                         want_amax ? c->p("amax") : nullptr, 10 * H2_AMAX_FLOATS + 64); });
+                                                                         want_amax ? c->p("amax") : nullptr, 10 * H2_AMAX_FLOATS + 64, bn_zero, bn_zero_n); });
     if (forked) {
         SAGEN_HIP_CHECK(hipEventRecord(c->ev_stft, c->aux));
         f.wait_before_mfma = c->ev_stft;
@@ -846,6 +849,7 @@
     if (n == "u8_fast_stem") { c->stem8 = value != 0; return SAGEN_OK; }
     if (n == "f16_fast_stem") { c->stem16 = value != 0; return SAGEN_OK; }
     if (n == "u8_stem_h2") { c->stem8h = value != 0; return SAGEN_OK; }
+    if (n == "stem_direct") { c->stem_direct = value != 0; return SAGEN_OK; }
     if (n == "train_bands") { c->train_bands = value != 0; return SAGEN_OK; }
     if (n == "train_rawpool") { c->train_rawpool = value != 0; return SAGEN_OK; }
     if (n == "fp16x2") { c->use_h2 = value != 0; return SAGEN_OK; }
diff --git a/spatialaudiogen_amd/csrc/stem8.hip b/spatialaudiogen_amd/csrc/stem8.hip
--- a/spatialaudiogen_amd/csrc/stem8.hip
+++ b/spatialaudiogen_amd/csrc/stem8.hip
@@ -14,6 +14,7 @@
 constexpr int S8_CT_BYTES = 256 * S8_NH * 4;
 constexpr int S8_THREADS = 512;
 constexpr int S8_LDS = S8_W_BYTES + S8_CT_BYTES + 2 * 8 * S8_NH * 4 + S8_NH * 4;
+constexpr int S8D_LDS = 14 * 2 * S8_NH * 32 + S8_CT_BYTES + 702 * 16 + 2 * 8 * S8_NH * 4 + S8_NH * 4;
 typedef _Float16 f16x8s __attribute__((ext_vector_type(8)));
 
 size_t stem8_plane_bytes(int B) { return (size_t)B * S8_UH * S8_UW * 8; }
@@ -76,7 +77,8 @@
                                                                   float* __restrict__ pooled_, double* __restrict__ stats_, int B,
                                                                   long plane_stride, const float* __restrict__ a_inv_, const float* __restrict__ w_inv_,
                                                                   float* __restrict__ raw2_, const GroupInfo gi) {
-    const char* __restrict__ plane = SAGEN_GRP(plane_);
+    constexpr bool DIRECT = MODE == 3;
+    const char* __restrict__ plane = DIRECT ? plane_ + (size_t)blockIdx.z * ((size_t)B * 224 * 448 * 3) : SAGEN_GRP(plane_);
     float* __restrict__ pooled = SAGEN_GRP(pooled_);
     double* __restrict__ stats = SAGEN_GRP(stats_);
     const float* __restrict__ a_inv = SAGEN_GRP(a_inv_);
@@ -85,12 +87,19 @@
     constexpr bool F16 = MODE != 0;
     constexpr int NPLA = MODE == 1 ? 2 : 1, NPLW = MODE == 0 ? 3 : 2;
     constexpr int W_BYTES = 14 * NPLW * S8_NH * 32;
+    constexpr int PROWS = 2 * (S8_RH - 1) + 7, PCH = (2 * (S8_RW - 1) + 8) / 2;
+    constexpr int NCHUNK = PROWS * PCH;
+    constexpr int PATCH_BYTES = NCHUNK * 16;
+    constexpr int CT_OFF = DIRECT ? W_BYTES : S8_W_BYTES;
+    constexpr int PA_OFF = DIRECT ? CT_OFF + S8_CT_BYTES : CT_OFF;
+    constexpr int RED_OFF = DIRECT ? PA_OFF + PATCH_BYTES : CT_OFF + S8_CT_BYTES;
+    static_assert(RED_OFF + 2 * 8 * S8_NH * 4 + S8_NH * 4 <= (DIRECT ? S8D_LDS : S8_LDS), "LDS layout");
     extern __shared__ __attribute__((aligned(16))) char smem[];
     char* const wl = smem;
-    char* const pa = smem + S8_W_BYTES;
-    float* const ct = reinterpret_cast<float*>(smem + S8_W_BYTES);
-    float* const red = reinterpret_cast<float*>(smem + S8_W_BYTES + S8_CT_BYTES);
-    float* const cb = reinterpret_cast<float*>(smem + S8_W_BYTES + S8_CT_BYTES + 2 * 8 * S8_NH * 4);
+    char* const pa = smem + PA_OFF;
+    float* const ct = reinterpret_cast<float*>(smem + CT_OFF);
+    float* const red = reinterpret_cast<float*>(smem + RED_OFF);
+    float* const cb = reinterpret_cast<float*>(smem + RED_OFF + 2 * 8 * S8_NH * 4);
     const int tid = threadIdx.x;
     const int lane = tid & 63;
     const int wave = __builtin_amdgcn_readfirstlane(tid >> 6);
@@ -109,7 +118,7 @@
             for (int k = 0; k < 224; ++k) s += (double)wf32[(nh * S8_NH + tid) * 224 + k];
         cb[tid] = (float)(s * (0.5 / 255.0));
     }
-    const float osc = MODE == 1 ? a_inv[0] * w_inv[0] : (MODE == 2 ? w_inv[0] * (1.f / 255.f) : 1.f / 255.f);
+    const float osc = MODE == 1 ? a_inv[0] * w_inv[0] : (MODE >= 2 ? w_inv[0] * (1.f / 255.f) : 1.f / 255.f);
     const int pch4 = tid & 7;
     bool use_min[4];
 #pragma unroll
@@ -141,9 +150,6 @@
     const float osc_l = osc * sgn_l;
 
     const int npatch = B * 7 * 16;
-    constexpr int PROWS = 2 * (S8_RH - 1) + 7, PCH = (2 * (S8_RW - 1) + 8) / 2;
-    constexpr int NCHUNK = PROWS * PCH;
-    constexpr int PATCH_BYTES = NCHUNK * 16;
     static_assert(NCHUNK <= 2 * S8_THREADS && NPLA * PATCH_BYTES <= S8_CT_BYTES, "patch staging");
     const int ck0 = tid, ck1 = tid + S8_THREADS;
     const int cr0 = ck0 / PCH, cc0 = ck0 - cr0 * PCH, cr1 = ck1 / PCH, cc1 = ck1 - cr1 * PCH;
@@ -153,13 +159,47 @@
         const int row = min(2 * 16 * pr + crow, S8_UH - 1);
         return plane + (((long)b * S8_UH + row) * S8_UW + 2 * 14 * pc) * 8 + ccol * 16;
     };
+    struct U8Chunk { unsigned d0, d1, d2; int sh; };
+    const int coff0 = (cr0 * 448 + 2 * cc0) * 3, coff1 = (cr1 * 448 + 2 * cc1) * 3;
+    auto chunk_load = [&](int patch, int crow, int ccol, int coff) {
+        U8Chunk k{0u, 0u, 0u, -1};
+        const int b = patch / 112, rem = patch - b * 112;
+        const int pr = rem >> 4, pc = rem & 15;
+        const int h0 = 32 * pr - 2, w0 = 28 * pc - 2;
+        if ((unsigned)(h0 + crow) < 224u && (unsigned)(w0 + 2 * ccol) < 448u) {
+            const char* const a = plane + (((long)b * 224 + h0) * 448 + w0) * 3 + coff;
+            k.sh = (int)(reinterpret_cast<uintptr_t>(a) & 3);
+            const unsigned* q = reinterpret_cast<const unsigned*>(a - k.sh);
+            k.d0 = q[0]; k.d1 = q[1];
+            if (k.sh == 3) k.d2 = q[2];
+        }
+        return k;
+    };
+    auto chunk_store = [&](int ck, const U8Chunk& k) {
+        u32x4 o = u32x4{0xB800B800u, 0x0000B800u, 0xB800B800u, 0x0000B800u};
+        if (k.sh >= 0) {
+            const unsigned lo = __builtin_amdgcn_alignbyte(k.d1, k.d0, (unsigned)k.sh) ^ 0x80808080u;
+            const unsigned hi = __builtin_amdgcn_alignbyte(k.d2, k.d1, (unsigned)k.sh) ^ 0x80808080u;
+            auto f = [](unsigned v, int i) { return (unsigned)__builtin_bit_cast(unsigned short, (_Float16)(short)(signed char)(v >> (8 * i))); };
+            o = u32x4{f(lo, 0) | (f(lo, 1) << 16), f(lo, 2), f(lo, 3) | (f(hi, 0) << 16), f(hi, 1)};
+        }
+        reinterpret_cast<u32x4*>(pa)[ck] = o;
+    };
     f32x4 ld0[NPLA], ld1[NPLA];
-#pragma unroll
-    for (int p = 0; p < NPLA; ++p) {
-        ld0[p] = f32x4{0.f, 0.f, 0.f, 0.f}; ld1[p] = ld0[p];
+    U8Chunk u0{0u, 0u, 0u, -1}, u1{0u, 0u, 0u, -1};
+    if constexpr (DIRECT) {
         if (wg < npatch) {
-            ld0[p] = *reinterpret_cast<const f32x4*>(patch_src(wg, cr0, cc0) + p * plane_stride);
-            if (ck1 < NCHUNK) ld1[p] = *reinterpret_cast<const f32x4*>(patch_src(wg, cr1, cc1) + p * plane_stride);
+            u0 = chunk_load(wg, cr0, cc0, coff0);
+            if (ck1 < NCHUNK) u1 = chunk_load(wg, cr1, cc1, coff1);
+        }
+    } else {
+#pragma unroll
+        for (int p = 0; p < NPLA; ++p) {
+            ld0[p] = f32x4{0.f, 0.f, 0.f, 0.f}; ld1[p] = ld0[p];
+            if (wg < npatch) {
+                ld0[p] = *reinterpret_cast<const f32x4*>(patch_src(wg, cr0, cc0) + p * plane_stride);
+                if (ck1 < NCHUNK) ld1[p] = *reinterpret_cast<const f32x4*>(patch_src(wg, cr1, cc1) + p * plane_stride);
+            }
         }
     }
     int aoff;
@@ -173,18 +213,28 @@
         const int b = patch / 112, rem = patch - b * 112;
         const int pr = rem >> 4, pc = rem & 15;
         const int R0 = 16 * pr, C0 = 14 * pc;
-#pragma unroll
-        for (int p = 0; p < NPLA; ++p) {
-            reinterpret_cast<f32x4*>(pa + p * PATCH_BYTES)[ck0] = ld0[p];
-            if (ck1 < NCHUNK) reinterpret_cast<f32x4*>(pa + p * PATCH_BYTES)[ck1] = ld1[p];
-        }
-        __syncthreads();
         const int next_patch = patch + nwg;
-        if (next_patch < npatch) {
+        if constexpr (DIRECT) {
+            chunk_store(ck0, u0);
+            if (ck1 < NCHUNK) chunk_store(ck1, u1);
+            if (next_patch < npatch) {
+                u0 = chunk_load(next_patch, cr0, cc0, coff0);
+                if (ck1 < NCHUNK) u1 = chunk_load(next_patch, cr1, cc1, coff1);
+            }
+            __syncthreads();
+        } else {
 #pragma unroll
             for (int p = 0; p < NPLA; ++p) {
-                ld0[p] = *reinterpret_cast<const f32x4*>(patch_src(next_patch, cr0, cc0) + p * plane_stride);
-                if (ck1 < NCHUNK) ld1[p] = *reinterpret_cast<const f32x4*>(patch_src(next_patch, cr1, cc1) + p * plane_stride);
+                reinterpret_cast<f32x4*>(pa + p * PATCH_BYTES)[ck0] = ld0[p];
+                if (ck1 < NCHUNK) reinterpret_cast<f32x4*>(pa + p * PATCH_BYTES)[ck1] = ld1[p];
+            }
+            __syncthreads();
+            if (next_patch < npatch) {
+#pragma unroll
+                for (int p = 0; p < NPLA; ++p) {
+                    ld0[p] = *reinterpret_cast<const f32x4*>(patch_src(next_patch, cr0, cc0) + p * plane_stride);
+                    if (ck1 < NCHUNK) ld1[p] = *reinterpret_cast<const f32x4*>(patch_src(next_patch, cr1, cc1) + p * plane_stride);
+                }
             }
         }
         f32x16 acc[2];
@@ -200,7 +250,7 @@
 #pragma unroll
             for (int pl = 0; pl < NPLW; ++pl) fb[pl] = *reinterpret_cast<const bf16x8*>(wl + ((ks * NPLW + pl) * S8_NH + li) * 32 + 16 * (g ^ ((li >> 3) & 1)));
             const int a = ks & 1;
-            if constexpr (MODE == 2) {
+            if constexpr (MODE >= 2) {
                 acc[a] = __builtin_amdgcn_mfma_f32_32x32x16_f16(__builtin_bit_cast(f16x8s, fa[0]), __builtin_bit_cast(f16x8s, fb[1]), acc[a], 0, 0, 0);
                 acc[a ^ 1] = __builtin_amdgcn_mfma_f32_32x32x16_f16(__builtin_bit_cast(f16x8s, fa[0]), __builtin_bit_cast(f16x8s, fb[0]), acc[a ^ 1], 0, 0, 0);
             } else if constexpr (F16) {
@@ -213,7 +263,7 @@
                 acc[a] = __builtin_amdgcn_mfma_f32_32x32x16_bf16(fa[0], fb[0], acc[a], 0, 0, 0);
             }
         }
-        __syncthreads();
+        if constexpr (!DIRECT) __syncthreads();
 #pragma unroll
         for (int e = 0; e < 16; ++e) {
             const float v = fmaf(acc[0][e] + acc[1][e], osc_l, cbl);
@@ -265,7 +315,7 @@
             }
             *reinterpret_cast<float4*>(pooled + (((long)b * 56 + 8 * pr + pr_l) * 112 + 7 * pc + pc_l) * 64 + nh * S8_NH + 4 * pch4) = ext;
         }
-        __syncthreads();
+        if constexpr (!DIRECT) __syncthreads();
     }
     ssum *= sgn_l;
     ssum = wave_xor_add<32>(ssum);
@@ -321,6 +371,21 @@
     }
     const int npatch = B * 7 * 16;
     hipLaunchKernelGGL((stem8pool_kernel<0, 2>), dim3(2 * std::min(npatch, 256), 1, cur_group().G), dim3(S8_THREADS), S8_LDS, s, reinterpret_cast<const char*>(plane), wp,
+                       reinterpret_cast<const char*>(wh2), gamma, pooled, stats, B, 0L, (const float*)nullptr, w_inv, (float*)nullptr, cur_group());
+    SAGEN_LAUNCH_CHECK();
+    return SAGEN_OK;
+}
+
+int stem8pool_u8_launch(const unsigned char* frames, const float* wp, const void* wh2, const float* w_inv, const float* gamma, float* pooled, double* stats,
+                        int B, hipStream_t s) {
+    if (!frames || !wp || !wh2 || !w_inv || !gamma || !pooled || !stats) return fail(SAGEN_ERR_NULL, "stem8pool_u8: null argument");
+    static bool attr_set = false;
+    if (!attr_set) {
+        SAGEN_HIP_CHECK(hipFuncSetAttribute(reinterpret_cast<const void*>(stem8pool_kernel<0, 3>), hipFuncAttributeMaxDynamicSharedMemorySize, S8D_LDS));
+        attr_set = true;
+    }
+    const int npatch = B * 7 * 16;
+    hipLaunchKernelGGL((stem8pool_kernel<0, 3>), dim3(2 * std::min(npatch, 256), 1, cur_group().G), dim3(S8_THREADS), S8D_LDS, s, reinterpret_cast<const char*>(frames), wp,
                        reinterpret_cast<const char*>(wh2), gamma, pooled, stats, B, 0L, (const float*)nullptr, w_inv, (float*)nullptr, cur_group());
     SAGEN_LAUNCH_CHECK();
     return SAGEN_OK;
```

After: 3133 (median of 6 runs). No clear change (+0.7%).
